# choi403/ALG

Hardware: AMD Instinct MI355X
Metric: frames/sec (whole node) CogVideoX-5B-I2V 49f x 50-step ALG (higher is better)
Workload: dtype bf16; 1 GPU; BASELINE config 2: CogVideoX-5B-I2V bf16, 49 frames @ 480x720, 50 steps, ALG interval down_up (resize_factor 0.25, interval [0, 0.04]), guidance 6.0; one video per GPU; layers=42, dit_sample_forwards=14, parallelism=dp1

## Files before the change

### alg_amd/_lib.py

```python
from __future__ import annotations

import ctypes
from collections import OrderedDict
import os
from ctypes import POINTER, Structure, byref, c_char_p, c_float, c_int, c_int32, c_int64, c_void_p

import torch

_HERE = os.path.dirname(os.path.abspath(__file__))
LIB_PATH = os.environ.get("ALG_HIP_LIB") or os.path.join(_HERE, "libalg_hip.so")

ALG_F32, ALG_BF16 = 0, 1
ACT_NONE, ACT_GELU_TANH, ACT_SILU = 0, 1, 2
GEMM_BIAS_PER_ROW, GEMM_PERMUTE_COLS, GEMM_GATE_F32, GEMM_GATE_SEG_STRIDE = 1, 4, 8, 16
GEMM_B_PACKED11 = 32

EXPORTS = (
    "alg_version", "alg_last_error", "alg_reload_env", "alg_down_up", "alg_gaussian_blur", "alg_cfg_ddim_step", "alg_gemm_bf16", "alg_gemm_bf16_pair", "alg_gemm_bf16_pair_qk", "alg_pack_b_p11", "alg_pack_b_p11_bytes",
    "alg_flash_attn_d64", "alg_layernorm_modulate", "alg_qk_norm_rope", "alg_patchify", "alg_unpatchify",
    "alg_timestep_embedding", "alg_cfg_combine", "alg_lincomb", "alg_unipc_update", "alg_concat_cast", "alg_flash_attn_d128", "alg_layernorm_mod_f32", "alg_layernorm_mod_f32_fp8", "alg_rmsnorm_rope",
    "alg_wan_modulation", "alg_patchify3d", "alg_unpatchify3d", "alg_timestep_embedding_f32", "alg_linear_f32",
    "alg_gelu_erf", "alg_layernorm_modulate_seg", "alg_headnorm_rope", "alg_masked_mean", "alg_silu", "alg_gemm_fp8", "alg_quantize_fp8_rows",
    "alg_conv_cl_bf16", "alg_vae_groupnorm_workspace", "alg_vae_groupnorm_stats", "alg_vae_spatial_norm", "alg_vae_upsample",
    "alg_vae_pack_latent", "alg_vae_unpack_video", "alg_vae_group_norm", "alg_vae_pad", "alg_vae_repitch",
    "alg_vae_unpack_planes", "alg_rms_norm_rows", "alg_softmax_hilo", "alg_flash_attn_d128_ex", "alg_flash_attn_d128_dual", "alg_rope_half", "alg_patchify_t", "alg_unpatchify_t", "alg_qk_norm_rope_scaled", "alg_flash_attn_d64_ex", "alg_embed_rows", "alg_t5_layernorm", "alg_attn_bias", "alg_mul_bf16", "alg_quick_gelu",
    "alg_lowpass_tables_bytes", "alg_lowpass_tables_build", "alg_down_up_workspace_bytes", "alg_gaussian_blur_workspace_bytes",
    "alg_flash_attn_d64_workspace_bytes", "alg_calib_mfma_bf16", "alg_wall_clock_khz", "alg_attn_clock_tap",
)
_RET_I64 = ("alg_vae_groupnorm_workspace", "alg_lowpass_tables_bytes", "alg_down_up_workspace_bytes",
            "alg_gaussian_blur_workspace_bytes", "alg_flash_attn_d64_workspace_bytes", "alg_pack_b_p11_bytes")


class AlgHipError(RuntimeError):
    pass


class GemmArgs(Structure):
    _fields_ = [
        ("A", c_void_p), ("B", c_void_p), ("C", c_void_p), ("bias", c_void_p), ("R", c_void_p), ("gate", c_void_p),
        ("lda", c_int64), ("ldb", c_int64), ("ldc", c_int64), ("ldr", c_int64),
        ("strideA", c_int64), ("strideB", c_int64), ("strideC", c_int64), ("strideR", c_int64),
        ("strideGate", c_int64),
        ("M", c_int32), ("N", c_int32), ("K", c_int32), ("batch", c_int32),
        ("seg_split", c_int32), ("act", c_int32), ("flags", c_int32),
        ("gate_seg_stride", c_int64), ("perm_col0", c_int32), ("conv_cin_log2", c_int32),
        ("a_scale", c_void_p), ("b_scale", c_void_p), ("strideAScale", c_int64), ("strideBScale", c_int64),
        ("conv_wp", c_int32), ("conv_hpwp", c_int32), ("conv_kw", c_int32), ("reserved1", c_int32),
    ]


class QkNormRopeArgs(Structure):
    _fields_ = [("wq", c_void_p), ("bq", c_void_p), ("wk", c_void_p), ("bk", c_void_p), ("cos_tab", c_void_p),
                ("sin_tab", c_void_p), ("heads", c_int32), ("text_len", c_int32), ("eps", c_float),
                ("q_scale", c_float)]


class VaeGeom(Structure):
    _fields_ = [(n, c_int32) for n in ("frames", "H", "W", "C", "first_len", "seg_len", "lat_first_single", "lat_rate",
                                       "lat_scale", "lat_h", "lat_w")]


_lib = None


def build_library(verbose=False):
    import subprocess

    src = os.path.join(_HERE, "csrc")
    r = subprocess.run(["make", "-C", src, "-j8"], capture_output=True, text=True)
    if verbose or r.returncode != 0:
        print(r.stdout[-4000:])
        print(r.stderr[-4000:])
    if r.returncode != 0:
        raise AlgHipError("building libalg_hip.so failed (see output above)")
    return LIB_PATH


def load_library():
    global _lib
    if _lib is not None:
        return _lib
    if not os.path.exists(LIB_PATH):
        raise AlgHipError(
            "%s not found: the HIP extension is not built (run `python -c 'import __graft_entry__ as g; g.build()'` "
            "or `make -C alg_amd/csrc`).  There is no CPU fallback for the ALG hot path." % LIB_PATH)
    lib = ctypes.CDLL(LIB_PATH)
    lib.alg_version.restype = c_int
    lib.alg_last_error.restype = c_char_p
    lib.alg_reload_env.restype = None
    lib.alg_reload_env.argtypes = []
    lib.alg_down_up.argtypes = [c_void_p, c_void_p, c_int64, c_int, c_int, c_int, c_int, c_int, c_int, c_void_p, c_void_p,
                                c_int64, c_void_p]
    lib.alg_gaussian_blur.argtypes = [c_void_p, c_void_p, c_int64, c_int, c_int, c_int, c_float, c_int, c_void_p, c_int64,
                                      c_void_p]
    lib.alg_lowpass_tables_bytes.argtypes = [c_int] * 4
    lib.alg_lowpass_tables_build.argtypes = [c_void_p, c_int64] + [c_int] * 4 + [c_void_p]
    lib.alg_down_up_workspace_bytes.argtypes = [c_int64] + [c_int] * 4
    lib.alg_gaussian_blur_workspace_bytes.argtypes = [c_int64] + [c_int] * 3
    lib.alg_flash_attn_d64_workspace_bytes.argtypes = [c_int] * 4
    lib.alg_pack_b_p11_bytes.argtypes = [c_int, c_int]
    lib.alg_pack_b_p11_bytes.restype = c_int64
    lib.alg_pack_b_p11.argtypes = [c_void_p, c_void_p, c_int, c_int, c_int64, c_void_p]
    lib.alg_cfg_ddim_step.argtypes = [c_void_p, c_int, c_void_p, c_int, c_int, c_int64, c_float, c_float, c_float,
                                      c_float, c_float, c_void_p]
    lib.alg_cfg_combine.argtypes = [c_void_p, c_void_p, c_int, c_int, c_int64, c_float, c_void_p]
    lib.alg_lincomb.argtypes = [POINTER(c_void_p), POINTER(c_float), POINTER(c_int), c_int, c_void_p, c_int, c_int64,
                                c_void_p]
    lib.alg_concat_cast.argtypes = [POINTER(c_void_p), c_int, POINTER(c_void_p), c_int, c_int] + [c_int64] * 7 + [
        c_void_p, c_int, c_void_p]
    lib.alg_flash_attn_d128.argtypes = [c_void_p] * 4 + [c_int] * 4 + [c_int64] * 8 + [c_float, c_void_p]
    lib.alg_flash_attn_d128_ex.argtypes = [c_void_p] * 4 + [c_int] * 4 + [c_int64] * 8 + [c_float, c_int, c_int, c_void_p]
    lib.alg_flash_attn_d128_dual.argtypes = ([c_void_p] * 3 + [c_int] + [c_int64] * 4 + [c_void_p] * 2 + [c_int] + [c_int64] * 4 +
                                             [c_void_p] + [c_int] * 3 + [c_int64] * 4 + [c_float, c_void_p])
    lib.alg_rope_half.argtypes = [c_void_p, c_void_p, c_void_p, c_void_p, c_int64, c_int, c_int64, c_void_p]
    lib.alg_layernorm_mod_f32.argtypes = [c_void_p] * 6 + [c_int64, c_int, c_int, c_int, c_float, c_void_p]
    lib.alg_layernorm_mod_f32_fp8.argtypes = [c_void_p] * 7 + [c_int64, c_int, c_int, c_int, c_float, c_void_p]
    lib.alg_rmsnorm_rope.argtypes = [c_void_p] * 4 + [c_int64, c_int, c_int, c_int, c_float, c_void_p]
    lib.alg_wan_modulation.argtypes = [c_void_p] * 3 + [c_int] * 5 + [c_void_p]
    lib.alg_patchify3d.argtypes = [c_void_p, c_void_p] + [c_int] * 8 + [c_void_p]
    lib.alg_unpatchify3d.argtypes = [c_void_p, c_int64, c_void_p] + [c_int] * 8 + [c_void_p]
    lib.alg_layernorm_modulate_seg.argtypes = [c_void_p] * 6 + [c_int64, c_int64, c_int, c_int, c_int, c_int64, c_int64,
                                               c_int, c_float, c_void_p]
    lib.alg_headnorm_rope.argtypes = [c_void_p] * 4 + [c_int64, c_int64, c_int, c_int, c_int, c_int, c_float, c_void_p]
    lib.alg_masked_mean.argtypes = [c_void_p, c_void_p, c_void_p, c_int, c_int, c_int, c_void_p]
    lib.alg_silu.argtypes = [c_void_p, c_void_p, c_int64, c_void_p]
    lib.alg_rms_norm_rows.argtypes = [c_void_p, c_void_p, c_void_p, c_int64, c_int, c_int, c_int, c_void_p]
    lib.alg_softmax_hilo.argtypes = [c_void_p, c_void_p, c_void_p, c_int64, c_int, c_int64, ctypes.c_float, c_void_p]
    lib.alg_gemm_fp8.argtypes = [POINTER(GemmArgs), c_void_p]
    lib.alg_conv_cl_bf16.argtypes = [c_void_p] * 5 + [c_int] * 7 + [c_void_p]
    lib.alg_vae_groupnorm_workspace.argtypes = [POINTER(VaeGeom)]
    lib.alg_vae_groupnorm_stats.argtypes = [c_void_p, POINTER(VaeGeom), c_float, c_void_p, c_void_p, c_void_p]
    lib.alg_vae_spatial_norm.argtypes = [c_void_p] * 6 + [POINTER(VaeGeom), c_int, c_void_p]
    lib.alg_vae_group_norm.argtypes = [c_void_p] * 5 + [POINTER(VaeGeom), c_int, c_void_p]
    lib.alg_vae_pad.argtypes = [c_void_p, c_void_p] + [c_int] * 4 + [c_void_p]
    lib.alg_vae_repitch.argtypes = [c_void_p, c_void_p] + [c_int] * 6 + [c_void_p]
    lib.alg_vae_unpack_planes.argtypes = [c_void_p, c_void_p] + [c_int] * 4 + [c_void_p]
    lib.alg_embed_rows.argtypes = [c_void_p, c_void_p, c_void_p, c_int64, c_int, c_int, c_void_p]
    lib.alg_t5_layernorm.argtypes = [c_void_p, c_void_p, c_void_p, c_int64, c_int, c_float, c_void_p]
    lib.alg_attn_bias.argtypes = [c_void_p] * 7 + [c_int, c_int, c_int, c_int, c_int64, c_int64, c_float, c_int, c_void_p]
    lib.alg_quick_gelu.argtypes = [c_void_p, c_int64, c_void_p]
    lib.alg_mul_bf16.argtypes = [c_void_p, c_void_p, c_void_p, c_int64, c_void_p]
    lib.alg_vae_upsample.argtypes = [c_void_p, c_void_p] + [c_int] * 6 + [c_void_p]
    lib.alg_vae_pack_latent.argtypes = [c_void_p, c_int64, c_int64, c_void_p, c_int, c_int, c_int, c_int, c_float, c_void_p]
    lib.alg_vae_unpack_video.argtypes = [c_void_p, c_void_p, c_int, c_int, c_int, c_int, c_void_p]
    lib.alg_quantize_fp8_rows.argtypes = [c_void_p, c_int64, c_void_p, c_void_p, c_int64, c_int, c_void_p]
    lib.alg_timestep_embedding_f32.argtypes = [c_void_p, c_void_p, c_int, c_int, c_void_p]
    lib.alg_linear_f32.argtypes = [c_void_p] * 6 + [c_int] * 4 + [c_void_p]
    lib.alg_gelu_erf.argtypes = [c_void_p, c_int64, c_void_p]
    lib.alg_unipc_update.argtypes = [c_void_p] * 5 + [c_int64] + [c_float] * 6 + [c_void_p]
    lib.alg_gemm_bf16.argtypes = [POINTER(GemmArgs), c_void_p]
    lib.alg_gemm_bf16_pair.argtypes = [POINTER(GemmArgs), POINTER(GemmArgs), c_void_p]
    lib.alg_gemm_bf16_pair_qk.argtypes = [POINTER(GemmArgs), POINTER(GemmArgs), POINTER(QkNormRopeArgs), c_void_p]
    lib.alg_flash_attn_d64.argtypes = [c_void_p, c_void_p, c_void_p, c_void_p, c_int, c_int, c_int, c_int64, c_int64,
                                       c_int64, c_int64, c_int64, c_int64, c_float, c_void_p]
    lib.alg_layernorm_modulate.argtypes = [c_void_p, c_void_p, c_void_p, c_void_p, c_void_p, c_void_p, c_int64, c_int,
                                           c_int, c_int, c_int64, c_int64, c_int, c_float, c_void_p]
    lib.alg_qk_norm_rope.argtypes = [c_void_p, c_void_p, c_void_p, c_void_p, c_void_p, c_void_p, c_void_p, c_int,
                                     c_int, c_int, c_int, c_float, c_void_p]
    lib.alg_qk_norm_rope_scaled.argtypes = [c_void_p] * 7 + [c_int, c_int, c_int, c_int, c_float, c_float, c_void_p]
    lib.alg_flash_attn_d64_ex.argtypes = [c_void_p, c_void_p, c_void_p, c_void_p, c_int, c_int, c_int, c_int64, c_int64,
                                          c_int64, c_int64, c_int64, c_int64, c_float, c_int, c_void_p, c_int64, c_void_p]
    lib.alg_patchify.argtypes = [c_void_p, c_int64, POINTER(c_void_p), c_void_p, c_int, c_int, c_int, c_int, c_int,
                                 c_int, c_void_p]
    lib.alg_unpatchify.argtypes = [c_void_p, c_void_p, c_int, c_int, c_int, c_int, c_int, c_int, c_void_p]
    lib.alg_patchify_t.argtypes = [c_void_p, c_int64, POINTER(c_void_p), c_void_p] + [c_int] * 7 + [c_void_p]
    lib.alg_unpatchify_t.argtypes = [c_void_p, c_void_p] + [c_int] * 7 + [c_void_p]
    lib.alg_timestep_embedding.argtypes = [c_void_p, c_void_p, c_int, c_int, c_int, c_void_p]
    lib.alg_calib_mfma_bf16.argtypes = [c_void_p, c_int, ctypes.c_uint, c_int, c_void_p, c_void_p]
    lib.alg_attn_clock_tap.argtypes = [c_void_p, c_int]
    for name in EXPORTS:
        fn = getattr(lib, name)
        if name == "alg_attn_clock_tap":
            fn.restype = None
        elif name not in ("alg_version", "alg_last_error", "alg_reload_env"):
            fn.restype = c_int64 if name in _RET_I64 else c_int
    _lib = lib
    return lib


def reload_env():
    load_library().alg_reload_env()


def _check(rc, what):
    if rc != 0:
        msg = load_library().alg_last_error()
        raise AlgHipError("%s failed (code %d): %s" % (what, rc, msg.decode() if msg else "?"))


def _stream():
    return c_void_p(torch.cuda.current_stream().cuda_stream)


def _dt(t):
    if t.dtype == torch.float32:
        return ALG_F32
    if t.dtype == torch.bfloat16:
        return ALG_BF16
    raise AlgHipError("unsupported dtype %s (the HIP path handles float32 and bfloat16)" % t.dtype)


def _dev(t, name):
    if not t.is_cuda:
        raise AlgHipError("%s must be a device tensor: the ALG hot path is HIP-only (no CPU fallback)" % name)
    return t


def _ptr(t):
    return c_void_p(t.data_ptr()) if t is not None else c_void_p(0)



_TABLES = OrderedDict()
_TABLES_MAX = 64
_SCRATCH = {}
_PINNED = {}


def _stream_key(t):
    return (t.device.index, torch.cuda.current_stream(t.device).cuda_stream)


def _capturing():
    return torch.cuda.is_available() and torch.cuda.is_current_stream_capturing()


def _pin(t):
    _PINNED[id(t)] = t
    return t


def release_captured_buffers():
    _PINNED.clear()


def clear_caches():
    _TABLES.clear()
    _SCRATCH.clear()


def lowpass_tables(x, h1, w1):
    lib = load_library()
    H, W = x.shape[-2:]
    key = _stream_key(x) + (H, W, h1, w1)
    cap = _capturing()
    t = _TABLES.get(key)
    if t is not None:
        _TABLES.move_to_end(key)
        return _pin(t) if cap else t
    n = int(lib.alg_lowpass_tables_bytes(H, W, h1, w1))
    if n <= 0:
        return None
    t = torch.empty(n, dtype=torch.uint8, device=x.device)
    _check(lib.alg_lowpass_tables_build(_ptr(t), n, H, W, h1, w1, _stream()), "alg_lowpass_tables_build")
    if cap:
        return _pin(t)
    _TABLES[key] = t
    while len(_TABLES) > _TABLES_MAX:
        _TABLES.popitem(last=False)
    return t


def scratch(ref, nbytes, tag):
    if nbytes <= 0:
        return None
    key = _stream_key(ref) + (tag,)
    t = _SCRATCH.get(key)
    cap = _capturing()
    if t is None or t.numel() < nbytes:
        t = torch.empty(int(nbytes), dtype=torch.uint8, device=ref.device)
        if cap:
            return _pin(t)
        _SCRATCH[key] = t
    return _pin(t) if cap else t


def calib_mfma_bf16(sink, iters, seed=1, blocks=0, clocks=None):
    lib = load_library()
    if clocks is not None:
        if int(blocks) <= 0:
            blocks = 2 * torch.cuda.get_device_properties(sink.device).multi_processor_count
        if not (clocks.is_cuda and clocks.device == sink.device and clocks.dtype == torch.int64 and clocks.is_contiguous()
                and clocks.numel() >= 4 * int(blocks)):
            raise AlgHipError("calib_mfma_bf16: clocks must be a contiguous int64 tensor on the sink's device with >= 4 * %d "
                              "elements" % int(blocks))
    rc = lib.alg_calib_mfma_bf16(_ptr(_dev(sink, "sink")), int(iters), int(seed), int(blocks), _ptr(clocks), _stream())
    if rc <= 0:
        _check(rc if rc < 0 else -1, "alg_calib_mfma_bf16")
    return rc


def wall_clock_khz():
    return int(load_library().alg_wall_clock_khz())


def attn_clock_tap(buffer):
    lib = load_library()
    if buffer is None:
        lib.alg_attn_clock_tap(None, 0)
        return
    if not (buffer.is_cuda and buffer.dtype == torch.int64 and buffer.is_contiguous() and buffer.dim() == 2 and buffer.shape[1] == 4):
        raise AlgHipError("attn_clock_tap needs a contiguous int64 device tensor [slots, 4]")
    lib.alg_attn_clock_tap(_ptr(buffer), int(buffer.shape[0]))


def clock_mhz_from_taps(taps, wall_khz):
    t = taps.detach().cpu().to(torch.float64)
    dc, dw = t[:, 2] - t[:, 0], t[:, 3] - t[:, 1]
    ok = (dc > 0) & (dw > 0)
    if not bool(ok.any()) or wall_khz <= 0:
        return None
    mhz = dc[ok] / dw[ok] * (wall_khz / 1e3)
    return {"mean": float(mhz.mean()), "min": float(mhz.min()), "max": float(mhz.max()), "workgroups": int(ok.sum())}


def down_up(x, h1, w1, round_intermediate=True):
    lib = load_library()
    _dev(x, "x")
    if not x.is_contiguous():
        raise AlgHipError("down_up needs a contiguous tensor")
    H, W = x.shape[-2:]
    planes = x.numel() // (H * W) if x.numel() else 0
    out = torch.empty_like(x)
    if planes == 0:
        return out
    wsb = int(lib.alg_down_up_workspace_bytes(planes, H, W, h1, w1))
    ws = scratch(x, wsb, "down_up")
    tables = lowpass_tables(x, h1, w1) if wsb == 0 else None
    _check(lib.alg_down_up(_ptr(x), _ptr(out), planes, H, W, h1, w1, _dt(x), 1 if round_intermediate else 0,
                           _ptr(tables), _ptr(ws), wsb, _stream()), "alg_down_up")
    return out


def gaussian_blur(x, ksize, sigma):
    lib = load_library()
    _dev(x, "x")
    if not x.is_contiguous():
        raise AlgHipError("gaussian_blur needs a contiguous tensor")
    H, W = x.shape[-2:]
    planes = x.numel() // (H * W) if x.numel() else 0
    out = torch.empty_like(x)
    wsb = int(lib.alg_gaussian_blur_workspace_bytes(planes, H, W, int(ksize))) if planes else 0
    ws = scratch(x, wsb, "gaussian")
    _check(lib.alg_gaussian_blur(_ptr(x), _ptr(out), planes, H, W, int(ksize), float(sigma), _dt(x), _ptr(ws), wsb,
                                 _stream()), "alg_gaussian_blur")
    return out


def cfg_ddim_step_(pred, latents, n_pass, guidance_scale, sqrt_alpha_t, sqrt_beta_t, coef_a, coef_b):
    lib = load_library()
    _dev(pred, "pred")
    _dev(latents, "latents")
    if not (pred.is_contiguous() and latents.is_contiguous()):
        raise AlgHipError("cfg_ddim_step_ needs contiguous tensors")
    numel = latents.numel()
    if pred.numel() != n_pass * numel:
        raise AlgHipError("pred has %d elements, expected n_pass*numel = %d" % (pred.numel(), n_pass * numel))
    _check(lib.alg_cfg_ddim_step(_ptr(pred), _dt(pred), _ptr(latents), _dt(latents), n_pass, numel,
                                 float(guidance_scale), float(sqrt_alpha_t), float(sqrt_beta_t), float(coef_a),
                                 float(coef_b), _stream()), "alg_cfg_ddim_step")
    return latents


def cfg_combine(pred, n_pass, guidance_scale):
    lib = load_library()
    _dev(pred, "pred")
    if not pred.is_contiguous() or pred.shape[0] % n_pass:
        raise AlgHipError("cfg_combine needs a contiguous [n_pass * B, ...] tensor")
    out = torch.empty((pred.shape[0] // n_pass,) + tuple(pred.shape[1:]), device=pred.device, dtype=pred.dtype)
    _check(lib.alg_cfg_combine(_ptr(pred), _ptr(out), _dt(pred), n_pass, out.numel(), float(guidance_scale), _stream()),
           "alg_cfg_combine")
    return out


def lincomb(terms, out_dtype, out=None):
    lib = load_library()
    xs = [t for _, t in terms]
    for t in xs:
        _dev(t, "term")
        if not t.is_contiguous() or t.shape != xs[0].shape:
            raise AlgHipError("lincomb needs contiguous tensors of one shape")
    n = len(xs)
    if out is None:
        out = torch.empty(xs[0].shape, device=xs[0].device, dtype=out_dtype)
    elif out.dtype != out_dtype or out.shape != xs[0].shape or not out.is_contiguous():
        raise AlgHipError("lincomb: `out` must be a contiguous tensor of the requested dtype and shape")
    arr = (c_void_p * n)(*[t.data_ptr() for t in xs])
    cf = (c_float * n)(*[float(c) for c, _ in terms])
    dts = (c_int * n)(*[_dt(t) for t in xs])
    _check(lib.alg_lincomb(arr, cf, dts, n, _ptr(out), ALG_F32 if out_dtype == torch.float32 else ALG_BF16,
                           out.numel(), _stream()), "alg_lincomb")
    return out


def concat_cast(src0, src1, O, A0, A1, R, s0_ostride, s1_ostride, a1_off, out_dtype):
    lib = load_library()
    n = len(src0)
    for t in list(src0) + list(src1):
        _dev(t, "concat source")
        if not t.is_contiguous():
            raise AlgHipError("concat_cast needs contiguous sources")
    out = torch.empty((n, O, A0 + A1, R), device=src0[0].device, dtype=out_dtype)
    a0 = (c_void_p * n)(*[t.data_ptr() for t in src0])
    a1 = (c_void_p * n)(*[t.data_ptr() for t in src1])
    _check(lib.alg_concat_cast(a0, _dt(src0[0]), a1, _dt(src1[0]), n, O, A0, A1, R, s0_ostride, s1_ostride, a1_off,
                               _ptr(out), ALG_F32 if out_dtype == torch.float32 else ALG_BF16, _stream()),
           "alg_concat_cast")
    return out


def rope_half_(x, cos, sin, pos, rows, heads, x_rstride, x_off=0):
    _check(load_library().alg_rope_half(_p(x, x_off), _p(cos), _p(sin), _p(pos), rows, heads, x_rstride, _stream()),
           "alg_rope_half")
    return x


def flash_attn_d128_dual(q, k, vt, Skv, k_bs, k_rs, vt_bs, vt_rs, k2, vt2, Skv2, k2_bs, k2_rs, vt2_bs, vt2_rs, o, batch, heads, Sq,
                         q_bs, q_rs, o_bs, o_rs, scale):
    lib = load_library()
    for t in (q, k, vt, k2, vt2, o):
        _dev(t, "attention operand")
    _check(lib.alg_flash_attn_d128_dual(_p(q), _p(k), _p(vt), Skv, k_bs, k_rs, vt_bs, vt_rs, _p(k2), _p(vt2), Skv2, k2_bs, k2_rs,
                                        vt2_bs, vt2_rs, _p(o), batch, heads, Sq, q_bs, q_rs, o_bs, o_rs, float(scale), _stream()),
           "alg_flash_attn_d128_dual")
    return o


def flash_attn_d128(q, k, vt, o, batch, heads, Sq, Skv, q_bs, q_rs, k_bs, k_rs, vt_bs, vt_rs, o_bs, o_rs, scale,
                    q_off=0, k_off=0, vt_off=0, o_off=0, kv_group=1, causal=False):
    lib = load_library()
    for t in (q, k, vt, o):
        _dev(t, "attention operand")
    at = lambda t, off: c_void_p(t.data_ptr() + 2 * off)
    if kv_group != 1 or causal:
        _check(lib.alg_flash_attn_d128_ex(at(q, q_off), at(k, k_off), at(vt, vt_off), at(o, o_off), batch, heads, Sq, Skv, q_bs,
                                          q_rs, k_bs, k_rs, vt_bs, vt_rs, o_bs, o_rs, float(scale), int(kv_group),
                                          int(bool(causal)), _stream()), "alg_flash_attn_d128_ex")
        return o
    _check(lib.alg_flash_attn_d128(at(q, q_off), at(k, k_off), at(vt, vt_off), at(o, o_off), batch, heads, Sq, Skv, q_bs, q_rs, k_bs, k_rs, vt_bs, vt_rs, o_bs, o_rs, float(scale),
                                   _stream()), "alg_flash_attn_d128")
    return o


def _p(t, off=0):
    if t is None:
        return c_void_p(0)
    _dev(t, "tensor")
    return c_void_p(t.data_ptr() + off * t.element_size())


def layernorm_mod_f32(x, y, weight, bias, scale, shift, mod_bstride, batch, rows, D, eps, scale_off=0, shift_off=0):
    _check(load_library().alg_layernorm_mod_f32(_p(x), _p(y), _p(weight), _p(bias), _p(scale, scale_off),
                                                _p(shift, shift_off), mod_bstride, batch, rows, D, float(eps), _stream()),
           "alg_layernorm_mod_f32")
    return y


def layernorm_mod_f32_fp8(x, q8, q8_scale, weight, bias, scale, shift, mod_bstride, batch, rows, D, eps, scale_off=0,
                          shift_off=0):
    _check(load_library().alg_layernorm_mod_f32_fp8(_p(x), _p(q8), _p(q8_scale), _p(weight), _p(bias),
                                                    _p(scale, scale_off), _p(shift, shift_off), mod_bstride, batch, rows,
                                                    D, float(eps), _stream()), "alg_layernorm_mod_f32_fp8")
    return q8


def rmsnorm_rope_(x, weight, cos, sin, x_rstride, batch, rows, D, eps, x_off=0):
    _check(load_library().alg_rmsnorm_rope(_p(x, x_off), _p(weight), _p(cos), _p(sin), x_rstride, batch, rows, D,
                                           float(eps), _stream()), "alg_rmsnorm_rope")
    return x


def wan_modulation(table, vec, out, layers, batch, J, D, vec_per_j):
    _check(load_library().alg_wan_modulation(_p(table), _p(vec), _p(out), layers, batch, J, D, int(vec_per_j), _stream()),
           "alg_wan_modulation")
    return out


def patchify3d(x, out, n, C, F, H, W, ph, pw, Kpad):
    _check(load_library().alg_patchify3d(_p(x), _p(out), n, C, F, H, W, ph, pw, Kpad, _stream()), "alg_patchify3d")
    return out


def unpatchify3d(x, ldin, out, n, C, F, H, W, ph, pw, channel_major=False):
    _check(load_library().alg_unpatchify3d(_p(x), ldin, _p(out), n, C, F, H, W, ph, pw, int(channel_major), _stream()),
           "alg_unpatchify3d")
    return out


def layernorm_modulate_seg(x, y, weight, bias, scale, shift, mod_bstride, seg_stride, batch, rows, D, seg_split, eps,
                           x_bstride=None, y_bstride=None, x_off=0, y_off=0, scale_off=0, shift_off=0):
    x_bstride = rows * D if x_bstride is None else x_bstride
    y_bstride = rows * D if y_bstride is None else y_bstride
    _check(load_library().alg_layernorm_modulate_seg(_p(x, x_off), _p(y, y_off), _p(weight), _p(bias), _p(scale, scale_off),
                                                     _p(shift, shift_off), mod_bstride, seg_stride, batch, rows, D,
                                                     x_bstride, y_bstride, seg_split, float(eps), _stream()),
           "alg_layernorm_modulate_seg")
    return y


def headnorm_rope_(x, weight, cos, sin, x_rstride, x_bstride, batch, rows, heads, rope_tokens, eps, x_off=0):
    _check(load_library().alg_headnorm_rope(_p(x, x_off), _p(weight), _p(cos), _p(sin), x_rstride, x_bstride, batch, rows,
                                            heads, rope_tokens, float(eps), _stream()), "alg_headnorm_rope")
    return x


def masked_mean(x, valid, out, batch, L, D):
    _check(load_library().alg_masked_mean(_p(x), _p(valid), _p(out), batch, L, D, _stream()), "alg_masked_mean")
    return out


def silu(x, y):
    _check(load_library().alg_silu(_p(x), _p(y), x.numel(), _stream()), "alg_silu")
    return y


def rms_norm_rows(x, gamma, y, rows, C, Cp, silu=True):
    _check(load_library().alg_rms_norm_rows(_p(x), _p(gamma), _p(y), rows, C, Cp, int(silu), _stream()), "alg_rms_norm_rows")
    return y


def softmax_hilo(neg_hi, lo, p, rows, cols, ld, scale):
    _check(load_library().alg_softmax_hilo(_p(neg_hi), _p(lo), _p(p), rows, cols, ld, float(scale), _stream()),
           "alg_softmax_hilo")
    return p


CONV_PLAIN, CONV_PAIR, CONV_STRIDE2 = 0, 1, 2


def conv_cl(x, w, bias, res, y, frames, Hp, Wp, Cin, Cout, kt, pair=False, stride2=False, x_off=0, y_off=0, res_off=0):
    mode = CONV_STRIDE2 if stride2 else (CONV_PAIR if pair else CONV_PLAIN)
    _check(load_library().alg_conv_cl_bf16(_p(x, x_off), _p(w), _p(bias), _p(res, res_off), _p(y, y_off), frames, Hp, Wp,
                                           Cin, Cout, kt, mode, _stream()), "alg_conv_cl_bf16")
    return y


def embed_rows(ids, table, out):
    _check(load_library().alg_embed_rows(_p(ids), _p(table), _p(out), ids.numel(), table.shape[1], table.shape[0],
                                         _stream()), "alg_embed_rows")
    return out


def t5_layernorm(x, weight, y, rows, D, eps):
    _check(load_library().alg_t5_layernorm(_p(x), _p(weight), _p(y), rows, D, eps, _stream()), "alg_t5_layernorm")
    return y


def attn_bias(qkv, out, bias_table, rel_bucket, key_mask, batch, heads, L, scale=1.0, head_dim=64, causal=False):
    inner = heads * head_dim
    _check(load_library().alg_attn_bias(_p(qkv), _p(qkv, inner), _p(qkv, 2 * inner), _p(out), _p(bias_table),
                                        _p(rel_bucket), _p(key_mask), batch, heads, head_dim, L, 3 * inner, inner,
                                        float(scale), int(causal), _stream()), "alg_attn_bias")
    return out


def quick_gelu_(x):
    _check(load_library().alg_quick_gelu(_p(x), x.numel(), _stream()), "alg_quick_gelu")
    return x


def mul_bf16(a, b, out):
    _check(load_library().alg_mul_bf16(_p(a), _p(b), _p(out), a.numel(), _stream()), "alg_mul_bf16")
    return out


def vae_group_norm(x, stats, gamma, beta, out, g, silu=True):
    _check(load_library().alg_vae_group_norm(_p(x), _p(stats), _p(gamma), _p(beta), _p(out), byref(g), int(silu),
                                             _stream()), "alg_vae_group_norm")
    return out


def vae_pad(x, out, frames, H, W, C):
    _check(load_library().alg_vae_pad(_p(x), _p(out), frames, H, W, C, _stream()), "alg_vae_pad")
    return out


def vae_repitch(x, out, frames, H, W, C, src_rows, src_wp):
    _check(load_library().alg_vae_repitch(_p(x), _p(out), frames, H, W, C, src_rows, src_wp, _stream()), "alg_vae_repitch")
    return out


def vae_unpack_planes(x, out, frames, H, W, C):
    _check(load_library().alg_vae_unpack_planes(_p(x), _p(out), frames, H, W, C, _stream()), "alg_vae_unpack_planes")
    return out


def pack_conv_pair(w, bias, taps_t):
    co = w.shape[0]
    w = w.reshape(co, taps_t, 3, 3, -1)
    wp = w.new_zeros(2, co, taps_t, 3, 4, w.shape[-1])
    wp[0, :, :, :, 0:3] = w
    wp[1, :, :, :, 1:4] = w
    return wp.reshape(2 * co, -1).contiguous(), torch.cat([bias, bias]).contiguous()


def vae_geom(**kw):
    g = VaeGeom()
    for k, v in kw.items():
        setattr(g, k, v)
    return g


def vae_groupnorm_workspace(g):
    n = load_library().alg_vae_groupnorm_workspace(byref(g))
    if n < 0:
        _check(1, "alg_vae_groupnorm_workspace")
    return n


def vae_groupnorm_stats(x, g, eps, workspace, stats):
    _check(load_library().alg_vae_groupnorm_stats(_p(x), byref(g), eps, _p(workspace), _p(stats), _stream()),
           "alg_vae_groupnorm_stats")
    return stats


def vae_spatial_norm(x, stats, gamma, beta, zyb, out, g, silu=True):
    _check(load_library().alg_vae_spatial_norm(_p(x), _p(stats), _p(gamma), _p(beta), _p(zyb), _p(out), byref(g),
                                               int(silu), _stream()), "alg_vae_spatial_norm")
    return out


def vae_upsample(x, out, frames_out, H, W, C, compress_time, first_single):
    _check(load_library().alg_vae_upsample(_p(x), _p(out), frames_out, H, W, C, int(compress_time), int(first_single),
                                           _stream()), "alg_vae_upsample")
    return out


def vae_pack_latent(z, c_stride, frame_stride, out, frames, h, w, channels, scale, z_off=0):
    _check(load_library().alg_vae_pack_latent(_p(z, z_off), c_stride, frame_stride, _p(out), frames, h, w, channels, scale,
                                              _stream()), "alg_vae_pack_latent")
    return out


def vae_unpack_video(x, out, frames, H, W, to_uint8=False):
    _check(load_library().alg_vae_unpack_video(_p(x), _p(out), frames, H, W, int(to_uint8), _stream()),
           "alg_vae_unpack_video")
    return out


def timestep_embedding_f32(t, out, n, dim):
    _check(load_library().alg_timestep_embedding_f32(_p(t), _p(out), n, dim, _stream()), "alg_timestep_embedding_f32")
    return out


def linear_f32(x, W, b, y, y_bf16, y_silu_bf16, M, N, K, act=0):
    _check(load_library().alg_linear_f32(_p(x), _p(W), _p(b), _p(y), _p(y_bf16), _p(y_silu_bf16), M, N, K, act, _stream()),
           "alg_linear_f32")


def gelu_erf_(x):
    _check(load_library().alg_gelu_erf(_p(x), x.numel(), _stream()), "alg_gelu_erf")
    return x


def unipc_update(x, m0, m1, m_new, r, c, k, rk=1.0, rho0=0.0, rho_new=0.0):
    lib = load_library()
    for t in (x, m0, m1, m_new):
        if t is None:
            continue
        _dev(t, "unipc term")
        if t.dtype != torch.float32 or not t.is_contiguous() or t.shape != x.shape:
            raise AlgHipError("unipc_update needs contiguous fp32 tensors of one shape")
    out = torch.empty_like(x)
    p = lambda t: None if t is None else _ptr(t)
    _check(lib.alg_unipc_update(p(x), p(m0), p(m1), p(m_new), _ptr(out), x.numel(), float(r), float(c), float(k),
                                float(rk), float(rho0), float(rho_new), _stream()), "alg_unipc_update")
    return out


def gemm_args(A, B, C, M, N, K, lda, ldb, ldc, bias=None, R=None, ldr=0, gate=None, batch=1, strideA=0, strideB=0,
              strideC=0, strideR=0, strideGate=0, seg_split=0, act=ACT_NONE, flags=0, a_off=0, b_off=0, c_off=0, r_off=0,
              gate_off=0, gate_seg_stride=None, bias_off=0, perm_col0=0, a_scale=None, b_scale=None, strideAScale=0,
              strideBScale=0, a_scale_off=0, b_scale_off=0):
    args = GemmArgs()
    fp8 = a_scale is not None
    if isinstance(B, PackedB):
        if (B.N, B.K) != (N, K) or b_off or strideB:
            raise AlgHipError("packed B was built for N = %d, K = %d (shared by the batch, no offset)" % (B.N, B.K))
        flags |= GEMM_B_PACKED11
    args.A = A.data_ptr() + A.element_size() * a_off
    args.B = B.data_ptr() + B.element_size() * b_off
    if fp8:
        args.a_scale = a_scale.data_ptr() + 4 * a_scale_off
        args.b_scale = b_scale.data_ptr() + 4 * b_scale_off
        args.strideAScale, args.strideBScale = strideAScale, strideBScale
    args.C = C.data_ptr() + 2 * c_off
    args.bias = (bias.data_ptr() + 2 * bias_off) if bias is not None else None
    if gate_seg_stride is not None:
        flags |= GEMM_GATE_SEG_STRIDE
        args.gate_seg_stride = gate_seg_stride
    args.R = (R.data_ptr() + 2 * r_off) if R is not None else None
    args.gate = (gate.data_ptr() + gate.element_size() * gate_off) if gate is not None else None
    args.lda, args.ldb, args.ldc, args.ldr = lda, ldb, ldc, ldr
    args.strideA, args.strideB, args.strideC, args.strideR, args.strideGate = strideA, strideB, strideC, strideR, strideGate
    args.M, args.N, args.K, args.batch = M, N, K, batch
    args.seg_split, args.act, args.flags = seg_split, act, flags
    args.perm_col0 = perm_col0
    return args, fp8


class PackedB:

    def __init__(self, w):
        lib = load_library()
        _dev(w, "weight")
        if w.dtype != torch.bfloat16 or w.dim() != 2 or w.stride(1) != 1:
            raise AlgHipError("PackedB takes a 2-D bf16 weight with unit column stride")
        self.N, self.K = int(w.shape[0]), int(w.shape[1])
        nbytes = int(lib.alg_pack_b_p11_bytes(self.N, self.K))
        if nbytes <= 0:
            raise AlgHipError("PackedB: K = %d must be a positive multiple of 64" % self.K)
        self.data = torch.empty(nbytes, dtype=torch.uint8, device=w.device)
        _check(lib.alg_pack_b_p11(_ptr(w), _ptr(self.data), self.N, self.K, int(w.stride(0)), _stream()), "alg_pack_b_p11")

    def data_ptr(self):
        return self.data.data_ptr()

    def element_size(self):
        return 2


def gemm(*a, **kw):
    lib = load_library()
    args, fp8 = gemm_args(*a, **kw)
    if fp8:
        _check(lib.alg_gemm_fp8(ctypes.byref(args), _stream()), "alg_gemm_fp8")
    else:
        _check(lib.alg_gemm_bf16(ctypes.byref(args), _stream()), "alg_gemm_bf16")


def gemm_pair(first, second):
    lib = load_library()
    a, fa = gemm_args(*first[0], **first[1])
    b, fb = gemm_args(*second[0], **second[1])
    if fa or fb:
        raise AlgHipError("gemm_pair takes bf16 problems")
    _check(lib.alg_gemm_bf16_pair(ctypes.byref(a), ctypes.byref(b), _stream()), "alg_gemm_bf16_pair")


def gemm_pair_qk(first, second, wq, bq, wk, bk, cos, sin, heads, text_len, eps, q_scale=1.0):
    lib = load_library()
    a, fa = gemm_args(*first[0], **first[1])
    b, fb = gemm_args(*second[0], **second[1])
    if fa or fb:
        raise AlgHipError("gemm_pair_qk takes bf16 problems")
    ptrs = [t.data_ptr() if t is not None else None for t in (wq, bq, wk, bk, cos, sin)]
    e = QkNormRopeArgs(*ptrs, heads, text_len, float(eps), float(q_scale))
    _check(lib.alg_gemm_bf16_pair_qk(ctypes.byref(a), ctypes.byref(b), ctypes.byref(e), _stream()), "alg_gemm_bf16_pair_qk")


def quantize_fp8_rows(x, q, scale, rows, K, x_rstride=None, x_off=0, q_off=0, scale_off=0):
    x_rstride = K if x_rstride is None else x_rstride
    _check(load_library().alg_quantize_fp8_rows(_p(x, x_off), x_rstride, _p(q, q_off), _p(scale, scale_off), rows, K,
                                                _stream()), "alg_quantize_fp8_rows")
    return q, scale


ATTN_Q_PRESCALED = 1


def flash_attn_d64(q, k, vt, o, batch, heads, S, q_bstride, q_rstride, vt_bstride, vt_rstride, o_bstride, o_rstride,
                   scale, q_off=0, k_off=0, q_prescaled=False):
    lib = load_library()
    flags = ATTN_Q_PRESCALED if q_prescaled else 0
    wsb = int(lib.alg_flash_attn_d64_workspace_bytes(batch, heads, S, flags))
    ws = scratch(o, wsb, "attn_d64")
    _check(lib.alg_flash_attn_d64_ex(c_void_p(q.data_ptr() + 2 * q_off), c_void_p(k.data_ptr() + 2 * k_off), _ptr(vt),
                                     _ptr(o), batch, heads, S, q_bstride, q_rstride, vt_bstride, vt_rstride, o_bstride,
                                     o_rstride, float(scale), flags, _ptr(ws), wsb, _stream()),
           "alg_flash_attn_d64")


def layernorm_modulate(x, y, weight, bias, scale, shift, mod_bstride, batch, rows, D, seg_split, eps,
                       x_bstride=None, y_bstride=None, x_off=0, y_off=0, scale_off=0, shift_off=0):
    lib = load_library()
    x_bstride = rows * D if x_bstride is None else x_bstride
    y_bstride = rows * D if y_bstride is None else y_bstride
    sc = c_void_p(scale.data_ptr() + 2 * scale_off) if scale is not None else c_void_p(0)
    sh = c_void_p(shift.data_ptr() + 2 * shift_off) if shift is not None else c_void_p(0)
    _check(lib.alg_layernorm_modulate(c_void_p(x.data_ptr() + 2 * x_off), c_void_p(y.data_ptr() + 2 * y_off),
                                      _ptr(weight), _ptr(bias), sc, sh, mod_bstride, batch, rows, D, x_bstride,
                                      y_bstride, seg_split, float(eps), _stream()), "alg_layernorm_modulate")


def qk_norm_rope_(qk, wq, bq, wk, bk, cos, sin, batch, S, heads, text_len, eps, q_scale=1.0):
    lib = load_library()
    _check(lib.alg_qk_norm_rope_scaled(_ptr(qk), _ptr(wq), _ptr(bq), _ptr(wk), _ptr(bk), _ptr(cos), _ptr(sin), batch, S,
                                       heads, text_len, float(eps), float(q_scale), _stream()), "alg_qk_norm_rope")


def patchify(latents, lat_bstride, conds, out, n_samples, frames, C, H, W, p, p_t=1):
    lib = load_library()
    arr = (c_void_p * n_samples)(*[c.data_ptr() for c in conds])
    _check(lib.alg_patchify_t(_ptr(latents), lat_bstride, arr, _ptr(out), n_samples, frames, C, H, W, p, p_t, _stream()),
           "alg_patchify")


def unpatchify(x, out, n_samples, frames, C, H, W, p, p_t=1):
    lib = load_library()
    _check(lib.alg_unpatchify_t(_ptr(x), _ptr(out), n_samples, frames, C, H, W, p, p_t, _stream()), "alg_unpatchify")


def timestep_embedding(t, out, n, dim, flip_sin_to_cos=True):
    lib = load_library()
    _check(lib.alg_timestep_embedding(_ptr(t), _ptr(out), n, dim, 1 if flip_sin_to_cos else 0, _stream()),
           "alg_timestep_embedding")
```

### alg_amd/csrc/gemm.hip

```cpp
#include <stdlib.h>

#include "common.h"

namespace alg {
constexpr int BM = 256, BN = 256;
int launch_gemm_p6(const alg_gemm_args* a, int m_tiles, int n_tiles, int64_t nwg, hipStream_t s);
int launch_gemm_p9(const alg_gemm_args* a, int m_tiles, int n_tiles, int64_t nwg, hipStream_t s);
int launch_gemm_p9_pair(const alg_gemm_args* a, int m_tiles_a, int n_tiles_a, const alg_gemm_args* b, int m_tiles_b, int n_tiles_b,
                        hipStream_t s);
int launch_gemm_p9_pair_qk(const alg_gemm_args* a, int m_tiles_a, int n_tiles_a, const alg_gemm_args* b, int m_tiles_b, int n_tiles_b,
                           const alg_qk_norm_rope_args* e, hipStream_t s);
int launch_gemm_p10(const alg_gemm_args* a, int m_tiles, int n_tiles, int64_t nwg, hipStream_t s);
int launch_gemm_p10_pair(const alg_gemm_args* a, int m_tiles_a, int n_tiles_a, const alg_gemm_args* b, int m_tiles_b, int n_tiles_b,
                         hipStream_t s);
int launch_gemm_p10_pair_qk(const alg_gemm_args* a, int m_tiles_a, int n_tiles_a, const alg_gemm_args* b, int m_tiles_b, int n_tiles_b,
                            const alg_qk_norm_rope_args* e, hipStream_t s);
int launch_gemm_p11(const alg_gemm_args* a, int m_tiles, int n_tiles, int64_t nwg, hipStream_t s);
int launch_gemm_p6_fp8(const alg_gemm_args* a, int m_tiles, int n_tiles, int64_t nwg, hipStream_t s);
int launch_gemm_p9_fp8(const alg_gemm_args* a, int m_tiles, int n_tiles, int64_t nwg, hipStream_t s);
int launch_gemm_p6_conv(const alg_gemm_args* a, int m_tiles, int n_tiles, int64_t nwg, hipStream_t s);
static int gemm_pipe() { return opt(OPT_GEMM_PIPE); }
static bool asm_pipe() { return gemm_pipe() == 9 || gemm_pipe() == 10; }
}

using namespace alg;

static int gemm_entry(const alg_gemm_args* a, void* stream, bool fp8, bool validate_only = false) {
  if (!a || !a->A || !a->B || !a->C) {
    set_error("alg_gemm_bf16: null argument");
    return ALG_EINVAL;
  }
  if (a->M <= 0 || a->N <= 0 || a->K <= 0 || a->batch <= 0) {
    set_error("alg_gemm_bf16: bad shape M=%d N=%d K=%d batch=%d", a->M, a->N, a->K, a->batch);
    return ALG_EINVAL;
  }
  if (a->K % (fp8 ? 128 : 64) != 0) {
    set_error("alg_gemm_%s: K=%d must be a multiple of %d", fp8 ? "fp8" : "bf16", a->K, fp8 ? 128 : 64);
    return ALG_EINVAL;
  }
  const int al = fp8 ? 16 : 8;
  if (a->lda % al || a->ldb % al || a->strideA % al || a->strideB % al || ((uintptr_t)a->A & 15) ||
      ((uintptr_t)a->B & 15)) {
    set_error("alg_gemm: A/B must be 16-byte aligned with lda/ldb/strides multiples of 16 bytes");
    return ALG_EINVAL;
  }
  if (fp8 && (!a->a_scale || !a->b_scale || ((uintptr_t)a->b_scale & 15) || (a->strideBScale & 3))) {
    set_error("alg_gemm_fp8: a_scale / b_scale are required (b_scale 16-byte aligned)");
    return ALG_EINVAL;
  }
  if (a->act < ALG_ACT_NONE || a->act > ALG_ACT_SILU) {
    set_error("alg_gemm_bf16: unknown activation %d", a->act);
    return ALG_EINVAL;
  }
  if ((a->flags & ALG_GEMM_PERMUTE_COLS) && (a->R || a->gate)) {
    set_error("alg_gemm_bf16: PERMUTE_COLS cannot be combined with residual/gate");
    return ALG_EINVAL;
  }
  if (a->R && a->act != ALG_ACT_NONE) {
    set_error("alg_gemm_bf16: an activation cannot be combined with the residual epilogue");
    return ALG_EINVAL;
  }
  if (a->gate && !a->R) {
    set_error("alg_gemm_bf16: gate needs a residual");
    return ALG_EINVAL;
  }
  if ((a->N & 3) == 0) {
    const bool bad = (a->ldc & 3) || (a->strideC & 3) || ((uintptr_t)a->C & 7) ||
                     (a->bias && !(a->flags & ALG_GEMM_BIAS_PER_ROW) && ((uintptr_t)a->bias & 7)) ||
                     (a->R && ((a->ldr & 3) || (a->strideR & 3) || ((uintptr_t)a->R & 7))) ||
                     (a->gate && ((a->strideGate & 3) ||
                                  ((uintptr_t)a->gate & ((a->flags & ALG_GEMM_GATE_F32) ? 15 : 7))));
    if (bad) {
      set_error("alg_gemm_bf16: C/bias/R/gate must be 8-byte aligned with ldc/ldr/strides multiples of 4 elements");
      return ALG_EINVAL;
    }
  }
  if (a->conv_wp) {
    const int cl = a->conv_cin_log2;
    const int taps = (cl >= 6 && cl <= 12) ? a->K >> cl : 0;
    const int kw = a->conv_kw;
    if (fp8 || (kw != 3 && kw != 4) || (taps != 3 * kw && taps != 9 * kw) || (taps << cl) != a->K ||
        (a->lda != ((int64_t)(kw - 2) << cl) && !(kw == 3 && a->lda == (2ll << cl))) || a->conv_wp < 3 ||
        a->conv_hpwp < 3 * a->conv_wp || a->act != ALG_ACT_NONE ||
        ((2ll * a->conv_hpwp + 2ll * a->conv_wp + 3) << cl) >= (1ll << 31)) {
      set_error("alg_gemm_bf16: bad convolution addressing (cin_log2=%d K=%d lda=%lld wp=%d hpwp=%d)", cl, a->K,
                (long long)a->lda, a->conv_wp, a->conv_hpwp);
      return ALG_EINVAL;
    }
  }
  if (validate_only) return ALG_OK;
  if ((int64_t)a->M * a->ldc >= (1ll << 31) || (a->R && (int64_t)a->M * a->ldr >= (1ll << 31))) {
    const int64_t ld = (a->R && a->ldr > a->ldc) ? a->ldr : a->ldc;
    const int64_t rows = ((1ll << 31) - 1) / ld / BM * BM;
    if (a->conv_wp || rows <= 0) {
      set_error("alg_gemm_bf16: M*ldc must stay below 2^31 (32-bit epilogue offsets)");
      return ALG_ELIMIT;
    }
    const int64_t esz = fp8 ? 1 : 2;
    for (int64_t m0 = 0; m0 < a->M; m0 += rows) {
      alg_gemm_args c = *a;
      c.M = (int32_t)((a->M - m0) < rows ? (a->M - m0) : rows);
      c.A = (const char*)a->A + m0 * a->lda * esz;
      c.C = (char*)a->C + m0 * a->ldc * 2;
      if (a->R) c.R = (const char*)a->R + m0 * a->ldr * 2;
      if (a->bias && (a->flags & ALG_GEMM_BIAS_PER_ROW)) c.bias = (const char*)a->bias + m0 * 2;
      if (a->a_scale) c.a_scale = a->a_scale + m0;
      c.seg_split = a->seg_split > m0 ? (int32_t)(a->seg_split - m0) : 0;
      const int rc = gemm_entry(&c, stream, fp8);
      if (rc != ALG_OK) return rc;
    }
    return ALG_OK;
  }
  const int m_tiles = (a->M + BM - 1) / BM, n_tiles = (a->N + BN - 1) / BN;
  const int64_t nwg = (int64_t)m_tiles * n_tiles * a->batch;
  if (nwg > 0x7fffffff) {
    set_error("alg_gemm_bf16: grid too large");
    return ALG_ELIMIT;
  }
  hipStream_t s = (hipStream_t)stream;
  if (fp8) {
    if (asm_pipe() && a->K >= 256 && 256 * a->lda + (int64_t)a->K < (1ll << 32) && 256 * a->ldb + (int64_t)a->K < (1ll << 32))
      return launch_gemm_p9_fp8(a, m_tiles, n_tiles, nwg, s);
    return launch_gemm_p6_fp8(a, m_tiles, n_tiles, nwg, s);
  }
  if (a->conv_wp) return launch_gemm_p6_conv(a, m_tiles, n_tiles, nwg, s);
  if (a->flags & ALG_GEMM_B_PACKED11) {
    if (a->K < 128 || 256 * a->lda * 2 + (int64_t)a->K * 2 >= (1ll << 32) || a->strideB != 0 ||
        (a->flags & (ALG_GEMM_BIAS_PER_ROW | ALG_GEMM_PERMUTE_COLS)) || ((uintptr_t)a->B & 15)) {
      set_error("alg_gemm_bf16: a packed B (ALG_GEMM_B_PACKED11) needs K >= 128, 32-bit byte offsets inside a 256-row A panel, a B shared by "
                "the batch (strideB = 0) and a plain column layout (no per-row bias / column permutation)");
      return ALG_EINVAL;
    }
    return launch_gemm_p11(a, m_tiles, n_tiles, nwg, s);
  }
  switch (gemm_pipe()) {
    case 9:
    case 10:
      if (a->K >= 128 && 256 * a->lda * 2 + (int64_t)a->K * 2 < (1ll << 32) && 256 * a->ldb * 2 + (int64_t)a->K * 2 < (1ll << 32))
        return gemm_pipe() == 10 ? launch_gemm_p10(a, m_tiles, n_tiles, nwg, s) : launch_gemm_p9(a, m_tiles, n_tiles, nwg, s);
      return launch_gemm_p6(a, m_tiles, n_tiles, nwg, s);
    default: return launch_gemm_p6(a, m_tiles, n_tiles, nwg, s);
  }
}

extern "C" int alg_gemm_bf16(const alg_gemm_args* a, void* stream) { return gemm_entry(a, stream, false); }

static bool pair_eligible(const alg_gemm_args* a) {
  return a && a->A && a->B && a->C && !a->R && !a->gate && a->act == ALG_ACT_NONE && !a->conv_wp && a->M > 0 && a->N > 0 &&
         a->batch > 0 && a->K >= 128 && a->K % 64 == 0 && 256 * a->lda * 2 + (int64_t)a->K * 2 < (1ll << 32) &&
         256 * a->ldb * 2 + (int64_t)a->K * 2 < (1ll << 32) && (int64_t)a->M * a->ldc < (1ll << 31) &&
         !(a->lda % 8 || a->ldb % 8 || a->strideA % 8 || a->strideB % 8 || ((uintptr_t)a->A & 15) || ((uintptr_t)a->B & 15)) &&
         ((a->N & 3) != 0 || !((a->ldc & 3) || (a->strideC & 3) || ((uintptr_t)a->C & 7) ||
                               (a->bias && !(a->flags & ALG_GEMM_BIAS_PER_ROW) && ((uintptr_t)a->bias & 7))));
}

extern "C" int alg_gemm_bf16_pair(const alg_gemm_args* a, const alg_gemm_args* b, void* stream) {
  int rc = gemm_entry(a, stream, false, true);
  if (rc == ALG_OK) rc = gemm_entry(b, stream, false, true);
  if (rc != ALG_OK) return rc;
  if (asm_pipe() && pair_eligible(a) && pair_eligible(b)) {
    const int64_t ta = (int64_t)((a->M + BM - 1) / BM) * ((a->N + BN - 1) / BN) * a->batch;
    const int64_t tb = (int64_t)((b->M + BM - 1) / BM) * ((b->N + BN - 1) / BN) * b->batch;
    if (ta + tb <= 0x7fffffff)
      return (gemm_pipe() == 10 ? launch_gemm_p10_pair : launch_gemm_p9_pair)(a, (a->M + BM - 1) / BM, (a->N + BN - 1) / BN, b, (b->M + BM - 1) / BM, (b->N + BN - 1) / BN,
                                 (hipStream_t)stream);
  }
  rc = gemm_entry(a, stream, false);
  return rc != ALG_OK ? rc : gemm_entry(b, stream, false);
}

extern "C" int alg_gemm_bf16_pair_qk(const alg_gemm_args* a, const alg_gemm_args* b, const alg_qk_norm_rope_args* e, void* stream) {
  int rc = gemm_entry(a, stream, false, true);
  if (rc == ALG_OK) rc = gemm_entry(b, stream, false, true);
  if (rc != ALG_OK) return rc;
  if (!e || !e->wq || !e->bq || !e->wk || !e->bk || e->heads <= 0 || e->text_len < 0 || e->text_len > a->M ||
      (e->cos_tab == nullptr) != (e->sin_tab == nullptr)) {
    set_error("alg_gemm_bf16_pair_qk: bad LayerNorm / rotary arguments");
    return ALG_EINVAL;
  }
  if (((uintptr_t)e->wq & 15) || ((uintptr_t)e->bq & 15) || ((uintptr_t)e->wk & 15) || ((uintptr_t)e->bk & 15) ||
      ((uintptr_t)e->cos_tab & 15) || ((uintptr_t)e->sin_tab & 15) || ((uintptr_t)a->C & 15)) {
    set_error("alg_gemm_bf16_pair_qk: pointers must be 16-byte aligned");
    return ALG_EINVAL;
  }
  if (a->N != 2 * e->heads * 64 || a->ldc != a->N || a->strideC != (int64_t)a->M * a->N || (a->flags & ALG_GEMM_PERMUTE_COLS) ||
      a->R || a->act != ALG_ACT_NONE) {
    set_error("alg_gemm_bf16_pair_qk: qk must be a plain GEMM onto the contiguous [batch][S][2][heads][64] tensor (N=%d heads=%d ldc=%lld)",
              a->N, e->heads, (long long)a->ldc);
    return ALG_EINVAL;
  }
  const bool fused = asm_pipe() && pair_eligible(a) && pair_eligible(b) && e->heads % 4 == 0 &&
                     !(a->bias && (a->flags & ALG_GEMM_BIAS_PER_ROW));
  if (fused) {
    const int64_t ta = (int64_t)((a->M + BM - 1) / BM) * ((a->N + BN - 1) / BN) * a->batch;
    const int64_t tb = (int64_t)((b->M + BM - 1) / BM) * ((b->N + BN - 1) / BN) * b->batch;
    if (ta + tb <= 0x7fffffff)
      return (gemm_pipe() == 10 ? launch_gemm_p10_pair_qk : launch_gemm_p9_pair_qk)(a, (a->M + BM - 1) / BM, (a->N + BN - 1) / BN, b, (b->M + BM - 1) / BM, (b->N + BN - 1) / BN, e,
                                    (hipStream_t)stream);
  }
  rc = alg_gemm_bf16_pair(a, b, stream);
  if (rc != ALG_OK) return rc;
  return alg_qk_norm_rope_scaled(a->C, e->wq, e->bq, e->wk, e->bk, e->cos_tab, e->sin_tab, a->batch, a->M, e->heads, e->text_len,
                                 e->eps, e->q_scale, stream);
}

extern "C" int alg_gemm_fp8(const alg_gemm_args* a, void* stream) { return gemm_entry(a, stream, true); }

extern "C" int alg_conv_cl_bf16(const void* x, const void* w, const void* bias, const void* res, void* y, int frames,
                                int Hp, int Wp, int Cin, int Cout, int kt, int mode, void* stream) {
  const bool pair = mode == ALG_CONV_PAIR, down = mode == ALG_CONV_STRIDE2;
  if (frames <= 0 || Hp < 3 || Wp < 3 || (kt != 1 && kt != 3) || Cin < 64 || (Cin & (Cin - 1)) || Cout <= 0 || (Cout & 3) ||
      mode < 0 || mode > ALG_CONV_STRIDE2 || (pair && (((Hp * Wp) & 1) || Cout > 128)) ||
      (down && (kt != 1 || (Hp & 1) || (Wp & 1)))) {
    set_error("alg_conv_cl_bf16: bad shape frames=%d Hp=%d Wp=%d Cin=%d Cout=%d kt=%d (Cin a power of two >= 64, Cout %% 4 == 0)",
              frames, Hp, Wp, Cin, Cout, kt);
    return ALG_EINVAL;
  }
  alg_gemm_args a = {};
  a.A = x, a.B = w, a.C = y, a.bias = bias, a.R = res;
  const int vox = pair ? 2 : 1, kw = pair ? 4 : 3;
  a.lda = (int64_t)vox * Cin, a.ldb = (int64_t)kt * 3 * kw * Cin, a.ldc = (int64_t)vox * Cout, a.ldr = a.ldc;
  a.strideA = (int64_t)Hp * Wp * Cin, a.strideB = 0, a.strideC = (int64_t)Hp * Wp * Cout, a.strideR = a.strideC;
  a.M = Hp * Wp / vox, a.N = vox * Cout, a.K = kt * 3 * kw * Cin, a.batch = frames;
  a.act = ALG_ACT_NONE;
  a.conv_cin_log2 = __builtin_ctz((unsigned)Cin), a.conv_wp = Wp, a.conv_hpwp = Hp * Wp, a.conv_kw = kw;
  if (down) {
    a.A = (const bf16_t*)x + (int64_t)(Wp + 1) * Cin;
    a.lda = 2ll * Cin;
    a.M = (Hp - 2) / 2 * Wp;
    a.strideC = a.strideR = (int64_t)a.M * Cout;
  }
  return gemm_entry(&a, stream, false);
}
```

### alg_amd/csrc/gemm_kernel.h

```cpp
#pragma once
#include <stdlib.h>

#include <type_traits>

#include "common.h"
#include "qk_norm_rope.h"
#ifdef ALG_P9_LOOP_INC
#include ALG_P9_LOOP_INC
#else
#include "gemm_p9_loop.inc"
#endif
#include "gemm_p9_fp8_loop.inc"
#ifdef ALG_P11_LOOP_INC
#include ALG_P11_LOOP_INC
#else
#include "gemm_p11_loop.inc"
#endif
#ifdef ALG_P10_LOOP_INC
#include ALG_P10_LOOP_INC
#else
#include "gemm_p10_loop.inc"
#endif

#ifndef ALG_FP8_MX
#define ALG_FP8_MX 1
#endif

namespace alg {

#ifdef ALG_ABL_NOSTORE
#define ALG_STORE16(ptr, val) asm volatile("" ::"v"((val).x), "v"((val).y), "v"((val).z), "v"((val).w))
#else
#define ALG_STORE16(ptr, val) (*(uint4*)(ptr) = (val))
#endif
#ifdef ALG_GEMM_TAP
static __device__ uint64_t gemm_tap_buf[1024 * 4];
static inline int gemm_tap_read(uint64_t* host) { return hipMemcpyFromSymbol(host, HIP_SYMBOL(gemm_tap_buf), sizeof(uint64_t) * 4096) == hipSuccess ? 0 : -1; }
#endif

#ifndef ALG_AUX_A
#define ALG_AUX_A 0
#endif
#ifndef ALG_AUX_B
#define ALG_AUX_B 0
#endif
constexpr int BM = 256, BN = 256;
constexpr int GEMM_LDS = 128 * 1024;
constexpr int GEMM_LDS_P9 = 160 * 1024;
constexpr int GROUP_M = 8;

template <int V>
struct IntC { static constexpr int value = V; };

template <typename F, int... I>
__device__ __forceinline__ void static_for_impl(F&& f, std::integer_sequence<int, I...>) {
  (f(IntC<I>{}), ...);
}
template <int N, typename F>
__device__ __forceinline__ void static_for(F&& f) {
  static_for_impl(f, std::make_integer_sequence<int, N>{});
}

template <int BLK>
__device__ __forceinline__ f32x16 read_acc_block() {
  float f[16];
  asm volatile("v_accvgpr_read_b32 %0, a[%c16]\n\tv_accvgpr_read_b32 %1, a[%c17]\n\tv_accvgpr_read_b32 %2, a[%c18]\n\t"
               "v_accvgpr_read_b32 %3, a[%c19]\n\tv_accvgpr_read_b32 %4, a[%c20]\n\tv_accvgpr_read_b32 %5, a[%c21]\n\t"
               "v_accvgpr_read_b32 %6, a[%c22]\n\tv_accvgpr_read_b32 %7, a[%c23]\n\tv_accvgpr_read_b32 %8, a[%c24]\n\t"
               "v_accvgpr_read_b32 %9, a[%c25]\n\tv_accvgpr_read_b32 %10, a[%c26]\n\tv_accvgpr_read_b32 %11, a[%c27]\n\t"
               "v_accvgpr_read_b32 %12, a[%c28]\n\tv_accvgpr_read_b32 %13, a[%c29]\n\tv_accvgpr_read_b32 %14, a[%c30]\n\t"
               "v_accvgpr_read_b32 %15, a[%c31]\n\ts_nop 0"
               : "=v"(f[0]), "=v"(f[1]), "=v"(f[2]), "=v"(f[3]), "=v"(f[4]), "=v"(f[5]), "=v"(f[6]), "=v"(f[7]), "=v"(f[8]),
                 "=v"(f[9]), "=v"(f[10]), "=v"(f[11]), "=v"(f[12]), "=v"(f[13]), "=v"(f[14]), "=v"(f[15])
               : "n"(BLK * 16), "n"(BLK * 16 + 1), "n"(BLK * 16 + 2), "n"(BLK * 16 + 3), "n"(BLK * 16 + 4), "n"(BLK * 16 + 5),
                 "n"(BLK * 16 + 6), "n"(BLK * 16 + 7), "n"(BLK * 16 + 8), "n"(BLK * 16 + 9), "n"(BLK * 16 + 10),
                 "n"(BLK * 16 + 11), "n"(BLK * 16 + 12), "n"(BLK * 16 + 13), "n"(BLK * 16 + 14), "n"(BLK * 16 + 15)
               : ALG_GEMM_P9_ACC_CLOBBERS);
  f32x16 r;
#pragma unroll
  for (int e = 0; e < 16; ++e) r[e] = f[e];
  return r;
}

typedef const __attribute__((address_space(1))) void* gptr_t;
typedef __attribute__((address_space(3))) void* lptr_t;

__device__ __forceinline__ float act_apply(float x, int act) {
  if (act == ALG_ACT_GELU_TANH) {
    const float k1 = -2.0f * 1.4426950408889634f * 0.7978845608028654f, k2 = 0.044715f * k1;
    return x * __builtin_amdgcn_rcpf(1.0f + __builtin_amdgcn_exp2f(x * fmaf(k2, x * x, k1)));
  }
  if (act == ALG_ACT_SILU) {
    return x * __builtin_amdgcn_rcpf(1.0f + __builtin_amdgcn_exp2f(-1.4426950408889634f * x));
  }
  return x;
}

__device__ __forceinline__ void unpack4(const uint2 v, float (&f)[4]) {
  f[0] = __uint_as_float(v.x << 16);
  f[1] = __uint_as_float(v.x & 0xffff0000u);
  f[2] = __uint_as_float(v.y << 16);
  f[3] = __uint_as_float(v.y & 0xffff0000u);
}

struct GemmNoPair {};
struct GemmPairArgs {
  alg_gemm_args p;
  int m_tiles, n_tiles, group_m;
};
struct GemmPairQkArgs : GemmPairArgs {
  QkNormRope qe;
};
template <int PAIR> struct GemmPairT { typedef GemmNoPair type; };
template <> struct GemmPairT<1> { typedef GemmPairArgs type; };
template <> struct GemmPairT<2> { typedef GemmPairQkArgs type; };
template <int ACT, bool RES, int PIPE, int WNW = 4, bool FP8 = false, bool CONV = false, int PAIR = 0>
__global__ __launch_bounds__((PIPE == 11 ? 1 : 2) * WNW * 64) void gemm_bf16_kernel(
    const alg_gemm_args p1, int m_tiles1, int n_tiles1, int group_m1, const typename GemmPairT<PAIR>::type pr) {
  constexpr bool P9 = PIPE == 9 || PIPE == 10 || PIPE == 11;
  constexpr bool M16 = PIPE == 10 || PIPE == 11;
  constexpr bool P11 = PIPE == 11;
  constexpr int WMW = P11 ? 1 : 2;
  constexpr int MT = BM / WMW / 32;
  static_assert(!PAIR || (P9 && !P11 && !RES && ACT == ALG_ACT_NONE), "the pair launch is built for the plain schedule-9 / 10 kernels");
  static_assert(!FP8 || PIPE == 6 || PIPE == 9, "the fp8 operands are built on the ping-pong schedule and on schedule 9");
  static_assert(!CONV || (PIPE == 6 && !FP8), "the convolution addressing is built on the bf16 ping-pong schedule");
  typedef typename std::conditional<FP8, uint8_t, bf16_t>::type elem_t;
  constexpr int EPS = 16 / (int)sizeof(elem_t);
  constexpr int GEMM_THREADS = WMW * WNW * 64;
  constexpr int NT = BN / WNW / 32;
  static_assert(PIPE == 0 || PIPE == 6 || PIPE == 7 || PIPE == 8 || P9,
                "schedules built: 0 (2-stage ring), 6 (ping-pong), 7 (4-wave interleaved), 8 (4-wave BK = 32 ring), 9 / 10 (asm loops)");
  static_assert((PIPE == 7 || PIPE == 8 || PIPE == 9 || PIPE == 10) == (WNW == 2) && P11 == (WNW == 4 && WMW == 1),
                "PIPE 7 / 8 / 9 / 10 are the 2 x 2 4-wave layouts, 11 the 1 x 4 one, the others run 8 waves");
  static_assert(!P11 || (!FP8 && !CONV), "schedule 11 takes bf16 plain GEMM addressing with a packed B");
  static_assert(!P9 || !CONV, "schedules 9 / 10 take plain GEMM addressing (bf16, or e4m3 on 9 since round 4)");
  constexpr bool BK64 = true;
  constexpr bool PP = PIPE == 6;
  constexpr int BK = FP8 ? 128 : 64;
  constexpr int NSTAGE = 2;
  constexpr int ROW_BYTES = BK * (int)sizeof(elem_t);
  constexpr int SLOTS = ROW_BYTES / 16;
  constexpr int TILE_BYTES = BM * ROW_BYTES;
  constexpr int STAGE_BYTES = 2 * TILE_BYTES;
  constexpr int LD_PER_OP = TILE_BYTES / (GEMM_THREADS * 16);
  constexpr int ROWS_PER_LD = GEMM_THREADS / SLOTS;
  static_assert(NSTAGE * STAGE_BYTES == GEMM_LDS, "ring must fill the 128 KiB LDS budget");

  extern __shared__ __attribute__((aligned(16))) char smem[];
  const int tid = threadIdx.x;
  const int lane = tid & 63;
  const int wave = __builtin_amdgcn_readfirstlane(tid >> 6);
  const int wm = wave / WNW, wn = wave % WNW;

  constexpr int abl = 0;
#ifdef ALG_GEMM_TAP
  uint64_t tap_loop = 0, tap_tiles = 0;
  const uint64_t tap_c0 = __builtin_readcyclecounter(), tap_r0 = wall_clock64();
#endif
  group_m1 &= 0xffff;
  const int total1 = m_tiles1 * n_tiles1 * p1.batch;
  auto do_tile = [&](const int wg_in) __attribute__((always_inline)) {
  bool second = false;
  if constexpr (PAIR) second = wg_in >= total1;
  const alg_gemm_args& p = [&]() -> const alg_gemm_args& {
    if constexpr (PAIR) return second ? pr.p : p1;
    else return p1;
  }();
  int m_tiles = m_tiles1, n_tiles = n_tiles1, group_m = group_m1, wg = wg_in;
  if constexpr (PAIR) {
    if (second) m_tiles = pr.m_tiles, n_tiles = pr.n_tiles, group_m = pr.group_m, wg = wg_in - total1;
  }
  const int tiles = m_tiles * n_tiles;
  const int b = wg / tiles;
  int t = wg - b * tiles;
  const int grp = t / (group_m * n_tiles);
  const int first_m = grp * group_m;
  const int gsize = min(m_tiles - first_m, group_m);
  t -= grp * group_m * n_tiles;
  const int m0 = (first_m + t % gsize) * BM;
  const int n0 = (t / gsize) * BN;

  const elem_t* A = (const elem_t*)p.A + (int64_t)b * p.strideA;
  const elem_t* B = (const elem_t*)p.B + (int64_t)b * p.strideB;

  const int srow = tid / SLOTS;
  const int sw_src = !BK64 ? ((tid >> 4) & 3) : ((tid >> 4) & 7);
  const int sslot = (tid & (SLOTS - 1)) ^ sw_src;
  const elem_t* a_src[LD_PER_OP];
  const elem_t* b_src[LD_PER_OP];
#pragma unroll
  for (int i = 0; i < LD_PER_OP; ++i) {
    const int r = i * ROWS_PER_LD + srow;
    const int am = (abl & 8) ? 0 : m0, bn = (abl & 8) ? 0 : n0;
    a_src[i] = A + (int64_t)min(am + r, p.M - 1) * p.lda + sslot * EPS;
    b_src[i] = B + (int64_t)min(bn + r, p.N - 1) * p.ldb + sslot * EPS;
  }
  auto a_koff = [&](int kt) -> int {
    if constexpr (CONV) {
      const int cl = p.conv_cin_log2 - 6;
      const int tap = kt >> cl;
      const bool k4 = p.conv_kw == 4;
      const int dt = k4 ? tap / 12 : tap / 9, r9 = tap - dt * (k4 ? 12 : 9);
      const int dy = k4 ? r9 >> 2 : r9 / 3, dx = r9 - dy * (k4 ? 4 : 3);
      return ((dt * p.conv_hpwp + dy * p.conv_wp + dx) << p.conv_cin_log2) + (kt & ((1 << cl) - 1)) * BK;
    } else {
      return kt * BK;
    }
  };
  auto stage = [&](int buf, int kt) {
    char* base = smem + buf * STAGE_BYTES;
#pragma unroll
    for (int i = 0; i < LD_PER_OP; ++i) {
      __builtin_amdgcn_global_load_lds((gptr_t)(a_src[i] + kt * BK),
                                       (lptr_t)(base + (i * GEMM_THREADS + wave * 64) * 16), 16, 0, 0);
      __builtin_amdgcn_global_load_lds((gptr_t)(b_src[i] + kt * BK),
                                       (lptr_t)(base + TILE_BYTES + (i * GEMM_THREADS + wave * 64) * 16), 16, 0, 0);
    }
  };

  auto stage_piece = [&](int buf, int kt, int w) {
    char* base = smem + buf * STAGE_BYTES;
    const int i = w >> 1;
    if (w & 1)
      __builtin_amdgcn_global_load_lds((gptr_t)(b_src[i] + kt * BK),
                                       (lptr_t)(base + TILE_BYTES + (i * GEMM_THREADS + wave * 64) * 16), 16, 0, 0);
    else
      __builtin_amdgcn_global_load_lds((gptr_t)(a_src[i] + kt * BK),
                                       (lptr_t)(base + (i * GEMM_THREADS + wave * 64) * 16), 16, 0, 0);
  };

  const int l31 = lane & 31, h2 = lane >> 5;
  const int sw = !BK64 ? ((l31 >> 2) & 3) : ((l31 >> 1) & 7);
  const int a_row_off = (wm * 128 + l31) * ROW_BYTES;
  const int b_row_off = (wn * (NT * 32) + l31) * ROW_BYTES;
  auto pp_a_row = [&](int mt) { return ((mt >> 1) * 128 + wm * 64 + (mt & 1) * 32 + l31) * ROW_BYTES; };
  auto pp_b_row = [&](int nt) { return (nt * 128 + wn * 32 + l31) * ROW_BYTES; };

  auto fma_frag = [](const bf16x8 bfrag, const bf16x8 afrag, f32x16 c) -> f32x16 {
    if constexpr (FP8) {
      typedef long l2 __attribute__((ext_vector_type(2)));
      const l2 bq = __builtin_bit_cast(l2, bfrag), aq = __builtin_bit_cast(l2, afrag);
      c = __builtin_amdgcn_mfma_f32_32x32x16_fp8_fp8(bq[0], aq[0], c, 0, 0, 0);
      return __builtin_amdgcn_mfma_f32_32x32x16_fp8_fp8(bq[1], aq[1], c, 0, 0, 0);
    } else {
      return __builtin_amdgcn_mfma_f32_32x32x16_bf16(bfrag, afrag, c, 0, 0, 0);
    }
  };

  f32x16 acc[4][NT];
  if constexpr (!P9) {
#pragma unroll
    for (int i = 0; i < 4; ++i)
#pragma unroll
      for (int j = 0; j < NT; ++j)
#pragma unroll
        for (int e = 0; e < 16; ++e) acc[i][j][e] = 0.0f;
  }
  auto get_acc = [&](auto mt_c, auto nt_c) -> f32x16 {
    constexpr int mt = decltype(mt_c)::value, nt = decltype(nt_c)::value;
    if constexpr (P9)
      return read_acc_block<NT * mt + nt>();
    else
      return acc[mt][nt];
  };

  auto load_frags = [&](const char* As, const char* Bs, int ks, bf16x8 (&af)[4], bf16x8 (&bfr)[NT]) {
    const int so = ((2 * ks + h2) ^ sw) * 16;
#pragma unroll
    for (int nt = 0; nt < NT; ++nt) bfr[nt] = *(const bf16x8*)(Bs + b_row_off + nt * 32 * ROW_BYTES + so);
#pragma unroll
    for (int mt = 0; mt < 4; ++mt) af[mt] = *(const bf16x8*)(As + a_row_off + mt * 32 * ROW_BYTES + so);
  };
  auto mma = [&](const bf16x8 (&af)[4], const bf16x8 (&bfr)[NT]) {
#pragma unroll
    for (int mt = 0; mt < 4; ++mt)
#pragma unroll
      for (int nt = 0; nt < NT; ++nt)
        acc[mt][nt] = fma_frag(bfr[nt], af[mt], acc[mt][nt]);
  };
  auto compute = [&](int buf) {
    const char* As = smem + buf * STAGE_BYTES;
    const char* Bs = As + TILE_BYTES;
    constexpr int KS = BK / 16;
    bf16x8 af0[4], bf0[NT], af1[4], bf1[NT];
    load_frags(As, Bs, 0, af0, bf0);
    auto interleave = [&]() {
#pragma unroll
      for (int i = 0; i < 4 + NT; ++i) {
        __builtin_amdgcn_sched_group_barrier(0x008, 1, 0);
        __builtin_amdgcn_sched_group_barrier(0x100, 1, 0);
      }
      __builtin_amdgcn_sched_group_barrier(0x008, 4 * NT - (4 + NT), 0);
    };
    __builtin_amdgcn_sched_barrier(0);
#pragma unroll
    for (int ks = 0; ks < KS; ks += 2) {
      load_frags(As, Bs, ks + 1, af1, bf1);
      mma(af0, bf0);
      interleave();
      __builtin_amdgcn_sched_barrier(0);
      if (ks + 2 < KS) {
        load_frags(As, Bs, ks + 2, af0, bf0);
        mma(af1, bf1);
        interleave();
      } else {
        mma(af1, bf1);
      }
      __builtin_amdgcn_sched_barrier(0);
    }
  };

  const int nk = p.K / BK;
  if constexpr (PIPE == 0) {
    stage(0, 0);
    for (int kt = 0; kt < nk; ++kt) {
      asm volatile("s_waitcnt vmcnt(0)" ::: "memory");
      __syncthreads();
      if (kt + 1 < nk) stage((kt + 1) & 1, kt + 1);
      compute(kt & 1);
    }
  } else if constexpr (PIPE == 6) {
    auto stage_half = [&](int kt, int kind) {
      char* base = smem + (kt & 1) * STAGE_BYTES + (kind >> 1) * TILE_BYTES;
#pragma unroll
      for (int ii = 0; ii < 2; ++ii) {
        const int i = (kind & 1) * 2 + ii;
        const elem_t* src = (kind >> 1) ? b_src[i] + kt * BK : a_src[i] + a_koff(kt);
        if (kind >> 1)
          __builtin_amdgcn_global_load_lds((gptr_t)src, (lptr_t)(base + (i * GEMM_THREADS + wave * 64) * 16), 16, 0, ALG_AUX_B);
        else
          __builtin_amdgcn_global_load_lds((gptr_t)src, (lptr_t)(base + (i * GEMM_THREADS + wave * 64) * 16), 16, 0, ALG_AUX_A);
      }
    };
    bf16x8 af[2][4], b0f[4], b1f[4];
    auto load_a = [&](const char* As, int half) {
#pragma unroll
      for (int m2 = 0; m2 < 2; ++m2)
#pragma unroll
        for (int ks = 0; ks < 4; ++ks)
          af[m2][ks] = *(const bf16x8*)(As + pp_a_row(half * 2 + m2) + (((2 * ks + h2) ^ sw) * 16));
    };
    auto load_b = [&](const char* Bs, int half, bf16x8 (&bf)[4]) {
#pragma unroll
      for (int ks = 0; ks < 4; ++ks) bf[ks] = *(const bf16x8*)(Bs + pp_b_row(half) + (((2 * ks + h2) ^ sw) * 16));
    };
    auto quad = [&](int mh, int nt, const bf16x8 (&bf)[4]) {
      __builtin_amdgcn_s_setprio(1);
      if constexpr (FP8 && ALG_FP8_MX) {
        typedef int i8v __attribute__((ext_vector_type(8)));
        typedef int i4v __attribute__((ext_vector_type(4)));
        auto cat = [](const bf16x8 lo, const bf16x8 hi) -> i8v {
          const i4v l = __builtin_bit_cast(i4v, lo), h = __builtin_bit_cast(i4v, hi);
          return i8v{l[0], l[1], l[2], l[3], h[0], h[1], h[2], h[3]};
        };
#pragma unroll
        for (int kp = 0; kp < 2; ++kp) {
          const i8v bq = cat(bf[2 * kp], bf[2 * kp + 1]);
#pragma unroll
          for (int m2 = 0; m2 < 2; ++m2)
            acc[mh * 2 + m2][nt] = __builtin_amdgcn_mfma_scale_f32_32x32x64_f8f6f4(
                bq, cat(af[m2][2 * kp], af[m2][2 * kp + 1]), acc[mh * 2 + m2][nt], 0, 0, 0, 0x7f7f7f7f, 0, 0x7f7f7f7f);
        }
      } else {
#pragma unroll
        for (int ks = 0; ks < 4; ++ks)
#pragma unroll
          for (int m2 = 0; m2 < 2; ++m2)
            acc[mh * 2 + m2][nt] = fma_frag(bf[ks], af[m2][ks], acc[mh * 2 + m2][nt]);
      }
      __builtin_amdgcn_s_setprio(0);
    };
    auto enter_mfma = [&]() {
      asm volatile("s_waitcnt lgkmcnt(0)" ::: "memory");
      __builtin_amdgcn_s_barrier();
      __builtin_amdgcn_sched_barrier(0);
    };
    auto leave_mfma = [&]() {
      __builtin_amdgcn_sched_barrier(0);
      __builtin_amdgcn_s_barrier();
      __builtin_amdgcn_sched_barrier(0);
    };
    stage_half(0, 0); stage_half(0, 3); stage_half(0, 1); stage_half(0, 2);
    if (nk > 1) {
      stage_half(1, 0); stage_half(1, 3); stage_half(1, 1);
      asm volatile("s_waitcnt vmcnt(6)" ::: "memory");
    } else {
      asm volatile("s_waitcnt vmcnt(0)" ::: "memory");
    }
    __builtin_amdgcn_s_barrier();
    if (wm == 1) __builtin_amdgcn_s_barrier();
    for (int t = 0; t < nk; ++t) {
      const char* As = smem + (t & 1) * STAGE_BYTES;
      const char* Bs = As + TILE_BYTES;
      bool do_b0 = true, do_b1 = true;
      if constexpr (CONV) {
        if (p.conv_kw == 4 && p.N == 256) {
          const int dx = (t >> (p.conv_cin_log2 - 6)) & 3;
          do_b0 = dx != 3, do_b1 = dx != 0;
        }
      }
      load_a(As, 0);
      if (do_b0) load_b(Bs, 0, b0f);
      if (t + 1 < nk) stage_half(t + 1, 2);
      enter_mfma();
      if (do_b0) quad(0, 0, b0f);
      leave_mfma();
      if (do_b1) load_b(Bs, 1, b1f);
      if (t + 2 < nk) stage_half(t + 2, 0);
      enter_mfma();
      if (do_b1) quad(0, 1, b1f);
      leave_mfma();
      load_a(As, 1);
      if (t + 2 < nk) stage_half(t + 2, 3);
      enter_mfma();
      if (do_b1) quad(1, 1, b1f);
      leave_mfma();
      if (t + 2 < nk) {
        stage_half(t + 2, 1);
        asm volatile("s_waitcnt vmcnt(6)" ::: "memory");
      } else {
        asm volatile("s_waitcnt vmcnt(0)" ::: "memory");
      }
      enter_mfma();
      if (do_b0) quad(1, 0, b0f);
      leave_mfma();
    }
    if (wm == 0) __builtin_amdgcn_s_barrier();
  } else if constexpr (PIPE == 7) {
    constexpr int NDMA = 2 * LD_PER_OP;
    bf16x8 af0[4], bf0[NT], af1[4], bf1[NT];
    auto il_ds = [&]() {
#pragma unroll
      for (int i = 0; i < 4 + NT; ++i) {
        __builtin_amdgcn_sched_group_barrier(0x008, 1, 0);
        __builtin_amdgcn_sched_group_barrier(0x100, 1, 0);
      }
      __builtin_amdgcn_sched_group_barrier(0x008, 4 * NT - (4 + NT), 0);
    };
    auto il_ds_dma = [&]() {
#pragma unroll
      for (int i = 0; i < 4 + NT; ++i) {
        __builtin_amdgcn_sched_group_barrier(0x008, 1, 0);
        __builtin_amdgcn_sched_group_barrier(0x100, 1, 0);
      }
#pragma unroll
      for (int i = 0; i < NDMA / 2; ++i) {
        __builtin_amdgcn_sched_group_barrier(0x008, 1, 0);
        __builtin_amdgcn_sched_group_barrier(0x010, 1, 0);
      }
    };
    auto iter = [&](int kt, auto dma0_c, auto bar_c, auto dma3_c) {
      constexpr bool DMA0 = decltype(dma0_c)::value, BAR = decltype(bar_c)::value, DMA3 = decltype(dma3_c)::value;
      const char* As = smem + (kt & 1) * STAGE_BYTES;
      const char* Bs = As + TILE_BYTES;
      load_frags(As, Bs, 1, af1, bf1);
      mma(af0, bf0);
      if (DMA0) {
#pragma unroll
        for (int w = NDMA / 2; w < NDMA; ++w) stage_piece((kt + 1) & 1, kt + 1, w);
        il_ds_dma();
      } else {
        il_ds();
      }
      __builtin_amdgcn_sched_barrier(0);
      load_frags(As, Bs, 2, af0, bf0);
      mma(af1, bf1);
      il_ds();
      __builtin_amdgcn_sched_barrier(0);
      load_frags(As, Bs, 3, af1, bf1);
      mma(af0, bf0);
      il_ds();
      __builtin_amdgcn_sched_barrier(0);
// ... 377 lines not shown
      }
      __builtin_amdgcn_sched_barrier(0);
      auto park_band = [&](auto mt_c, auto br_c) {
        constexpr int mt = decltype(mt_c)::value;
        constexpr bool BR = decltype(br_c)::value != 0;
        const float a_sc = a_sc4[mt];
        static_for<NT>([&](auto nt_c) {
          constexpr int nt = decltype(nt_c)::value;
          const f32x16 blk = get_acc(mt_c, nt_c);
#pragma unroll
          for (int g = 0; g < 4; ++g) {
            const float brow = brow4[mt][rq(g)];
            float bv[4], sv[4] = {1.f, 1.f, 1.f, 1.f};
            if constexpr (BIAS_F32) {
#pragma unroll
              for (int i = 0; i < 4; ++i) bv[i] = bvf[nt][cq(g)][i];
            } else {
              unpack4(bcol[nt][cq(g)], bv);
            }
            if constexpr (FP8) {
              const float4 s4 = scol[nt][g];
              sv[0] = s4.x * a_sc; sv[1] = s4.y * a_sc; sv[2] = s4.z * a_sc; sv[3] = s4.w * a_sc;
            }
            float v[4];
#pragma unroll
            for (int i = 0; i < 4; ++i) {
              const float dot = FP8 ? blk[4 * g + i] * sv[i] : blk[4 * g + i];
              v[i] = BR ? dot + bv[i] + brow : dot + bv[i];
            }
            if constexpr (ACT != ALG_ACT_NONE) {
#pragma unroll
              for (int i = 0; i < 4; i += 2) {
                const uint32_t pk = pack_bf2(v[i], v[i + 1]);
                v[i] = act_apply(__uint_as_float(pk << 16), ACT);
                v[i + 1] = act_apply(__uint_as_float(pk & 0xffff0000u), ACT);
              }
            }
            uint2 o;
            o.x = pack_bf2(v[0], v[1]);
            o.y = pack_bf2(v[2], v[3]);
            if constexpr (M16) {
              const int pr_ = quad_row(g, lane_e), pc_ = quad_col(g, lane_e);
              *(uint2*)(my + (mt * NT + nt) * 2048 + pr_ * 64 + (((pc_ >> 3) ^ ((pr_ >> 2) & 3)) * 16) + (pc_ & 7) * 2) = o;
            } else {
              *(uint2*)(my + (mt * NT + nt) * 2048 + l31_e * 64 + ((g ^ ((l31_e >> 2) & 3)) * 16) + h2_e * 8) = o;
            }
          }
          if constexpr (FP8 && PIPE == 9) __builtin_amdgcn_sched_barrier(0);
        });
      };
      if constexpr (NT_OUTER) {
        uint2 bc[2][4];
        float4 sc4[2][4];
        auto load_cols = [&](auto nt_c) {
          constexpr int nt = decltype(nt_c)::value;
#pragma unroll
          for (int g = 0; g < 4; ++g) {
            const int n = n0 + blk_col(nt) + 8 * g + 4 * h2_e;
            const int nc = n < p.N ? n : 0;
            bc[nt & 1][g] = (bias && !bias_row) ? *(const uint2*)(bias + nc) : make_uint2(0u, 0u);
            sc4[nt & 1][g] = *(const float4*)(p.b_scale + (int64_t)b * p.strideBScale + nc);
          }
        };
        load_cols(IntC<0>{});
        static_for<NT>([&](auto nt_c) {
          constexpr int nt = decltype(nt_c)::value;
          if constexpr (nt + 1 < NT) load_cols(IntC<nt + 1>{});
          static_for<4>([&](auto mt_c) {
            constexpr int mt = decltype(mt_c)::value;
            const float a_sc = a_sc4[mt];
            const f32x16 blk = get_acc(mt_c, nt_c);
#pragma unroll
            for (int g = 0; g < 4; ++g) {
              float bv[4];
              unpack4(bc[nt & 1][g], bv);
              const float4 s4 = sc4[nt & 1][g];
              const float sv[4] = {s4.x * a_sc, s4.y * a_sc, s4.z * a_sc, s4.w * a_sc};
              float v[4];
#pragma unroll
              for (int i = 0; i < 4; ++i) v[i] = blk[4 * g + i] * sv[i] + bv[i];
              uint2 o;
              o.x = pack_bf2(v[0], v[1]);
              o.y = pack_bf2(v[2], v[3]);
              *(uint2*)(my + (mt * NT + nt) * 2048 + l31_e * 64 + ((g ^ ((l31_e >> 2) & 3)) * 16) + h2_e * 8) = o;
            }
            __builtin_amdgcn_sched_barrier(0);
          });
        });
      } else {
      constexpr bool BR_SPLIT = !RES && ACT == ALG_ACT_NONE;
      constexpr bool BR_ALWAYS = BR_SPLIT && FP8 && PIPE == 9;
      if (BR_ALWAYS) {
        static_for<MT>([&](auto mt_c) { park_band(mt_c, IntC<1>{}); });
      } else if (BR_SPLIT && bias && bias_row) {
        static_for<MT>([&](auto mt_c) { park_band(mt_c, IntC<1>{}); });
      } else {
        static_for<MT>([&](auto mt_c) { park_band(mt_c, IntC<0>{}); });
      }
      }
      asm volatile("s_waitcnt lgkmcnt(0)" ::: "memory");
      if (RES && !P9) {
#pragma unroll
        for (int it = 0; it < NIT; ++it) {
          const int blk = it >> 1, mt = blk / NT, nt = blk % NT;
          const int rr = (it & 1) * 16 + (lane_e >> 2), ch = lane_e & 3;
          const int row = m0 + blk_row(mt) + rr;
          const int c0 = n0 + blk_col(nt) + ch * 8;
          rbuf[it] = (row < p.M && c0 < p.N) ? *(const uint4*)(R + row * ldr + c0) : make_uint4(0, 0, 0, 0);
        }
        __builtin_amdgcn_sched_barrier(0);
      }
      if constexpr (RES) {
        auto res_loop = [&](auto kind_c) {
          constexpr int KIND = decltype(kind_c)::value;
          if constexpr (!GATE_EARLY) load_gates();
          if constexpr (KIND == 1) {
#pragma unroll
            for (int nt = 0; nt < NT; ++nt)
              asm volatile("" : "+v"(g0p[nt].x), "+v"(g0p[nt].y), "+v"(g0p[nt].z), "+v"(g0p[nt].w), "+v"(g1p[nt].x),
                           "+v"(g1p[nt].y), "+v"(g1p[nt].z), "+v"(g1p[nt].w));
          }
          if constexpr (KIND == 2) {
#pragma unroll
            for (int nt = 0; nt < NT; ++nt)
              asm volatile("" : "+v"(gfa[nt].x), "+v"(gfa[nt].y), "+v"(gfa[nt].z), "+v"(gfa[nt].w), "+v"(gfb[nt].x),
                           "+v"(gfb[nt].y), "+v"(gfb[nt].z), "+v"(gfb[nt].w));
          }
          const int lrow = lane_e >> 2, ch = lane_e & 3;
          const uint32_t voff = (uint32_t)(lrow * ldc + ch * 8) * 2;
          const char* ldsl = my + lrow * 64 + ((ch ^ ((lrow >> 2) & 3)) * 16);
          auto lds_raw = [&](auto it_c) -> uint4 {
            constexpr int it = decltype(it_c)::value;
            return *(const uint4*)(ldsl + (it >> 1) * 2048 + (it & 1) * 1024);
          };
          uint4 raw_next = lds_raw(IntC<0>{});
          static_for<NIT>([&](auto it_c) {
            constexpr int it = decltype(it_c)::value;
            constexpr int blk = it >> 1, mt = blk / NT, nt = blk % NT;
            const uint4 raw = raw_next;
            if constexpr (it + 1 < NIT) raw_next = lds_raw(IntC<it + 1>{});
            const int r0 = m0 + blk_row(mt) + (it & 1) * 16, cb = n0 + blk_col(nt);
            char* const cp = (char*)(Cb + (int64_t)r0 * ldc + cb);
            const bool ok = lrow < p.M - r0 && ch * 8 < p.N - cb;
            const uint4 rraw = rbuf[it];
            const uint32_t u[4] = {raw.x, raw.y, raw.z, raw.w};
            const uint32_t ru[4] = {rraw.x, rraw.y, rraw.z, rraw.w};
            uint32_t gu[4] = {0, 0, 0, 0};
            float gq[8] = {1.f, 1.f, 1.f, 1.f, 1.f, 1.f, 1.f, 1.f};
            if constexpr (KIND == 1) {
              const bool seg1 = lrow >= p.seg_split - r0;
              gu[0] = seg1 ? g1p[nt].x : g0p[nt].x; gu[1] = seg1 ? g1p[nt].y : g0p[nt].y;
              gu[2] = seg1 ? g1p[nt].z : g0p[nt].z; gu[3] = seg1 ? g1p[nt].w : g0p[nt].w;
            }
            if constexpr (KIND == 2) {
              gq[0] = gfa[nt].x; gq[1] = gfa[nt].y; gq[2] = gfa[nt].z; gq[3] = gfa[nt].w;
              gq[4] = gfb[nt].x; gq[5] = gfb[nt].y; gq[6] = gfb[nt].z; gq[7] = gfb[nt].w;
            }
            float y[8];
#pragma unroll
            for (int k = 0; k < 4; ++k) {
              const float x0 = __uint_as_float(u[k] << 16), x1 = __uint_as_float(u[k] & 0xffff0000u);
              const float r0f = __uint_as_float(ru[k] << 16), r1f = __uint_as_float(ru[k] & 0xffff0000u);
              if constexpr (KIND == 0) {
                y[2 * k] = r0f + x0;
                y[2 * k + 1] = r1f + x1;
              } else if constexpr (KIND == 1) {
                const uint32_t pk = pack_bf2(__uint_as_float(gu[k] << 16) * x0, __uint_as_float(gu[k] & 0xffff0000u) * x1);
                y[2 * k] = r0f + __uint_as_float(pk << 16);
                y[2 * k + 1] = r1f + __uint_as_float(pk & 0xffff0000u);
              } else {
                float m0_ = gq[2 * k] * x0, m1_ = gq[2 * k + 1] * x1;
                asm volatile("" : "+v"(m0_), "+v"(m1_));
                y[2 * k] = r0f + m0_;
                y[2 * k + 1] = r1f + m1_;
              }
            }
            if (ok) {
              uint4 outv;
              outv.x = pack_bf2(y[0], y[1]); outv.y = pack_bf2(y[2], y[3]);
              outv.z = pack_bf2(y[4], y[5]); outv.w = pack_bf2(y[6], y[7]);
              ALG_STORE16(cp + voff, outv);
            }
            __builtin_amdgcn_sched_barrier(0);
          });
        };
        if (gkind == 0) { res_loop(IntC<0>{}); return; }
        if (gkind == 1) { res_loop(IntC<1>{}); return; }
        if (gkind == 2) { res_loop(IntC<2>{}); return; }
      } else {
        const int lrow = lane_e >> 2, ch = lane_e & 3;
        const uint32_t voff = (uint32_t)(lrow * ldc + ch * 8) * 2;
        const char* ldsl = my + lrow * 64 + ((ch ^ ((lrow >> 2) & 3)) * 16);
        auto plain_loop = [&](auto perm_c) {
          constexpr bool PERM = decltype(perm_c)::value != 0;
          static_for<NIT / 8>([&](auto grp_c) {
            constexpr int g0 = decltype(grp_c)::value * 8;
            uint4 raw[8];
            static_for<8>([&](auto j_c) {
              constexpr int it = g0 + decltype(j_c)::value;
              raw[decltype(j_c)::value] = *(const uint4*)(ldsl + (it >> 1) * 2048 + (it & 1) * 1024);
            });
            static_for<8>([&](auto j_c) {
              constexpr int it = g0 + decltype(j_c)::value;
              constexpr int blk = it >> 1, mt = blk / NT, nt = blk % NT;
              const int r0 = m0 + blk_row(mt) + (it & 1) * 16, cb = n0 + blk_col(nt);
              const uint4 outv = raw[decltype(j_c)::value];
              if (lrow < p.M - r0 && ch * 8 < p.N - cb) {
                if constexpr (PERM) {
                  const int c0 = cb + ch * 8;
                  bf16_t* crow = Cb + (int64_t)(r0 + lrow) * ldc;
                  const int base = col0 + (c0 & ~12), b3 = (c0 >> 3) & 1;
                  *(uint2*)(crow + base + (b3 << 2)) = make_uint2(outv.x, outv.y);
                  *(uint2*)(crow + base + 8 + (b3 << 2)) = make_uint2(outv.z, outv.w);
                } else {
                  ALG_STORE16((char*)(Cb + (int64_t)r0 * ldc + cb) + voff, outv);
                }
              }
            });
            __builtin_amdgcn_sched_barrier(0);
          });
        };
        if constexpr (PAIR == 2) {
          if (!second) {
            const QkNormRope& e = pr.qe;
            const bool is_k = n0 >= e.heads * 64;
            const float qs = is_k ? 1.0f : e.q_scale;
            float wA[8], bA[8], wB[8], bB[8];
            unpack8(*(const uint4*)((is_k ? e.wk : e.wq) + ch * 8), wA);
            unpack8(*(const uint4*)((is_k ? e.wk : e.wq) + 32 + ch * 8), wB);
            unpack8(*(const uint4*)((is_k ? e.bk : e.bq) + ch * 8), bA);
            unpack8(*(const uint4*)((is_k ? e.bk : e.bq) + 32 + ch * 8), bB);
            const bool any_rope = e.cos_tab && e.text_len < p.M;
            float tab[2][32] = {};
            bool rp[2];
            auto fetch = [&](auto u_c) {
              constexpr int u = decltype(u_c)::value, slot = u & 1;
              const int srow = m0 + blk_row(u >> 1) + (u & 1) * 16 + lrow;
              rp[slot] = any_rope && srow >= e.text_len && srow < p.M;
              if (any_rope) {
                const int64_t pos = rp[slot] ? (int64_t)(srow - e.text_len) * 64 + ch * 8 : (int64_t)ch * 8;
                const float4 c0 = *(const float4*)(e.cos_tab + pos), c1 = *(const float4*)(e.cos_tab + pos + 4);
                const float4 c2 = *(const float4*)(e.cos_tab + pos + 32), c3 = *(const float4*)(e.cos_tab + pos + 36);
                const float4 s0 = *(const float4*)(e.sin_tab + pos), s1 = *(const float4*)(e.sin_tab + pos + 4);
                const float4 s2 = *(const float4*)(e.sin_tab + pos + 32), s3 = *(const float4*)(e.sin_tab + pos + 36);
                const float4 q[8] = {c0, c1, c2, c3, s0, s1, s2, s3};
#pragma unroll
                for (int k = 0; k < 8; ++k)
                  tab[slot][4 * k] = q[k].x, tab[slot][4 * k + 1] = q[k].y, tab[slot][4 * k + 2] = q[k].z, tab[slot][4 * k + 3] = q[k].w;
              }
            };
            fetch(IntC<0>{});
            static_for<8>([&](auto u_c) {
              constexpr int u = decltype(u_c)::value, mt = u >> 1, half = u & 1, slot = u & 1;
              uint4 raw[4];
              static_for<4>([&](auto nt_c) {
                constexpr int nt = decltype(nt_c)::value;
                raw[nt] = *(const uint4*)(ldsl + (mt * NT + nt) * 2048 + half * 1024);
              });
              const bool roped = rp[slot];
              float csA[8], csB[8], snA[8], snB[8];
#pragma unroll
              for (int k = 0; k < 8; ++k)
                csA[k] = tab[slot][k], csB[k] = tab[slot][8 + k], snA[k] = tab[slot][16 + k], snB[k] = tab[slot][24 + k];
              if constexpr (u + 1 < 8) fetch(IntC<u + 1>{});
              static_for<2>([&](auto hh_c) {
                constexpr int hh = decltype(hh_c)::value;
                uint4& ra = raw[2 * hh];
                uint4& rb = raw[2 * hh + 1];
                float va[8], vb[8];
                unpack8(ra, va);
                unpack8(rb, vb);
                float sa = qk_chunk_sum(va), sb = qk_chunk_sum(vb);
                sa += __shfl_xor(sa, 1, 64); sb += __shfl_xor(sb, 1, 64);
                sa += __shfl_xor(sa, 2, 64); sb += __shfl_xor(sb, 2, 64);
                const float mean = qk_mean(sa + sb);
                float qa = qk_chunk_sqdev(va, mean), qb = qk_chunk_sqdev(vb, mean);
                qa += __shfl_xor(qa, 1, 64); qb += __shfl_xor(qb, 1, 64);
                qa += __shfl_xor(qa, 2, 64); qb += __shfl_xor(qb, 2, 64);
                const float rstd = qk_rstd(qa + qb, e.eps);
                float oa[8], ob[8];
                qk_ln_chunk(va, mean, rstd, wA, bA, roped, qs, oa);
                qk_ln_chunk(vb, mean, rstd, wB, bB, roped, qs, ob);
                float ta[8], tb[8];
#pragma unroll
                for (int k = 0; k < 8; ++k) ta[k] = oa[k], tb[k] = ob[k];
                qk_rope_chunk(ta, csA, snA, qs);
                qk_rope_chunk(tb, csB, snB, qs);
#pragma unroll
                for (int k = 0; k < 8; ++k) oa[k] = roped ? ta[k] : oa[k], ob[k] = roped ? tb[k] : ob[k];
                ra = pack8(oa);
                rb = pack8(ob);
              });
              const int r0 = m0 + blk_row(mt) + half * 16;
              static_for<4>([&](auto nt_c) {
                constexpr int nt = decltype(nt_c)::value;
                const int cb = n0 + blk_col(nt);
                if (lrow < p.M - r0 && ch * 8 < p.N - cb) *(uint4*)((char*)(Cb + (int64_t)r0 * ldc + cb) + voff) = raw[nt];
              });
              __builtin_amdgcn_sched_barrier(0);
            });
            return;
          }
        }
        if (perm) plain_loop(IntC<1>{}); else plain_loop(IntC<0>{});
        return;
      }
#pragma unroll
      for (int it = 0; it < NIT; ++it) {
        const int blk = it >> 1, mt = blk / NT, nt = blk % NT;
        const int rr = (it & 1) * 16 + (lane_e >> 2), ch = lane_e & 3;
        const uint4 raw = *(const uint4*)(my + blk * 2048 + rr * 64 + ((ch ^ ((rr >> 2) & 3)) * 16));
        const int row = m0 + blk_row(mt) + rr;
        const int c0 = n0 + blk_col(nt) + ch * 8;
        if (row < p.M && c0 < p.N) {
          uint4 outv = raw;
          if (RES) {
            float x[8], r[8], gq[8];
            const uint32_t u[4] = {raw.x, raw.y, raw.z, raw.w};
            const uint4 rraw = rbuf[it];
            const uint32_t ru[4] = {rraw.x, rraw.y, rraw.z, rraw.w};
#pragma unroll
            for (int k = 0; k < 4; ++k) {
              x[2 * k] = __uint_as_float(u[k] << 16);
              x[2 * k + 1] = __uint_as_float(u[k] & 0xffff0000u);
              r[2 * k] = __uint_as_float(ru[k] << 16);
              r[2 * k + 1] = __uint_as_float(ru[k] & 0xffff0000u);
              gq[2 * k] = gq[2 * k + 1] = 1.0f;
            }
            const bool seg1 = row >= p.seg_split;
            if (gate) {
              if (gate_f32) {
                const float* gp = (const float*)p.gate + (int64_t)b * p.strideGate + (seg1 ? gate_seg : 0) + c0;
                const float4 g0 = *(const float4*)gp, g1 = *(const float4*)(gp + 4);
                gq[0] = g0.x; gq[1] = g0.y; gq[2] = g0.z; gq[3] = g0.w; gq[4] = g1.x; gq[5] = g1.y; gq[6] = g1.z; gq[7] = g1.w;
              } else {
                const uint4 graw = *(const uint4*)(gate + (seg1 ? gate_seg : 0) + c0);
                const uint32_t gu[4] = {graw.x, graw.y, graw.z, graw.w};
#pragma unroll
                for (int k = 0; k < 4; ++k) {
                  gq[2 * k] = __uint_as_float(gu[k] << 16);
                  gq[2 * k + 1] = __uint_as_float(gu[k] & 0xffff0000u);
                }
              }
            }
            float y[8];
#pragma unroll
            for (int k = 0; k < 8; ++k) y[k] = gate_f32 ? r[k] + gq[k] * x[k] : r[k] + rbf(gq[k] * x[k]);
            outv.x = pack_bf2(y[0], y[1]); outv.y = pack_bf2(y[2], y[3]);
            outv.z = pack_bf2(y[4], y[5]); outv.w = pack_bf2(y[6], y[7]);
          }
          bf16_t* crow = Cb + row * ldc;
          if (perm) {
            const int base = col0 + (c0 & ~12), b3 = (c0 >> 3) & 1;
            *(uint2*)(crow + base + (b3 << 2)) = make_uint2(outv.x, outv.y);
            *(uint2*)(crow + base + 8 + (b3 << 2)) = make_uint2(outv.z, outv.w);
          } else {
            *(uint4*)(crow + c0) = outv;
          }
        }
      }
      return;
    }
  }

  auto epilogue_band = [&](auto mt_c) {
    constexpr int mt = decltype(mt_c)::value;
    int row_[NRQ], rowc_[NRQ];
    float brow_[NRQ];
#pragma unroll
    for (int r = 0; r < NRQ; ++r) {
      row_[r] = (PP ? m0 + (mt >> 1) * 128 + wm * 64 + (mt & 1) * 32 : m0 + wm * (MT * 32) + mt * 32) + quad_row(2 * r, lane);
      rowc_[r] = row_[r] < p.M ? row_[r] : p.M - 1;
      brow_[r] = (bias && bias_row) ? bf2f(bias[rowc_[r]]) : 0.0f;
    }
    const float a_sc = FP8 ? p.a_scale[(int64_t)b * p.strideAScale + rowc_[0]] : 1.0f;
    static_for<NT>([&](auto nt_c) {
      constexpr int nt = decltype(nt_c)::value;
      const f32x16 blk = get_acc(mt_c, nt_c);
#pragma unroll
      for (int g = 0; g < 4; ++g) {
        const int row = row_[rq(g)], rowc = rowc_[rq(g)];
        const bool row_ok = row < p.M;
        const float brow = brow_[rq(g)];
        const bool seg1 = row >= p.seg_split;
        const int n = (PP ? n0 + nt * 128 + wn * 32 : n0 + wn * (NT * 32) + nt * 32) + quad_col(g, lane);
        if (n_vec) {
          if (n < p.N) {
            float bv[4] = {0.f, 0.f, 0.f, 0.f}, gv[4] = {1.f, 1.f, 1.f, 1.f}, rv[4] = {0.f, 0.f, 0.f, 0.f};
            if (bias && !bias_row) unpack4(*(const uint2*)(bias + n), bv);
            if (RES && gate) {
              if (gate_f32) {
                const float4 g4 = *(const float4*)((const float*)p.gate + (int64_t)b * p.strideGate + (seg1 ? gate_seg : 0) + n);
                gv[0] = g4.x; gv[1] = g4.y; gv[2] = g4.z; gv[3] = g4.w;
              } else {
                unpack4(*(const uint2*)(gate + (seg1 ? gate_seg : 0) + n), gv);
              }
            }
            if (RES) unpack4(*(const uint2*)(R + rowc * ldr + n), rv);
            float sv[4] = {1.f, 1.f, 1.f, 1.f};
            if (FP8) {
              const float4 s4 = *(const float4*)(p.b_scale + (int64_t)b * p.strideBScale + n);
              sv[0] = s4.x * a_sc; sv[1] = s4.y * a_sc; sv[2] = s4.z * a_sc; sv[3] = s4.w * a_sc;
            }
            float v[4];
#pragma unroll
            for (int i = 0; i < 4; ++i) {
              const float dot = FP8 ? blk[4 * g + i] * sv[i] : blk[4 * g + i];
              float x = rbf(dot + bv[i] + brow);
              if (ACT != ALG_ACT_NONE) x = rbf(act_apply(x, ACT));
              if (RES) x = gate_f32 ? rv[i] + gv[i] * x : rv[i] + rbf(gv[i] * x);
              v[i] = x;
            }
            if (row_ok) {
              const int nc = perm ? col0 + ((n & ~12) | ((n & 4) << 1) | ((n & 8) >> 1)) : n;
              uint2 o;
              o.x = pack_bf2(v[0], v[1]);
              o.y = pack_bf2(v[2], v[3]);
              *(uint2*)(Cb + row * ldc + nc) = o;
            }
          }
        } else {
#pragma unroll
          for (int i = 0; i < 4; ++i) {
            const int nn = n + i;
            if (nn < p.N && row_ok) {
              const float dot = FP8 ? blk[4 * g + i] * (a_sc * p.b_scale[(int64_t)b * p.strideBScale + nn]) : blk[4 * g + i];
              float x = rbf(dot + ((bias && !bias_row) ? bf2f(bias[nn]) : 0.0f) + brow);
              if (ACT != ALG_ACT_NONE) x = rbf(act_apply(x, ACT));
              if (RES) {
                if (gate_f32) {
                  x = bf2f(R[rowc * ldr + nn]) +
                      ((const float*)p.gate)[(int64_t)b * p.strideGate + (seg1 ? gate_seg : 0) + nn] * x;
                } else {
                  const float gg = gate ? bf2f(gate[(seg1 ? gate_seg : 0) + nn]) : 1.0f;
                  x = bf2f(R[rowc * ldr + nn]) + rbf(gg * x);
                }
              }
              const int nj = nn + col0;
              const int nc = perm ? ((nj & ~12) | ((nj & 4) << 1) | ((nj & 8) >> 1)) : nn;
              Cb[row * ldc + nc] = f2bf(x);
            }
          }
        }
      }
    });
  };
#ifndef ALG_EPI_STAGED_ONLY
  static_for<MT>([&](auto mt_c) { epilogue_band(mt_c); });
#endif
  };

  int total_wg = total1;
  if constexpr (PAIR) total_wg += pr.m_tiles * pr.n_tiles * pr.p.batch;
  for (int L = blockIdx.x; L < total_wg; L += gridDim.x) {
    const int xcd = L & 7, q = total_wg >> 3, r = total_wg & 7;
    const int wg = (xcd < r ? xcd * (q + 1) : r * (q + 1) + (xcd - r) * q) + (L >> 3);
    if (L != (int)blockIdx.x) __syncthreads();
    do_tile(wg);
  }
#ifdef ALG_GEMM_TAP
  if (threadIdx.x == 0 && blockIdx.x < 1024) {
    uint64_t* t = gemm_tap_buf + blockIdx.x * 4;
    t[0] = __builtin_readcyclecounter() - tap_c0, t[1] = wall_clock64() - tap_r0, t[2] = tap_loop, t[3] = tap_tiles;
  }
#endif
}

inline unsigned gemm_grid(int64_t nwg) {
  static std::atomic<int> cus{0};
  int n = cus.load();
  if (n == 0) {
    hipDeviceProp_t prop;
    int dev = 0;
    n = (hipGetDevice(&dev) == hipSuccess && hipGetDeviceProperties(&prop, dev) == hipSuccess) ? prop.multiProcessorCount : 256;
    n &= ~7;
    if (n < 8) n = 8;
    cus.store(n);
  }
  return (unsigned)(nwg < n ? nwg : n);
}

inline int gemm_group_m(int pipe, int n_tiles = 0, int K = 0) {
  const int dflt = (pipe != 9 && pipe != 10 && pipe != 11) ? GROUP_M : n_tiles >= 32 ? 4 : (K >= 8192 && n_tiles <= 16) ? 2 : 3;
#ifdef ALG_GROUP_M_OVERRIDE
  return ALG_GROUP_M_OVERRIDE;
#endif
  return dflt;
}

}

using namespace alg;

template <int PIPE, int WNW = 4, bool FP8 = false>
int launch_gemm(const alg_gemm_args* a, int m_tiles, int n_tiles, int64_t nwg, hipStream_t s) {
  constexpr int LDS = (PIPE == 9 || PIPE == 10 || PIPE == 11) ? GEMM_LDS_P9 : GEMM_LDS;
  static PerDeviceOnce attr_set;
  const int dev_slot = current_device_slot();
  if (!device_done(attr_set, dev_slot)) {
    const void* fns[4] = {(const void*)gemm_bf16_kernel<ALG_ACT_NONE, true, PIPE, WNW, FP8>,
                          (const void*)gemm_bf16_kernel<ALG_ACT_GELU_TANH, false, PIPE, WNW, FP8>,
                          (const void*)gemm_bf16_kernel<ALG_ACT_SILU, false, PIPE, WNW, FP8>,
                          (const void*)gemm_bf16_kernel<ALG_ACT_NONE, false, PIPE, WNW, FP8>};
    for (const void* fn : fns) {
      hipError_t e = hipFuncSetAttribute(fn, hipFuncAttributeMaxDynamicSharedMemorySize, LDS);
      if (e != hipSuccess) {
        set_error("alg_gemm_bf16: hipFuncSetAttribute(%d B LDS): %s", LDS, hipGetErrorString(e));
        return ALG_ELAUNCH;
      }
    }
    device_mark(attr_set, dev_slot);
  }
  const dim3 grid(gemm_grid(nwg)), block((PIPE == 11 ? 1 : 2) * WNW * 64);
  const int gm = gemm_group_m(PIPE, n_tiles, a->K);
  if (a->R) {
    hipLaunchKernelGGL((gemm_bf16_kernel<ALG_ACT_NONE, true, PIPE, WNW, FP8>), grid, block, LDS, s, *a, m_tiles,
                       n_tiles, gm, GemmNoPair{});
  } else if (a->act == ALG_ACT_GELU_TANH) {
    hipLaunchKernelGGL((gemm_bf16_kernel<ALG_ACT_GELU_TANH, false, PIPE, WNW, FP8>), grid, block, LDS, s, *a, m_tiles,
                       n_tiles, gm, GemmNoPair{});
  } else if (a->act == ALG_ACT_SILU) {
    hipLaunchKernelGGL((gemm_bf16_kernel<ALG_ACT_SILU, false, PIPE, WNW, FP8>), grid, block, LDS, s, *a, m_tiles,
                       n_tiles, gm, GemmNoPair{});
  } else {
    hipLaunchKernelGGL((gemm_bf16_kernel<ALG_ACT_NONE, false, PIPE, WNW, FP8>), grid, block, LDS, s, *a, m_tiles,
                       n_tiles, gm, GemmNoPair{});
  }
  return check_launch("alg_gemm_bf16");
}
```

### alg_amd/csrc/gemm_p11.hip

```cpp
#include "gemm_kernel.h"

namespace alg {
int launch_gemm_p11(const alg_gemm_args* a, int m_tiles, int n_tiles, int64_t nwg, hipStream_t s) {
  return launch_gemm<11, 4>(a, m_tiles, n_tiles, nwg, s);
}

__global__ __launch_bounds__(256) void pack_b_p11_kernel(const bf16_t* __restrict__ w, uint4* __restrict__ out, int N, int K, int64_t ldb,
                                                          int64_t total) {
  const int64_t i = (int64_t)blockIdx.x * 256 + threadIdx.x;
  if (i >= total) return;
  const int lane = (int)(i & 63);
  const int f = (int)((i >> 6) & 7), wv = (int)((i >> 9) & 3);
  const int64_t tile = i >> 11;
  const int nkt = K / 64;
  const int kt = (int)(tile % nkt);
  const int64_t nt = tile / nkt;
  const int n = (int)(nt * 256) + wv * 64 + (f & 3) * 16 + (lane & 15);
  const int k = kt * 64 + (f >> 2) * 32 + (lane >> 4) * 8;
  uint4 v = make_uint4(0u, 0u, 0u, 0u);
  if (n < N) v = *(const uint4*)(w + (int64_t)n * ldb + k);
  out[i] = v;
}
}

using namespace alg;

extern "C" int64_t alg_pack_b_p11_bytes(int N, int K) {
  if (N <= 0 || K <= 0 || K % 64) return 0;
  return (int64_t)((N + 255) / 256) * (K / 64) * 32768;
}

extern "C" int alg_pack_b_p11(const void* w, void* packed, int N, int K, int64_t ldb, void* stream) {
  if (!w || !packed || N <= 0 || K < 128 || K % 64 || ldb < K || ldb % 8 || ((uintptr_t)w & 15) || ((uintptr_t)packed & 15)) {
    set_error("alg_pack_b_p11: bad argument (N=%d K=%d ldb=%lld; K a multiple of 64 and >= 128, 16-byte aligned rows)", N, K, (long long)ldb);
    return ALG_EINVAL;
  }
  const int64_t total = alg_pack_b_p11_bytes(N, K) / 16;
  hipLaunchKernelGGL(pack_b_p11_kernel, dim3((unsigned)((total + 255) / 256)), dim3(256), 0, (hipStream_t)stream, (const bf16_t*)w,
                     (uint4*)packed, N, K, ldb, total);
  return check_launch("alg_pack_b_p11");
}

#ifdef ALG_GEMM_TAP
extern "C" int alg_dbg_gemm_tap(uint64_t* host) { return alg::gemm_tap_read(host); }
#endif
```

### alg_amd/transformer_cogvideox.py

```python
from __future__ import annotations

import math
import os
from dataclasses import dataclass, asdict
from typing import Optional

import torch

from . import _lib


@dataclass
class CogVideoXTransformerConfig:

    num_attention_heads: int = 48
    attention_head_dim: int = 64
    in_channels: int = 32
    out_channels: int = 16
    num_layers: int = 42
    time_embed_dim: int = 512
    text_embed_dim: int = 4096
    max_text_seq_length: int = 226
    sample_width: int = 90
    sample_height: int = 60
    sample_frames: int = 49
    patch_size: int = 2
    patch_size_t: Optional[int] = None
    temporal_compression_ratio: int = 4
    ff_inner_mult: int = 4
    norm_eps: float = 1e-5
    qk_norm_eps: float = 1e-6
    flip_sin_to_cos: bool = True
    freq_shift: int = 0
    use_rotary_positional_embeddings: bool = True
    use_learned_positional_embeddings: bool = True
    ofs_embed_dim: Optional[int] = None
    spatial_interpolation_scale: float = 1.875
    temporal_interpolation_scale: float = 1.0

    @property
    def inner_dim(self):
        return self.num_attention_heads * self.attention_head_dim

    def to_dict(self):
        return asdict(self)


def _bf(t, device):
    return t.to(device=device, dtype=torch.bfloat16).contiguous()


class CogVideoXTransformer3DModel:
    dtype = torch.bfloat16

    def __init__(self, config: CogVideoXTransformerConfig, weights: dict, device="cuda"):
        cfg = self.config = config
        self.device = torch.device(device)
        if self.device.type != "cuda":
            raise _lib.AlgHipError("CogVideoXTransformer3DModel runs on the GPU only (HIP kernels, no CPU fallback)")
        if cfg.attention_head_dim != 64:
            raise _lib.AlgHipError("the attention kernel is specialised for head_dim 64")
        if cfg.ofs_embed_dim is not None and cfg.ofs_embed_dim != cfg.time_embed_dim:
            raise _lib.AlgHipError("ofs_embed_dim must equal time_embed_dim (emb = emb + ofs_emb)")
        D = cfg.inner_dim
        if D % 512:
            raise _lib.AlgHipError("inner_dim must be a multiple of 512 (LayerNorm kernel tiling)")
        _lib.load_library()
        self.attn_prescale = True
        self.pair_qkv = True
        self.fuse_qk_norm = False
        self.packed_weights = True
        self._sincos = {}
        dev = self.device
        w = weights
        p = cfg.patch_size
        self.p_t = cfg.patch_size_t or 1
        self.k_patch = cfg.in_channels * p * p * self.p_t
        if self.k_patch % 64 or cfg.text_embed_dim % 64 or cfg.time_embed_dim % 64:
            raise _lib.AlgHipError("GEMM K dimensions must be multiples of 64")
        self.w_patch = _bf(w["patch_embed.proj.weight"].reshape(D, self.k_patch), dev)
        self.b_patch = _bf(w["patch_embed.proj.bias"], dev)
        self.w_text = _bf(w["patch_embed.text_proj.weight"], dev)
        self.b_text = _bf(w["patch_embed.text_proj.bias"], dev)
        self.pos_emb = _bf(w["patch_embed.pos_embedding"][0], dev) if cfg.use_learned_positional_embeddings else None
        self.w_t1 = _bf(w["time_embedding.linear_1.weight"], dev)
        self.b_t1 = _bf(w["time_embedding.linear_1.bias"], dev)
        self.w_t2 = _bf(w["time_embedding.linear_2.weight"], dev)
        self.b_t2 = _bf(w["time_embedding.linear_2.bias"], dev)
        if cfg.ofs_embed_dim is not None:
            self.w_o1, self.b_o1 = _bf(w["ofs_embedding.linear_1.weight"], dev), _bf(w["ofs_embedding.linear_1.bias"], dev)
            self.w_o2, self.b_o2 = _bf(w["ofs_embedding.linear_2.weight"], dev), _bf(w["ofs_embedding.linear_2.bias"], dev)

        def reorder6(t):
            c = t.chunk(6, dim=0)
            return torch.cat([c[3], c[0], c[4], c[1], c[5], c[2]], dim=0)

        mw, mb = [], []
        self.layers = []
        for i in range(cfg.num_layers):
            b = "transformer_blocks.%d." % i
            L = {}
            for nm in ("norm1", "norm2"):
                mw.append(reorder6(w[b + nm + ".linear.weight"]))
                mb.append(reorder6(w[b + nm + ".linear.bias"]))
                L[nm + "_w"] = _bf(w[b + nm + ".norm.weight"], dev)
                L[nm + "_b"] = _bf(w[b + nm + ".norm.bias"], dev)
            L["wqk"] = _bf(torch.cat([w[b + "attn1.to_q.weight"], w[b + "attn1.to_k.weight"]], dim=0), dev)
            L["bqk"] = _bf(torch.cat([w[b + "attn1.to_q.bias"], w[b + "attn1.to_k.bias"]], dim=0), dev)
            L["wv"] = _bf(w[b + "attn1.to_v.weight"], dev)
            L["bv"] = _bf(w[b + "attn1.to_v.bias"], dev)
            for nm in ("norm_q", "norm_k"):
                L[nm + "_w"] = _bf(w[b + "attn1." + nm + ".weight"], dev)
                L[nm + "_b"] = _bf(w[b + "attn1." + nm + ".bias"], dev)
            L["wo"] = _bf(w[b + "attn1.to_out.0.weight"], dev)
            L["bo"] = _bf(w[b + "attn1.to_out.0.bias"], dev)
            L["wf1"] = _bf(w[b + "ff.net.0.proj.weight"], dev)
            L["bf1"] = _bf(w[b + "ff.net.0.proj.bias"], dev)
            L["wf2"] = _bf(w[b + "ff.net.2.weight"], dev)
            L["bf2"] = _bf(w[b + "ff.net.2.bias"], dev)
            for nm in ("wo", "wf1", "wf2"):
                L["p" + nm] = _lib.PackedB(L[nm])
            self.layers.append(L)
        ow, ob = w["norm_out.linear.weight"], w["norm_out.linear.bias"]
        sh_w, sc_w = ow.chunk(2, dim=0)
        sh_b, sc_b = ob.chunk(2, dim=0)
        mw.append(torch.cat([sh_w, sh_w, sc_w, sc_w], dim=0))
        mb.append(torch.cat([sh_b, sh_b, sc_b, sc_b], dim=0))
        self.w_mod = _bf(torch.cat(mw, dim=0), dev)
        self.b_mod = _bf(torch.cat(mb, dim=0), dev)
        self.mod_cols = self.w_mod.shape[0]
        self.norm_final_w = _bf(w["norm_final.weight"], dev)
        self.norm_final_b = _bf(w["norm_final.bias"], dev)
        self.norm_out_w = _bf(w["norm_out.norm.weight"], dev)
        self.norm_out_b = _bf(w["norm_out.norm.bias"], dev)
        self.w_out = _bf(w["proj_out.weight"], dev)
        self.b_out = _bf(w["proj_out.bias"], dev)
        self._ws = {}
        self._rope_cache = {}
        self.profile = None

    def _positional(self, Hh, Ww, Fr, S):
        cfg = self.config
        learned = cfg.use_learned_positional_embeddings
        if not learned and cfg.use_rotary_positional_embeddings:
            return None
        pre_frames = (Fr - 1) * cfg.temporal_compression_ratio + 1
        if learned and pre_frames == cfg.sample_frames and self.pos_emb is not None and self.pos_emb.shape[0] == S:
            return self.pos_emb
        p = cfg.patch_size
        gh, gw, gt = Hh // p, Ww // p, Fr // self.p_t
        key = (gh, gw, gt)
        hit = self._sincos.get(key)
        if hit is None:
            D = cfg.inner_dim
            ds, dt = 3 * D // 4, D // 4

            def sc1(dim, pos):
                omega = 1.0 / 10000 ** (torch.arange(dim // 2, dtype=torch.float64) / (dim / 2.0))
                out = torch.outer(pos.reshape(-1).double(), omega)
                return torch.cat([out.sin(), out.cos()], dim=1)

            hh = torch.arange(gh, dtype=torch.float32) / cfg.spatial_interpolation_scale
            ww = torch.arange(gw, dtype=torch.float32) / cfg.spatial_interpolation_scale
            tt = torch.arange(gt, dtype=torch.float32) / cfg.temporal_interpolation_scale
            grid = torch.stack(torch.meshgrid(ww, hh, indexing="xy"), dim=0).reshape(2, 1, gh, gw)
            sp = torch.cat([sc1(ds // 2, grid[0]), sc1(ds // 2, grid[1])], dim=1)
            tp = sc1(dt, tt)
            pe = torch.cat([tp[:, None].expand(-1, gh * gw, -1), sp[None].expand(gt, -1, -1)], dim=-1).reshape(gt * gh * gw, D)
            joint = torch.zeros(cfg.max_text_seq_length + pe.shape[0], D, dtype=torch.float32)
            joint[cfg.max_text_seq_length:] = pe.float()
            hit = joint.to(device=self.device, dtype=torch.bfloat16).contiguous()
            self._sincos[key] = hit
        if hit.shape[0] != S:
            raise ValueError("positional embedding covers %d tokens, the sequence has %d" % (hit.shape[0], S))
        return hit

    def _timed(self, name, fn, *args, **kwargs):
        if self.profile is None:
            return fn(*args, **kwargs)
        e0, e1 = torch.cuda.Event(enable_timing=True), torch.cuda.Event(enable_timing=True)
        e0.record()
        out = fn(*args, **kwargs)
        e1.record()
        self.profile.setdefault(name, []).append((e0, e1))
        return out

    @classmethod
    def from_synthetic(cls, config=None, seed=1234, std=0.02, device="cuda", randomize_affine=False):
        from .weights import synthetic_state_dict

        config = config or CogVideoXTransformerConfig()
        return cls(config, synthetic_state_dict(config, seed=seed, std=std, device=device,
                                                 randomize_affine=randomize_affine), device=device)

    @classmethod
    def from_pretrained(cls, path, subfolder="transformer", torch_dtype=torch.bfloat16, device="cuda", **_):
        from .weights import load_diffusers_transformer

        config, sd = load_diffusers_transformer(path, subfolder)
        return cls(config, sd, device=device)

    def to(self, *args, **kwargs):
        return self

    def _workspace(self, N, S, P):
        key = (N, S, P)
        ws = self._ws.get(key)
        if ws is not None:
            return ws
        cfg, dev = self.config, self.device
        D = cfg.inner_dim
        bf = dict(device=dev, dtype=torch.bfloat16)
        S_pad = (S + 127) // 128 * 128
        ws = dict(
            S_pad=S_pad,
            x=torch.empty(N, S, D, **bf),
            y=torch.empty(N, S, D, **bf),
            qk=torch.empty(N, S, 2 * D, **bf),
            vt=torch.zeros(N, D, S_pad, **bf),
            att=torch.empty(N, S, D, **bf),
            h=torch.empty(N, S, cfg.ff_inner_mult * D, **bf),
            patches=torch.empty(N, P, self.k_patch, **bf),
            tsin=torch.empty(N, D, **bf),
            t1=torch.empty(N, cfg.time_embed_dim, **bf),
            semb=torch.empty(N, cfg.time_embed_dim, **bf),
            mod=torch.empty(N, self.mod_cols, **bf),
            po=torch.empty(N * P, self.w_out.shape[0], **bf),
        )
        if len(self._ws) >= 4:
            self._ws.pop(next(iter(self._ws)))
        self._ws[key] = ws
        return ws

    def _rope(self, image_rotary_emb):
        if image_rotary_emb is None:
            return None, None
        cos, sin = image_rotary_emb
        key = (cos.data_ptr(), sin.data_ptr(), tuple(cos.shape))
        hit = self._rope_cache.get(key)
        if hit is None:
            hit = (cos.to(device=self.device, dtype=torch.float32).contiguous(),
                   sin.to(device=self.device, dtype=torch.float32).contiguous())
            self._rope_cache = {key: hit}
        return hit

    def forward_assembled(self, latents, conds, encoder_hidden_states, timestep, image_rotary_emb=None, ofs=None):
        cfg = self.config
        N = len(conds)
        lat = latents.to(device=self.device, dtype=torch.bfloat16).contiguous()
        Bl, Fr, C, Hh, Ww = lat.shape
        if Bl not in (1, N):
            raise ValueError("latents batch must be 1 or len(conds)")
        if 2 * C != cfg.in_channels:
            raise ValueError("latents have %d channels, transformer expects in_channels=%d" % (C, cfg.in_channels))
        conds = [c.to(device=self.device, dtype=torch.bfloat16).contiguous() for c in conds]
        for c in conds:
            if c.numel() != Fr * C * Hh * Ww:
                raise ValueError("conditioning latents must have shape [1, F, C, H, W] matching the latents")
        ehs = encoder_hidden_states.to(device=self.device, dtype=torch.bfloat16).contiguous()
        if ehs.shape[0] != N:
            raise ValueError("encoder_hidden_states batch %d != %d samples" % (ehs.shape[0], N))
        T = ehs.shape[1]
        p, p_t = cfg.patch_size, self.p_t
        if Fr % p_t:
            raise ValueError("latent frames (%d) must be a multiple of patch_size_t=%d (cog:963-968 pads them)" % (Fr, p_t))
        P = (Fr // p_t) * (Hh // p) * (Ww // p)
        S = T + P
        D, Hn = cfg.inner_dim, cfg.num_attention_heads
        if cfg.use_learned_positional_embeddings:
            if cfg.sample_width != Ww or cfg.sample_height != Hh:
                raise ValueError(
                    "It is currently not possible to generate videos at a different resolution that the defaults. "
                    "This should only be the case with 'THUDM/CogVideoX-5b-I2V'.")
        pos_emb = self._positional(Hh, Ww, Fr, S)
        ws = self._workspace(N, S, P)
        x, y, qk, vt, att, h, mod = ws["x"], ws["y"], ws["qk"], ws["vt"], ws["att"], ws["h"], ws["mod"]
        S_pad = ws["S_pad"]
        cos, sin = self._rope(image_rotary_emb)
        G = _lib.gemm
        TM = self._timed

        ts = timestep.to(device=self.device, dtype=torch.float32).contiguous()
        if ts.numel() != N:
            ts = ts.reshape(-1)[:1].expand(N).contiguous()
        _lib.timestep_embedding(ts, ws["tsin"], N, D, cfg.flip_sin_to_cos)
        E = cfg.time_embed_dim
        G(ws["tsin"], self.w_t1, ws["t1"], N, E, D, D, D, E, bias=self.b_t1, act=_lib.ACT_SILU)
        if cfg.ofs_embed_dim is None:
            G(ws["t1"], self.w_t2, ws["semb"], N, E, E, E, E, E, bias=self.b_t2, act=_lib.ACT_SILU)
        else:
            if ofs is None:
                raise ValueError("this transformer has an ofs embedding: pass `ofs` (cog:998)")
            O = cfg.ofs_embed_dim
            emb, osin, o1, oemb = (torch.empty(N, E, device=self.device, dtype=torch.bfloat16) for _ in range(4))
            G(ws["t1"], self.w_t2, emb, N, E, E, E, E, E, bias=self.b_t2)
            ofs_v = ofs.to(device=self.device, dtype=torch.float32).reshape(-1)
            ofs_v = (ofs_v if ofs_v.numel() == N else ofs_v[:1].expand(N)).contiguous()
            _lib.timestep_embedding(ofs_v, osin, N, O, cfg.flip_sin_to_cos)
            G(osin, self.w_o1, o1, N, O, O, O, O, O, bias=self.b_o1, act=_lib.ACT_SILU)
            G(o1, self.w_o2, oemb, N, O, O, O, O, O, bias=self.b_o2)
            _lib.lincomb([(1.0, emb), (1.0, oemb)], torch.bfloat16, out=emb)
            _lib.silu(emb, ws["semb"])
        G(ws["semb"], self.w_mod, mod, N, self.mod_cols, E, E, E, self.mod_cols, bias=self.b_mod)

        G(ehs, self.w_text, x, T, D, cfg.text_embed_dim, cfg.text_embed_dim, cfg.text_embed_dim, D,
          bias=self.b_text, R=pos_emb, ldr=D, batch=N, strideA=T * cfg.text_embed_dim, strideC=S * D)
        _lib.patchify(lat, 0 if Bl == 1 else Fr * C * Hh * Ww, conds, ws["patches"], N, Fr, C, Hh, Ww, p, p_t)
        G(ws["patches"], self.w_patch, x, P, D, self.k_patch, self.k_patch, self.k_patch, D, bias=self.b_patch,
          R=pos_emb, ldr=D, r_off=T * D, batch=N, strideA=P * self.k_patch, strideC=S * D, c_off=T * D)

        scale = 1.0 / math.sqrt(cfg.attention_head_dim)
        prescale = self.attn_prescale
        q_scale = scale * 1.4426950408889634 if prescale else 1.0
        F4 = cfg.ff_inner_mult * D
        packed = self.packed_weights and os.environ.get("ALG_GEMM_PIPE", "10") == "10"
        wo_k, wf1_k, wf2_k = ("pwo", "pwf1", "pwf2") if packed else ("wo", "wf1", "wf2")
        for li, L in enumerate(self.layers):
            m1 = li * 12 * D
            m2 = m1 + 6 * D
            TM("ln_mod", _lib.layernorm_modulate, x, y, L["norm1_w"], L["norm1_b"], mod, mod, self.mod_cols, N, S, D,
               T, cfg.norm_eps, scale_off=m1 + 2 * D, shift_off=m1)
            qk_call = ((y, L["wqk"], qk, S, 2 * D, D, D, D, 2 * D), dict(bias=L["bqk"], batch=N, strideA=S * D, strideC=S * 2 * D))
            vt_call = ((L["wv"], y, vt, D, S, D, D, D, S_pad), dict(bias=L["bv"], batch=N, strideB=S * D, strideC=D * S_pad,
                                                                   flags=_lib.GEMM_BIAS_PER_ROW | _lib.GEMM_PERMUTE_COLS))
            if self.pair_qkv and self.fuse_qk_norm:
                TM("gemm_qkv", _lib.gemm_pair_qk, qk_call, vt_call, L["norm_q_w"], L["norm_q_b"], L["norm_k_w"], L["norm_k_b"], cos, sin,
                               Hn, T, cfg.qk_norm_eps, q_scale=q_scale)
            else:
                if self.pair_qkv:
                    TM("gemm_qkv", _lib.gemm_pair, qk_call, vt_call)
                else:
                    TM("gemm_qk", G, *qk_call[0], **qk_call[1])
                    TM("gemm_vt", G, *vt_call[0], **vt_call[1])
                TM("qk_norm_rope", _lib.qk_norm_rope_, qk, L["norm_q_w"], L["norm_q_b"], L["norm_k_w"], L["norm_k_b"], cos, sin, N, S, Hn, T,
                                   cfg.qk_norm_eps, q_scale=q_scale)
            TM("attn", _lib.flash_attn_d64, qk, qk, vt, att, N, Hn, S, S * 2 * D, 2 * D, D * S_pad, S_pad, S * D, D, scale,
                                k_off=D, q_prescaled=prescale)
            TM("gemm_out", G, att, L[wo_k], x, S, D, D, D, D, D, bias=L["bo"], R=x, ldr=D, gate=mod, gate_off=m1 + 4 * D,
              strideGate=self.mod_cols, seg_split=T, batch=N, strideA=S * D, strideC=S * D, strideR=S * D)
            TM("ln_mod", _lib.layernorm_modulate, x, y, L["norm2_w"], L["norm2_b"], mod, mod, self.mod_cols, N, S, D,
               T, cfg.norm_eps, scale_off=m2 + 2 * D, shift_off=m2)
            TM("gemm_ff1", G, y, L[wf1_k], h, S, F4, D, D, D, F4, bias=L["bf1"], act=_lib.ACT_GELU_TANH, batch=N, strideA=S * D,
              strideC=S * F4)
            TM("gemm_ff2", G, h, L[wf2_k], x, S, D, F4, F4, F4, D, bias=L["bf2"], R=x, ldr=D, gate=mod, gate_off=m2 + 4 * D,
              strideGate=self.mod_cols, seg_split=T, batch=N, strideA=S * F4, strideC=S * D, strideR=S * D)

        _lib.layernorm_modulate(x, y, self.norm_final_w, self.norm_final_b, None, None, 0, N, S, D, T, cfg.norm_eps)
        mo = cfg.num_layers * 12 * D
        _lib.layernorm_modulate(y, att, self.norm_out_w, self.norm_out_b, mod, mod, self.mod_cols, N, P, D, 0,
                                cfg.norm_eps, x_bstride=S * D, y_bstride=P * D, x_off=T * D, scale_off=mo + 2 * D,
                                shift_off=mo)
        n_out = self.w_out.shape[0]
        G(att, self.w_out, ws["po"], N * P, n_out, D, D, D, n_out, bias=self.b_out)
        out = torch.empty(N, Fr, cfg.out_channels, Hh, Ww, device=self.device, dtype=torch.bfloat16)
        _lib.unpatchify(ws["po"], out, N, Fr, cfg.out_channels, Hh, Ww, p, p_t)
        return out

    def __call__(self, hidden_states, encoder_hidden_states, timestep, timestep_cond=None, ofs=None,
                 image_rotary_emb=None, attention_kwargs=None, return_dict=True):
        if timestep_cond is not None:
            raise NotImplementedError("timestep_cond is not used by the CogVideoX I2V checkpoints")
        C = hidden_states.shape[2] // 2
        lat = hidden_states[:, :, :C].contiguous()
        conds = [hidden_states[n:n + 1, :, C:].contiguous() for n in range(hidden_states.shape[0])]
        out = self.forward_assembled(lat, conds, encoder_hidden_states, timestep, image_rotary_emb, ofs=ofs)
        if not return_dict:
            return (out,)
        return TransformerOutput(sample=out)


@dataclass
class TransformerOutput:
    sample: torch.Tensor
```

### alg_amd/transformer_wan.py

```python
from __future__ import annotations

import glob
import json
import math
import os
from dataclasses import asdict, dataclass
from types import SimpleNamespace

import torch

from . import _lib

BF = torch.bfloat16


@dataclass
class WanTransformerConfig:
    patch_size: tuple = (1, 2, 2)
    num_attention_heads: int = 40
    attention_head_dim: int = 128
    in_channels: int = 36
    out_channels: int = 16
    text_dim: int = 4096
    freq_dim: int = 256
    ffn_dim: int = 13824
    num_layers: int = 40
    cross_attn_norm: bool = True
    qk_norm: str = "rms_norm_across_heads"
    eps: float = 1e-6
    image_dim: int = 1280
    added_kv_proj_dim: int = 5120
    rope_max_seq_len: int = 1024
    pos_embed_seq_len: int = None

    @property
    def dim(self):
        return self.num_attention_heads * self.attention_head_dim

    def to_dict(self):
        return asdict(self)


def parameter_shapes(cfg):
    D, Ff = cfg.dim, cfg.ffn_dim
    pt, ph, pw = cfg.patch_size
    f32 = torch.float32
    s = {"patch_embedding.weight": ((D, cfg.in_channels, pt, ph, pw), BF), "patch_embedding.bias": ((D,), BF)}
    ce = "condition_embedder."
    s[ce + "time_embedder.linear_1.weight"] = ((D, cfg.freq_dim), f32)
    s[ce + "time_embedder.linear_1.bias"] = ((D,), f32)
    s[ce + "time_embedder.linear_2.weight"] = ((D, D), f32)
    s[ce + "time_embedder.linear_2.bias"] = ((D,), f32)
    for n, shp in (("time_proj", (6 * D, D)), ("text_embedder.linear_1", (D, cfg.text_dim)),
                   ("text_embedder.linear_2", (D, D))):
        s[ce + n + ".weight"] = (shp, BF)
        s[ce + n + ".bias"] = ((shp[0],), BF)
    if cfg.image_dim is not None:
        I = cfg.image_dim
        for n, shp in (("image_embedder.ff.net.0.proj", (I, I)), ("image_embedder.ff.net.2", (D, I))):
            s[ce + n + ".weight"] = (shp, BF)
            s[ce + n + ".bias"] = ((shp[0],), BF)
        for n, d in (("image_embedder.norm1", I), ("image_embedder.norm2", D)):
            s[ce + n + ".weight"] = ((d,), BF)
            s[ce + n + ".bias"] = ((d,), BF)
        if cfg.pos_embed_seq_len is not None:
            s[ce + "image_embedder.pos_embed"] = ((1, cfg.pos_embed_seq_len, I), BF)
    for l in range(cfg.num_layers):
        b = f"blocks.{l}."
        s[b + "scale_shift_table"] = ((1, 6, D), f32)
        for a in ("attn1", "attn2"):
            names = ["to_q", "to_k", "to_v", "to_out.0"]
            if a == "attn2" and cfg.added_kv_proj_dim is not None:
                names += ["add_k_proj", "add_v_proj"]
            for n in names:
                s[b + f"{a}.{n}.weight"] = ((D, D), BF)
                s[b + f"{a}.{n}.bias"] = ((D,), BF)
            s[b + f"{a}.norm_q.weight"] = ((D,), BF)
            s[b + f"{a}.norm_k.weight"] = ((D,), BF)
            if a == "attn2" and cfg.added_kv_proj_dim is not None:
                s[b + f"{a}.norm_added_k.weight"] = ((D,), BF)
        if cfg.cross_attn_norm:
            s[b + "norm2.weight"] = ((D,), f32)
            s[b + "norm2.bias"] = ((D,), f32)
        s[b + "ffn.net.0.proj.weight"] = ((Ff, D), BF)
        s[b + "ffn.net.0.proj.bias"] = ((Ff,), BF)
        s[b + "ffn.net.2.weight"] = ((D, Ff), BF)
        s[b + "ffn.net.2.bias"] = ((D,), BF)
    s["scale_shift_table"] = ((1, 2, D), f32)
    n_out = cfg.out_channels * pt * ph * pw
    s["proj_out.weight"] = ((n_out, D), BF)
    s["proj_out.bias"] = ((n_out,), BF)
    return s


def synthetic_state_dict(cfg, seed=1234, device="cuda"):
    dev = torch.device(device)
    g = torch.Generator(device=dev).manual_seed(seed)
    sd = {}
    for name, (shape, dt) in parameter_shapes(cfg).items():
        r = lambda: torch.randn(shape, generator=g, device=dev, dtype=torch.float32)
        if "scale_shift_table" in name:
            t = r() / shape[-1] ** 0.5
        elif name.endswith("weight") and len(shape) == 1:
            t = 1.0 + 0.1 * r()
        elif name.endswith("bias"):
            t = 0.02 * r()
        elif name.endswith("pos_embed"):
            t = 0.5 * r()
        else:
            t = r() / math.prod(shape[1:]) ** 0.5
        sd[name] = t.to(dt)
    return sd


class WanTransformer3DModel:
    dtype = BF

    def __init__(self, config: WanTransformerConfig, weights: dict, device="cuda", fp8=False):
        self.fp8 = bool(fp8)
        self.pair_qkv = True
        self.dual_cross = True
        self.fuse_quant = True
        self.packed_weights = True
        if config.qk_norm != "rms_norm_across_heads" or config.attention_head_dim != 128:
            raise NotImplementedError("the Wan DiT path is built for rms_norm_across_heads and head_dim 128")
        if tuple(config.patch_size)[0] != 1:
            raise NotImplementedError("temporal patch size 1 only (every Wan 2.1 checkpoint)")
        if config.pos_embed_seq_len is not None and config.image_dim is None:
            raise ValueError("pos_embed_seq_len (FLF2V) needs an image embedder (image_dim)")
        self.config = config
        self.device = torch.device(device)
        dev = self.device
        if dev.type != "cuda":
            raise _lib.AlgHipError("WanTransformer3DModel runs on the GPU only (HIP kernels); there is no CPU fallback")
        _lib.load_library()
        missing = [k for k in parameter_shapes(config) if k not in weights]
        if missing:
            raise KeyError("state dict is missing %d tensors, e.g. %s" % (len(missing), missing[:3]))
        D = config.dim
        bf = lambda n: weights[n].to(device=dev, dtype=BF).contiguous()
        f32 = lambda n: weights[n].to(device=dev, dtype=torch.float32).contiguous()
        w = SimpleNamespace()
        kin = config.in_channels * config.patch_size[1] * config.patch_size[2]
        self.k_patch = (kin + 63) // 64 * 64
        wp = torch.zeros(D, self.k_patch, dtype=BF, device=dev)
        wp[:, :kin] = bf("patch_embedding.weight").reshape(D, kin)
        w.patch_w, w.patch_b = wp, bf("patch_embedding.bias")
        ce = "condition_embedder."
        w.t1_w, w.t1_b = f32(ce + "time_embedder.linear_1.weight"), f32(ce + "time_embedder.linear_1.bias")
        w.t2_w, w.t2_b = f32(ce + "time_embedder.linear_2.weight"), f32(ce + "time_embedder.linear_2.bias")
        w.tp_w, w.tp_b = bf(ce + "time_proj.weight"), bf(ce + "time_proj.bias")
        w.x1_w, w.x1_b = bf(ce + "text_embedder.linear_1.weight"), bf(ce + "text_embedder.linear_1.bias")
        w.x2_w, w.x2_b = bf(ce + "text_embedder.linear_2.weight"), bf(ce + "text_embedder.linear_2.bias")
        self.has_image = config.image_dim is not None
        if self.has_image:
            ie = ce + "image_embedder."
            w.in1_w, w.in1_b = f32(ie + "norm1.weight"), f32(ie + "norm1.bias")
            w.in2_w, w.in2_b = f32(ie + "norm2.weight"), f32(ie + "norm2.bias")
            w.if1_w, w.if1_b = bf(ie + "ff.net.0.proj.weight"), bf(ie + "ff.net.0.proj.bias")
            w.if2_w, w.if2_b = bf(ie + "ff.net.2.weight"), bf(ie + "ff.net.2.bias")
            w.img_pos = bf(ie + "pos_embed").reshape(-1, config.image_dim) if config.pos_embed_seq_len is not None else None
        w.tables = torch.stack([f32(f"blocks.{l}.scale_shift_table").reshape(6, D)
                                for l in range(config.num_layers)]).contiguous()
        w.table_out = f32("scale_shift_table").reshape(1, 2, D).contiguous()
        w.out_w, w.out_b = bf("proj_out.weight"), bf("proj_out.bias")
        self.blocks = []
        for l in range(config.num_layers):
            b = f"blocks.{l}."
            L = SimpleNamespace()
            L.wqk = torch.cat([bf(b + "attn1.to_q.weight"), bf(b + "attn1.to_k.weight")], dim=0).contiguous()
            L.bqk = torch.cat([bf(b + "attn1.to_q.bias"), bf(b + "attn1.to_k.bias")]).contiguous()
            L.wv, L.bv = bf(b + "attn1.to_v.weight"), bf(b + "attn1.to_v.bias")
            L.wo, L.bo = bf(b + "attn1.to_out.0.weight"), bf(b + "attn1.to_out.0.bias")
            L.nq, L.nk = bf(b + "attn1.norm_q.weight"), bf(b + "attn1.norm_k.weight")
            L.n2w = f32(b + "norm2.weight") if config.cross_attn_norm else None
            L.n2b = f32(b + "norm2.bias") if config.cross_attn_norm else None
            L.cq_w, L.cq_b = bf(b + "attn2.to_q.weight"), bf(b + "attn2.to_q.bias")
            L.ck_w, L.ck_b = bf(b + "attn2.to_k.weight"), bf(b + "attn2.to_k.bias")
            L.cv_w, L.cv_b = bf(b + "attn2.to_v.weight"), bf(b + "attn2.to_v.bias")
            L.co_w, L.co_b = bf(b + "attn2.to_out.0.weight"), bf(b + "attn2.to_out.0.bias")
            L.cnq, L.cnk = bf(b + "attn2.norm_q.weight"), bf(b + "attn2.norm_k.weight")
            if config.added_kv_proj_dim is not None:
                L.ak_w, L.ak_b = bf(b + "attn2.add_k_proj.weight"), bf(b + "attn2.add_k_proj.bias")
                L.av_w, L.av_b = bf(b + "attn2.add_v_proj.weight"), bf(b + "attn2.add_v_proj.bias")
                L.cnak = bf(b + "attn2.norm_added_k.weight")
            L.f1_w, L.f1_b = bf(b + "ffn.net.0.proj.weight"), bf(b + "ffn.net.0.proj.bias")
            L.f2_w, L.f2_b = bf(b + "ffn.net.2.weight"), bf(b + "ffn.net.2.bias")
            if self.fp8:
                for name in ("wqk", "wv", "wo", "cq_w", "co_w", "f1_w", "f2_w"):
                    wt = getattr(L, name)
                    q = torch.empty(wt.shape, dtype=torch.uint8, device=dev)
                    sc = torch.empty(wt.shape[0], dtype=torch.float32, device=dev)
                    _lib.quantize_fp8_rows(wt, q, sc, wt.shape[0], wt.shape[1])
                    setattr(L, name, (q, sc))
            else:
                L.packed = {name: _lib.PackedB(getattr(L, name)) for name in ("wo", "cq_w", "co_w", "f1_w", "f2_w")}
            self.blocks.append(L)
        self.w = w
        self._ws = {}
        self._rope_cache = {}
        self.profile = None

    @classmethod
    def from_synthetic(cls, config=None, seed=1234, device="cuda", fp8=False):
        config = config or WanTransformerConfig()
        return cls(config, synthetic_state_dict(config, seed=seed, device=device), device=device, fp8=fp8)

    @classmethod
    def from_pretrained(cls, path, subfolder="transformer", torch_dtype=BF, device="cuda", fp8=False, **_):
        root = os.path.join(path, subfolder) if subfolder and os.path.isdir(os.path.join(path, subfolder)) else path
        cfg_path = os.path.join(root, "config.json")
        if not os.path.exists(cfg_path):
            raise FileNotFoundError("%s not found: weights must be on local disk (no network access in this build; use "
                                    "WanTransformer3DModel.from_synthetic for shape-faithful synthetic weights)" % cfg_path)
        with open(cfg_path) as f:
            raw = json.load(f)
        fields = WanTransformerConfig.__dataclass_fields__
        cfg = WanTransformerConfig(**{k: (tuple(v) if k == "patch_size" else v) for k, v in raw.items() if k in fields})
        from .weights import read_shards
        sd = read_shards(root)
        return cls(cfg, sd, device=device, fp8=fp8)

    def to(self, *args, **kwargs):
        return self

    def _timed(self, name, fn, *a, **k):
        if self.profile is None:
            return fn(*a, **k)
        e0, e1 = torch.cuda.Event(enable_timing=True), torch.cuda.Event(enable_timing=True)
        e0.record()
        r = fn(*a, **k)
        e1.record()
        self.profile.setdefault(name, []).append((e0, e1))
        return r

    def rope_tables(self, F_, H, W):
        key = (F_, H, W)
        hit = self._rope_cache.get(key)
        if hit is None:
            cfg = self.config
            d = cfg.attention_head_dim
            pt, ph, pw = cfg.patch_size
            h_dim = w_dim = 2 * (d // 6)
            t_dim = d - h_dim - w_dim
            tabs = []
            for dim in (t_dim, h_dim, w_dim):
                freqs = 1.0 / (10000.0 ** (torch.arange(0, dim, 2, dtype=torch.float64)[: dim // 2] / dim))
                tabs.append(torch.outer(torch.arange(cfg.rope_max_seq_len, dtype=torch.float64), freqs))
            ppf, pph, ppw = F_ // pt, H // ph, W // pw
            ang = torch.cat([tabs[0][:ppf].view(ppf, 1, 1, -1).expand(ppf, pph, ppw, -1),
                             tabs[1][:pph].view(1, pph, 1, -1).expand(ppf, pph, ppw, -1),
                             tabs[2][:ppw].view(1, 1, ppw, -1).expand(ppf, pph, ppw, -1)], dim=-1)
            ang = ang.reshape(ppf * pph * ppw, -1)
            hit = (torch.cos(ang).float().to(self.device).contiguous(), torch.sin(ang).float().to(self.device).contiguous())
            self._rope_cache[key] = hit
        return hit

    def _workspace(self, N, S, n_txt, n_img):
        key = (N, S, n_txt, n_img)
        ws = self._ws.get(key)
        if ws is None:
            self._ws.clear()
            cfg, dev = self.config, self.device
            D, Ff = cfg.dim, cfg.ffn_dim
            e = lambda *s, dt=BF: torch.empty(*s, dtype=dt, device=dev)
            z = lambda *s, dt=BF: torch.zeros(*s, dtype=dt, device=dev)
            ws = SimpleNamespace()
            ws.S_pad = (S + 63) // 64 * 64
            ws.patches = e(N, S, self.k_patch)
            ws.x, ws.y, ws.att, ws.qc = e(N, S, D), e(N, S, D), e(N, S, D), e(N, S, D)
            ws.qk = e(N, S, 2 * D)
            ws.vt = z(N, D, ws.S_pad)
            ws.h = e(N, S, Ff)
            ws.o2 = None
            ws.tok = e(N, S, self.w.out_w.shape[0])
            if self.fp8:
                ws.q8 = e(N * S, max(D, Ff), dt=torch.uint8)
                ws.q8s = e(N * S, dt=torch.float32)
            ws.temb_f32 = e(N, cfg.freq_dim, dt=torch.float32)
            ws.t1 = e(N, D, dt=torch.float32)
            ws.temb, ws.temb_silu = e(N, D), e(N, D)
            ws.tproj = e(N, 6 * D)
            ws.mod = e(cfg.num_layers, N, 6, D, dt=torch.float32)
            ws.mod_out = e(1, N, 2, D, dt=torch.float32)
            ws.txt_h, ws.txt = e(N, n_txt, D), e(N, n_txt, D)
            ws.kt = e(N, n_txt, D)
            ws.txt_pad = (n_txt + 63) // 64 * 64
            ws.vtt = z(N, D, ws.txt_pad)
            if n_img:
                I = cfg.image_dim
                ws.img_n, ws.img_h = e(N, n_img, I), e(N, n_img, I)
                ws.img_p, ws.img = e(N, n_img, D), e(N, n_img, D)
                ws.ki = e(N, n_img, D)
                ws.img_pad = (n_img + 63) // 64 * 64
                ws.vti = z(N, D, ws.img_pad)
            self._ws[key] = ws
        return ws

    def __call__(self, hidden_states, timestep, encoder_hidden_states, encoder_hidden_states_image=None,
                 attention_kwargs=None, return_dict=True):
        cfg, w, G, T = self.config, self.w, _lib.gemm, self._timed
        if hidden_states.device.type != "cuda":
            raise _lib.AlgHipError("WanTransformer3DModel needs device tensors; there is no CPU fallback")
        N, C, F_, H, W = hidden_states.shape
        pt, ph, pw = cfg.patch_size
        if C != cfg.in_channels or H % ph or W % pw:
            raise ValueError(f"hidden_states must be [N, {cfg.in_channels}, F, H, W] with H, W divisible by the patch size")
        if self.has_image and encoder_hidden_states_image is None:
            raise ValueError("this checkpoint has an image embedder: pass encoder_hidden_states_image")
        D, Ff, heads = cfg.dim, cfg.ffn_dim, cfg.num_attention_heads
        S = F_ * (H // ph) * (W // pw)
        n_txt = encoder_hidden_states.shape[1]
        if encoder_hidden_states_image is not None and cfg.pos_embed_seq_len is not None:
            b2, s2, i2 = encoder_hidden_states_image.shape
            if (b2 * s2) % cfg.pos_embed_seq_len or b2 * s2 // cfg.pos_embed_seq_len != N:
                raise ValueError("FLF2V: encoder_hidden_states_image %s does not view as [%d, %d, %d]" % (
                    tuple(encoder_hidden_states_image.shape), N, cfg.pos_embed_seq_len, i2))
            encoder_hidden_states_image = encoder_hidden_states_image.reshape(N, cfg.pos_embed_seq_len, i2)
        n_img = encoder_hidden_states_image.shape[1] if encoder_hidden_states_image is not None else 0
        ws = self._workspace(N, S, n_txt, n_img)
        S_pad, scale = ws.S_pad, 1.0 / math.sqrt(cfg.attention_head_dim)
        cos, sin = self.rope_tables(F_, H, W)
        hs = hidden_states.to(BF).contiguous()
        ehs_in = encoder_hidden_states.to(BF).contiguous()

        T("patchify", _lib.patchify3d, hs, ws.patches, N, C, F_, H, W, ph, pw, self.k_patch)
        T("gemm_patch", G, ws.patches, w.patch_w, ws.x, N * S, D, self.k_patch, self.k_patch, self.k_patch, D, bias=w.patch_b)
        t = timestep.to(device=self.device, dtype=torch.float32).reshape(-1)
        if t.numel() == 1:
            t = t.expand(N)
        t = t.contiguous()
        _lib.timestep_embedding_f32(t, ws.temb_f32, N, cfg.freq_dim)
        _lib.linear_f32(ws.temb_f32, w.t1_w, w.t1_b, ws.t1, None, None, N, D, cfg.freq_dim, act=1)
        _lib.linear_f32(ws.t1, w.t2_w, w.t2_b, None, ws.temb, ws.temb_silu, N, D, D, act=0)
        G(ws.temb_silu, w.tp_w, ws.tproj, N, 6 * D, D, D, D, 6 * D, bias=w.tp_b)
        _lib.wan_modulation(w.tables, ws.tproj, ws.mod, cfg.num_layers, N, 6, D, True)
        _lib.wan_modulation(w.table_out, ws.temb, ws.mod_out, 1, N, 2, D, False)
        G(ehs_in, w.x1_w, ws.txt_h, N * n_txt, D, cfg.text_dim, cfg.text_dim, cfg.text_dim, D, bias=w.x1_b,
          act=_lib.ACT_GELU_TANH)
        G(ws.txt_h, w.x2_w, ws.txt, N * n_txt, D, D, D, D, D, bias=w.x2_b)
        if n_img:
            I = cfg.image_dim
            im = encoder_hidden_states_image.to(BF).contiguous()
            if w.img_pos is not None:
                im = torch.stack([_lib.lincomb([(1.0, im[n]), (1.0, w.img_pos)], BF) for n in range(N)])
            _lib.layernorm_mod_f32(im, ws.img_n, w.in1_w, w.in1_b, None, None, 0, N, n_img, I, 1e-5)
            G(ws.img_n, w.if1_w, ws.img_h, N * n_img, I, I, I, I, I, bias=w.if1_b)
            _lib.gelu_erf_(ws.img_h)
            G(ws.img_h, w.if2_w, ws.img_p, N * n_img, D, I, I, I, D, bias=w.if2_b)
            _lib.layernorm_mod_f32(ws.img_p, ws.img, w.in2_w, w.in2_b, None, None, 0, N, n_img, D, 1e-5)

        mod_bs = 6 * D

        def lin(name, A, Wt, C, M_, N_, K_, lda, ldc, requant=True, **kw):
            if not self.fp8:
                return T(name, G, A, (packed.get(id(Wt)) or Wt) if packed else Wt, C, M_, N_, K_, lda, K_, ldc, **kw)
            if requant:
                T("quant", _lib.quantize_fp8_rows, A, ws.q8, ws.q8s, N * S, K_, x_rstride=lda)
            sa = kw.pop("strideA", 0)
            return T(name, G, ws.q8, Wt[0], C, M_, N_, K_, K_, K_, ldc, a_scale=ws.q8s, b_scale=Wt[1],
                     strideA=(S * K_ if sa else 0), strideAScale=(S if sa else 0), **kw)

        fuse_q = self.fp8 and D % 512 == 0 and self.fuse_quant

        def ln_mod(wgt, bia, sc, sh, bs, **kw):
            if fuse_q:
                return T("ln_mod", _lib.layernorm_mod_f32_fp8, ws.x, ws.q8, ws.q8s, wgt, bia, sc, sh, bs, N, S, D, cfg.eps, **kw)
            return T("ln_mod", _lib.layernorm_mod_f32, ws.x, ws.y, wgt, bia, sc, sh, bs, N, S, D, cfg.eps, **kw)

        use_packed = not self.fp8 and self.packed_weights and os.environ.get("ALG_GEMM_PIPE", "10") == "10"
        packed = None
        for li, L in enumerate(self.blocks):
            if use_packed:
                packed = {id(getattr(L, name)): pw for name, pw in L.packed.items()}
            m0 = li * N * 6 * D
            ln_mod(None, None, ws.mod, ws.mod, mod_bs, scale_off=m0 + D, shift_off=m0)
            vt_kw = dict(bias=L.bv, batch=N, strideB=S * D, strideC=D * S_pad, flags=_lib.GEMM_BIAS_PER_ROW | _lib.GEMM_PERMUTE_COLS)
            if self.fp8:
                lin("gemm_qk", ws.y, L.wqk, ws.qk, N * S, 2 * D, D, D, 2 * D, requant=not fuse_q, bias=L.bqk)
                T("gemm_vt", G, L.wv[0], ws.q8, ws.vt, D, S, D, D, D, S_pad, a_scale=L.wv[1], b_scale=ws.q8s, strideBScale=S, **vt_kw)
            elif self.pair_qkv:
                T("gemm_qkv", _lib.gemm_pair, ((ws.y, L.wqk, ws.qk, N * S, 2 * D, D, D, D, 2 * D), dict(bias=L.bqk)),
                  ((L.wv, ws.y, ws.vt, D, S, D, D, D, S_pad), vt_kw))
            else:
                lin("gemm_qk", ws.y, L.wqk, ws.qk, N * S, 2 * D, D, D, 2 * D, bias=L.bqk)
                T("gemm_vt", G, L.wv, ws.y, ws.vt, D, S, D, D, D, S_pad, **vt_kw)
            T("rms_rope", _lib.rmsnorm_rope_, ws.qk, L.nq, cos, sin, 2 * D, N, S, D, cfg.eps)
            T("rms_rope", _lib.rmsnorm_rope_, ws.qk, L.nk, cos, sin, 2 * D, N, S, D, cfg.eps, x_off=D)
            T("attn_self", _lib.flash_attn_d128, ws.qk, ws.qk, ws.vt, ws.att, N, heads, S, S, S * 2 * D, 2 * D,
              S * 2 * D, 2 * D, D * S_pad, S_pad, S * D, D, scale, k_off=D)
            lin("gemm_out", ws.att, L.wo, ws.x, S, D, D, D, D, bias=L.bo, R=ws.x, ldr=D, gate=ws.mod,
                gate_off=m0 + 2 * D, strideGate=mod_bs, batch=N, strideA=S * D, strideC=S * D, strideR=S * D,
                seg_split=1 << 30, flags=_lib.GEMM_GATE_F32)
            if cfg.cross_attn_norm:
                ln_mod(L.n2w, L.n2b, None, None, 0)
                lin("gemm_cq", ws.y, L.cq_w, ws.qc, N * S, D, D, D, D, requant=not fuse_q, bias=L.cq_b)
            else:
                lin("gemm_cq", ws.x, L.cq_w, ws.qc, N * S, D, D, D, D, bias=L.cq_b)
            T("rms_rope", _lib.rmsnorm_rope_, ws.qc, L.cnq, None, None, D, N, S, D, cfg.eps)
            G(ws.txt, L.ck_w, ws.kt, N * n_txt, D, D, D, D, D, bias=L.ck_b)
            _lib.rmsnorm_rope_(ws.kt, L.cnk, None, None, D, N, n_txt, D, cfg.eps)
            G(L.cv_w, ws.txt, ws.vtt, D, n_txt, D, D, D, ws.txt_pad, bias=L.cv_b, batch=N, strideB=n_txt * D,
              strideC=D * ws.txt_pad, flags=_lib.GEMM_BIAS_PER_ROW | _lib.GEMM_PERMUTE_COLS)
            if n_img:
                G(ws.img, L.ak_w, ws.ki, N * n_img, D, D, D, D, D, bias=L.ak_b)
                _lib.rmsnorm_rope_(ws.ki, L.cnak, None, None, D, N, n_img, D, cfg.eps)
                G(L.av_w, ws.img, ws.vti, D, n_img, D, D, D, ws.img_pad, bias=L.av_b, batch=N, strideB=n_img * D,
                  strideC=D * ws.img_pad, flags=_lib.GEMM_BIAS_PER_ROW | _lib.GEMM_PERMUTE_COLS)
            if n_img and self.dual_cross:
                T("attn_cross", _lib.flash_attn_d128_dual, ws.qc, ws.kt, ws.vtt, n_txt, n_txt * D, D, D * ws.txt_pad, ws.txt_pad,
                  ws.ki, ws.vti, n_img, n_img * D, D, D * ws.img_pad, ws.img_pad, ws.att, N, heads, S, S * D, D, S * D, D, scale)
            else:
                T("attn_cross", _lib.flash_attn_d128, ws.qc, ws.kt, ws.vtt, ws.att, N, heads, S, n_txt, S * D, D, n_txt * D, D,
                  D * ws.txt_pad, ws.txt_pad, S * D, D, scale)
                if n_img:
                    if ws.o2 is None:
                        ws.o2 = torch.empty_like(ws.att)
                    T("attn_cross", _lib.flash_attn_d128, ws.qc, ws.ki, ws.vti, ws.o2, N, heads, S, n_img, S * D, D, n_img * D,
                      D, D * ws.img_pad, ws.img_pad, S * D, D, scale)
                    T("add", _lib.lincomb, [(1.0, ws.att), (1.0, ws.o2)], BF, out=ws.att)
            lin("gemm_cout", ws.att, L.co_w, ws.x, N * S, D, D, D, D, bias=L.co_b, R=ws.x, ldr=D)
            ln_mod(None, None, ws.mod, ws.mod, mod_bs, scale_off=m0 + 4 * D, shift_off=m0 + 3 * D)
            lin("gemm_ff1", ws.y, L.f1_w, ws.h, N * S, Ff, D, D, Ff, requant=not fuse_q, bias=L.f1_b,
                act=_lib.ACT_GELU_TANH)
            lin("gemm_ff2", ws.h, L.f2_w, ws.x, S, D, Ff, Ff, D, bias=L.f2_b, R=ws.x, ldr=D, gate=ws.mod,
                gate_off=m0 + 5 * D, strideGate=mod_bs, batch=N, strideA=S * Ff, strideC=S * D, strideR=S * D,
                seg_split=1 << 30, flags=_lib.GEMM_GATE_F32)

        _lib.layernorm_mod_f32(ws.x, ws.y, None, None, ws.mod_out, ws.mod_out, 2 * D, N, S, D, cfg.eps, scale_off=D,
                               shift_off=0)
        n_out = w.out_w.shape[0]
        G(ws.y, w.out_w, ws.tok, N * S, n_out, D, D, D, n_out, bias=w.out_b)
        out = torch.empty(N, cfg.out_channels, F_, H, W, dtype=BF, device=self.device)
        _lib.unpatchify3d(ws.tok, n_out, out, N, cfg.out_channels, F_, H, W, ph, pw)
        if not return_dict:
            return (out,)
        return SimpleNamespace(sample=out)
```

### include/alg_hip.h

```cpp
#ifndef ALG_HIP_H
#define ALG_HIP_H

#include <stdint.h>

#ifdef __cplusplus
extern "C" {
#endif

#define ALG_F32 0
#define ALG_BF16 1

#define ALG_OK 0
#define ALG_EINVAL (-1)
#define ALG_ELAUNCH (-2)
#define ALG_ELIMIT (-3)

#define ALG_VERSION 110

int alg_version(void);
const char* alg_last_error(void);

void alg_reload_env(void);


int alg_down_up(const void* in, void* out, int64_t planes, int H, int W, int h1, int w1, int dtype,
                int round_intermediate, const void* tables, void* workspace, int64_t workspace_bytes, void* stream);

int64_t alg_lowpass_tables_bytes(int H, int W, int h1, int w1);
int alg_lowpass_tables_build(void* tables, int64_t bytes, int H, int W, int h1, int w1, void* stream);

int64_t alg_down_up_workspace_bytes(int64_t planes, int H, int W, int h1, int w1);

int alg_gaussian_blur(const void* in, void* out, int64_t planes, int H, int W, int ksize, float sigma, int dtype,
                      void* workspace, int64_t workspace_bytes, void* stream);
int64_t alg_gaussian_blur_workspace_bytes(int64_t planes, int H, int W, int ksize);

int alg_cfg_ddim_step(const void* pred, int pred_dtype, void* latents, int lat_dtype, int n_pass, int64_t numel,
                      float guidance_scale, float sqrt_alpha_t, float sqrt_beta_t, float coef_a, float coef_b,
                      void* stream);

int alg_cfg_combine(const void* pred, void* out, int dtype, int n_pass, int64_t numel, float guidance_scale,
                    void* stream);

int alg_lincomb(const void* const* xs, const float* coefs, const int* dtypes, int n_terms, void* out, int out_dtype,
                int64_t numel, void* stream);

int alg_concat_cast(const void* const* src0, int dtype0, const void* const* src1, int dtype1, int n, int64_t O,
                    int64_t A0, int64_t A1, int64_t R, int64_t s0_ostride, int64_t s1_ostride, int64_t a1_off,
                    void* out, int out_dtype, void* stream);

int alg_unipc_update(const float* x, const float* m0, const float* m1, const float* m_new, float* out,
                     int64_t numel, float r, float c, float k, float rk, float rho0, float rho_new, void* stream);


#define ALG_ACT_NONE 0
#define ALG_ACT_GELU_TANH 1
#define ALG_ACT_SILU 2

#define ALG_GEMM_BIAS_PER_ROW 1
#define ALG_GEMM_PERMUTE_COLS 4
#define ALG_GEMM_GATE_SEG_STRIDE 16
#define ALG_GEMM_B_PACKED11 32
#define ALG_GEMM_GATE_F32 8

typedef struct alg_gemm_args {
  const void* A;
  const void* B;
  void* C;
  const void* bias;
  const void* R;
  const void* gate;
  int64_t lda, ldb, ldc, ldr;
  int64_t strideA, strideB, strideC, strideR, strideGate;
  int32_t M, N, K, batch;
  int32_t seg_split;
  int32_t act;
  int32_t flags;
  int64_t gate_seg_stride;
  int32_t perm_col0;
  int32_t conv_cin_log2;
  const float* a_scale;
  const float* b_scale;
  int64_t strideAScale, strideBScale;
  int32_t conv_wp;
  int32_t conv_hpwp;
  int32_t conv_kw;
  int32_t reserved1;
} alg_gemm_args;

int alg_gemm_bf16(const alg_gemm_args* args, void* stream);

int64_t alg_pack_b_p11_bytes(int N, int K);
int alg_pack_b_p11(const void* w, void* packed, int N, int K, int64_t ldb, void* stream);

int alg_gemm_bf16_pair(const alg_gemm_args* a, const alg_gemm_args* b, void* stream);

typedef struct alg_qk_norm_rope_args {
  const void *wq, *bq, *wk, *bk;
  const float *cos_tab, *sin_tab;
  int32_t heads, text_len;
  float eps, q_scale;
} alg_qk_norm_rope_args;
int alg_gemm_bf16_pair_qk(const alg_gemm_args* qk, const alg_gemm_args* vt, const alg_qk_norm_rope_args* e, void* stream);

int alg_gemm_fp8(const alg_gemm_args* args, void* stream);

int alg_quantize_fp8_rows(const void* x, int64_t x_rstride, void* q, float* scale, int64_t rows, int K, void* stream);

int alg_flash_attn_d64(const void* q, const void* k, const void* vt, void* o, int batch, int heads, int S,
                       int64_t q_bstride, int64_t q_rstride, int64_t vt_bstride, int64_t vt_rstride,
                       int64_t o_bstride, int64_t o_rstride, float scale, void* stream);

#define ALG_ATTN_Q_PRESCALED 1
int alg_flash_attn_d64_ex(const void* q, const void* k, const void* vt, void* o, int batch, int heads, int S,
                          int64_t q_bstride, int64_t q_rstride, int64_t vt_bstride, int64_t vt_rstride,
                          int64_t o_bstride, int64_t o_rstride, float scale, int flags, void* workspace,
                          int64_t workspace_bytes, void* stream);
int64_t alg_flash_attn_d64_workspace_bytes(int batch, int heads, int S, int flags);

int alg_flash_attn_d128(const void* q, const void* k, const void* vt, void* o, int batch, int heads, int Sq, int Skv,
                        int64_t q_bstride, int64_t q_rstride, int64_t k_bstride, int64_t k_rstride, int64_t vt_bstride,
                        int64_t vt_rstride, int64_t o_bstride, int64_t o_rstride, float scale, void* stream);

int alg_flash_attn_d128_ex(const void* q, const void* k, const void* vt, void* o, int batch, int heads, int Sq, int Skv,
                           int64_t q_bstride, int64_t q_rstride, int64_t k_bstride, int64_t k_rstride, int64_t vt_bstride,
                           int64_t vt_rstride, int64_t o_bstride, int64_t o_rstride, float scale, int kv_group, int causal,
                           void* stream);

int alg_flash_attn_d128_dual(const void* q, const void* k, const void* vt, int Skv, int64_t k_bstride, int64_t k_rstride,
                             int64_t vt_bstride, int64_t vt_rstride, const void* k2, const void* vt2, int Skv2, int64_t k2_bstride,
                             int64_t k2_rstride, int64_t vt2_bstride, int64_t vt2_rstride, void* o, int batch, int heads, int Sq,
                             int64_t q_bstride, int64_t q_rstride, int64_t o_bstride, int64_t o_rstride, float scale, void* stream);

int alg_rope_half(void* x, const float* cos_tab, const float* sin_tab, const int* pos, int64_t rows, int heads,
                  int64_t x_rstride, void* stream);


int alg_embed_rows(const int64_t* ids, const void* table, void* out, int64_t n, int D, int vocab, void* stream);

int alg_t5_layernorm(const void* x, const void* weight, void* y, int64_t rows, int D, float eps, void* stream);

int alg_attn_bias(const void* q, const void* k, const void* v, void* out, const void* bias_table, const int* rel_bucket,
                  const int* key_mask, int batch, int heads, int head_dim, int L, int64_t qkv_rstride, int64_t out_rstride,
                  float scale, int causal, void* stream);

int alg_quick_gelu(void* x, int64_t numel, void* stream);

int alg_mul_bf16(const void* a, const void* b, void* out, int64_t numel, void* stream);


#define ALG_CONV_PLAIN 0
#define ALG_CONV_PAIR 1
#define ALG_CONV_STRIDE2 2
int alg_conv_cl_bf16(const void* x, const void* w, const void* bias, const void* res, void* y, int frames, int Hp,
                     int Wp, int Cin, int Cout, int kt, int mode, void* stream);

typedef struct alg_vae_geom {
  int32_t frames, H, W, C;
  int32_t first_len, seg_len;
  int32_t lat_first_single;
  int32_t lat_rate, lat_scale;
  int32_t lat_h, lat_w;
} alg_vae_geom;

int64_t alg_vae_groupnorm_workspace(const alg_vae_geom* g);
int alg_vae_groupnorm_stats(const void* x, const alg_vae_geom* g, float eps, void* workspace, float* stats, void* stream);

int alg_vae_spatial_norm(const void* x, const float* stats, const void* gamma, const void* beta, const void* zyb,
                         void* out, const alg_vae_geom* g, int silu, void* stream);

int alg_vae_group_norm(const void* x, const float* stats, const void* gamma, const void* beta, void* out,
                       const alg_vae_geom* g, int silu, void* stream);

int alg_vae_pad(const void* x, void* out, int frames, int H, int W, int C, void* stream);

int alg_vae_repitch(const void* x, void* out, int frames, int H, int W, int C, int src_rows, int src_wp, void* stream);

int alg_vae_unpack_planes(const void* x, void* out, int frames, int H, int W, int C, void* stream);

int alg_vae_upsample(const void* x, void* out, int frames_out, int H, int W, int C, int compress_time, int first_single,
                     void* stream);

int alg_vae_pack_latent(const void* z, int64_t c_stride, int64_t frame_stride, void* out, int frames, int h, int w,
                        int channels, float scale, void* stream);

int alg_vae_unpack_video(const void* x, void* out, int frames, int H, int W, int to_uint8, void* stream);


int alg_headnorm_rope(void* x, const void* weight, const float* cos_tab, const float* sin_tab, int64_t x_rstride,
                      int64_t x_bstride, int batch, int rows, int heads, int rope_tokens, float eps, void* stream);

int alg_masked_mean(const void* x, const int* valid, void* out, int batch, int L, int D, void* stream);

int alg_silu(const void* x, void* y, int64_t numel, void* stream);


int alg_layernorm_mod_f32(const void* x, void* y, const float* weight, const float* bias, const float* scale,
                          const float* shift, int64_t mod_bstride, int batch, int rows, int D, float eps, void* stream);

int alg_layernorm_mod_f32_fp8(const void* x, void* q8, float* q8_scale, const float* weight, const float* bias,
                              const float* scale, const float* shift, int64_t mod_bstride, int batch, int rows, int D,
                              float eps, void* stream);

int alg_rmsnorm_rope(void* x, const void* weight, const float* cos_tab, const float* sin_tab, int64_t x_rstride,
                     int batch, int rows, int D, float eps, void* stream);

int alg_wan_modulation(const float* table, const void* vec, float* out, int layers, int batch, int J, int D,
                       int vec_per_j, void* stream);

int alg_patchify3d(const void* in, void* out, int n, int C, int F, int H, int W, int ph, int pw, int Kpad, void* stream);

int alg_unpatchify3d(const void* in, int64_t ldin, void* out, int n, int C, int F, int H, int W, int ph, int pw,
                     int channel_major, void* stream);

int alg_timestep_embedding_f32(const float* t, float* out, int n, int dim, void* stream);

int alg_linear_f32(const float* x, const float* W, const float* b, float* y, void* y_bf16, void* y_silu_bf16, int M,
                   int N, int K, int act, void* stream);

int alg_gelu_erf(void* x, int64_t numel, void* stream);

int alg_layernorm_modulate(const void* x, void* y, const void* weight, const void* bias, const void* scale,
                           const void* shift, int64_t mod_bstride, int batch, int rows, int D, int64_t x_bstride,
                           int64_t y_bstride, int seg_split, float eps, void* stream);
int alg_layernorm_modulate_seg(const void* x, void* y, const void* weight, const void* bias, const void* scale,
                               const void* shift, int64_t mod_bstride, int64_t seg_stride, int batch, int rows, int D,
                               int64_t x_bstride, int64_t y_bstride, int seg_split, float eps, void* stream);

int alg_qk_norm_rope(void* qk, const void* wq, const void* bq, const void* wk, const void* bk, const float* cos_tab,
                     const float* sin_tab, int batch, int S, int heads, int text_len, float eps, void* stream);

int alg_qk_norm_rope_scaled(void* qk, const void* wq, const void* bq, const void* wk, const void* bk, const float* cos_tab,
                            const float* sin_tab, int batch, int S, int heads, int text_len, float eps, float q_scale,
                            void* stream);

int alg_patchify(const void* latents, int64_t lat_bstride, const void* const* cond_ptrs, void* out, int n_samples,
                 int frames, int C, int H, int W, int p, void* stream);

int alg_unpatchify(const void* in, void* out, int n_samples, int frames, int C, int H, int W, int p, void* stream);

int alg_patchify_t(const void* latents, int64_t lat_bstride, const void* const* cond_ptrs, void* out, int n_samples,
                   int frames, int C, int H, int W, int p, int p_t, void* stream);
int alg_unpatchify_t(const void* in, void* out, int n_samples, int frames, int C, int H, int W, int p, int p_t,
                     void* stream);

int alg_timestep_embedding(const float* t, void* out, int n, int dim, int flip_sin_to_cos, void* stream);


int alg_rms_norm_rows(const void* x, const void* gamma, void* y, int64_t rows, int C, int Cp, int silu, void* stream);

int alg_softmax_hilo(const void* neg_hi, const void* lo, void* p, int64_t rows, int cols, int64_t ld, float scale, void* stream);


int alg_calib_mfma_bf16(float* sink, int iters, unsigned seed, int blocks, uint64_t* clocks, void* stream);

int alg_wall_clock_khz(void);

void alg_attn_clock_tap(uint64_t* buffer, int slots);

#ifdef __cplusplus
}
#endif
#endif
```

Before: 1.557 frames/s.

## Fuse Q|K|V projection into one packed-B GEMM with transposed V epilogue

Measured after the change: 1.565 frames/s (median of 6 runs). Within noise of the previous version (+0.5%).

```diff
diff --git a/alg_amd/_lib.py b/alg_amd/_lib.py
--- a/alg_amd/_lib.py
+++ b/alg_amd/_lib.py
@@ -16,7 +16,7 @@
 GEMM_B_PACKED11 = 32
 
 EXPORTS = (
-    "alg_version", "alg_last_error", "alg_reload_env", "alg_down_up", "alg_gaussian_blur", "alg_cfg_ddim_step", "alg_gemm_bf16", "alg_gemm_bf16_pair", "alg_gemm_bf16_pair_qk", "alg_pack_b_p11", "alg_pack_b_p11_bytes",
+    "alg_version", "alg_last_error", "alg_reload_env", "alg_down_up", "alg_gaussian_blur", "alg_cfg_ddim_step", "alg_gemm_bf16", "alg_gemm_bf16_pair", "alg_gemm_bf16_pair_qk", "alg_gemm_bf16_qkv", "alg_pack_b_p11", "alg_pack_b_p11_bytes",
     "alg_flash_attn_d64", "alg_layernorm_modulate", "alg_qk_norm_rope", "alg_patchify", "alg_unpatchify",
     "alg_timestep_embedding", "alg_cfg_combine", "alg_lincomb", "alg_unipc_update", "alg_concat_cast", "alg_flash_attn_d128", "alg_layernorm_mod_f32", "alg_layernorm_mod_f32_fp8", "alg_rmsnorm_rope",
     "alg_wan_modulation", "alg_patchify3d", "alg_unpatchify3d", "alg_timestep_embedding_f32", "alg_linear_f32",
@@ -151,6 +151,7 @@
     lib.alg_gemm_bf16.argtypes = [POINTER(GemmArgs), c_void_p]
     lib.alg_gemm_bf16_pair.argtypes = [POINTER(GemmArgs), POINTER(GemmArgs), c_void_p]
     lib.alg_gemm_bf16_pair_qk.argtypes = [POINTER(GemmArgs), POINTER(GemmArgs), POINTER(QkNormRopeArgs), c_void_p]
+    lib.alg_gemm_bf16_qkv.argtypes = [POINTER(GemmArgs), POINTER(GemmArgs), c_void_p]
     lib.alg_flash_attn_d64.argtypes = [c_void_p, c_void_p, c_void_p, c_void_p, c_int, c_int, c_int, c_int64, c_int64,
                                        c_int64, c_int64, c_int64, c_int64, c_float, c_void_p]
     lib.alg_layernorm_modulate.argtypes = [c_void_p, c_void_p, c_void_p, c_void_p, c_void_p, c_void_p, c_int64, c_int,
@@ -675,6 +676,8 @@
     args = GemmArgs()
     fp8 = a_scale is not None
     if isinstance(B, PackedB):
+        if fp8:
+            raise AlgHipError("a packed B is a bf16 weight: no a_scale / b_scale")
         if (B.N, B.K) != (N, K) or b_off or strideB:
             raise AlgHipError("packed B was built for N = %d, K = %d (shared by the batch, no offset)" % (B.N, B.K))
         flags |= GEMM_B_PACKED11
@@ -749,6 +752,15 @@
     _check(lib.alg_gemm_bf16_pair_qk(ctypes.byref(a), ctypes.byref(b), ctypes.byref(e), _stream()), "alg_gemm_bf16_pair_qk")
 
 
+def gemm_qkv(qkv, vt):
+    lib = load_library()
+    a, fa = gemm_args(*qkv[0], **qkv[1])
+    b, fb = gemm_args(*vt[0], **vt[1])
+    if fa or fb:
+        raise AlgHipError("gemm_qkv takes bf16 problems")
+    _check(lib.alg_gemm_bf16_qkv(ctypes.byref(a), ctypes.byref(b), _stream()), "alg_gemm_bf16_qkv")
+
+
 def quantize_fp8_rows(x, q, scale, rows, K, x_rstride=None, x_off=0, q_off=0, scale_off=0):
     x_rstride = K if x_rstride is None else x_rstride
     _check(load_library().alg_quantize_fp8_rows(_p(x, x_off), x_rstride, _p(q, q_off), _p(scale, scale_off), rows, K,
diff --git a/alg_amd/csrc/gemm.hip b/alg_amd/csrc/gemm.hip
--- a/alg_amd/csrc/gemm.hip
+++ b/alg_amd/csrc/gemm.hip
@@ -16,6 +16,8 @@
 int launch_gemm_p10_pair_qk(const alg_gemm_args* a, int m_tiles_a, int n_tiles_a, const alg_gemm_args* b, int m_tiles_b, int n_tiles_b,
                             const alg_qk_norm_rope_args* e, hipStream_t s);
 int launch_gemm_p11(const alg_gemm_args* a, int m_tiles, int n_tiles, int64_t nwg, hipStream_t s);
+int launch_gemm_p11_qkv(const alg_gemm_args* a, int m_tiles, int n_tiles, int64_t nwg, void* vt, int64_t ldvt, int64_t stridevt,
+                        int split, hipStream_t s);
 int launch_gemm_p6_fp8(const alg_gemm_args* a, int m_tiles, int n_tiles, int64_t nwg, hipStream_t s);
 int launch_gemm_p9_fp8(const alg_gemm_args* a, int m_tiles, int n_tiles, int64_t nwg, hipStream_t s);
 int launch_gemm_p6_conv(const alg_gemm_args* a, int m_tiles, int n_tiles, int64_t nwg, hipStream_t s);
@@ -87,6 +89,13 @@
                 (long long)a->lda, a->conv_wp, a->conv_hpwp);
       return ALG_EINVAL;
     }
+  }
+  if ((a->flags & ALG_GEMM_B_PACKED11) &&
+      (fp8 || a->conv_wp || a->K < 128 || 256 * a->lda * 2 + (int64_t)a->K * 2 >= (1ll << 32) || a->strideB != 0 ||
+       (a->flags & (ALG_GEMM_BIAS_PER_ROW | ALG_GEMM_PERMUTE_COLS)) || ((uintptr_t)a->B & 15))) {
+    set_error("alg_gemm_bf16: a packed B (ALG_GEMM_B_PACKED11) needs bf16 operands, K >= 128, 32-bit byte offsets inside a 256-row A "
+              "panel, a B shared by the batch (strideB = 0) and a plain column layout (no per-row bias / column permutation)");
+    return ALG_EINVAL;
   }
   if (validate_only) return ALG_OK;
   if ((int64_t)a->M * a->ldc >= (1ll << 31) || (a->R && (int64_t)a->M * a->ldr >= (1ll << 31))) {
@@ -124,15 +133,7 @@
     return launch_gemm_p6_fp8(a, m_tiles, n_tiles, nwg, s);
   }
   if (a->conv_wp) return launch_gemm_p6_conv(a, m_tiles, n_tiles, nwg, s);
-  if (a->flags & ALG_GEMM_B_PACKED11) {
-    if (a->K < 128 || 256 * a->lda * 2 + (int64_t)a->K * 2 >= (1ll << 32) || a->strideB != 0 ||
-        (a->flags & (ALG_GEMM_BIAS_PER_ROW | ALG_GEMM_PERMUTE_COLS)) || ((uintptr_t)a->B & 15)) {
-      set_error("alg_gemm_bf16: a packed B (ALG_GEMM_B_PACKED11) needs K >= 128, 32-bit byte offsets inside a 256-row A panel, a B shared by "
-                "the batch (strideB = 0) and a plain column layout (no per-row bias / column permutation)");
-      return ALG_EINVAL;
-    }
-    return launch_gemm_p11(a, m_tiles, n_tiles, nwg, s);
-  }
+  if (a->flags & ALG_GEMM_B_PACKED11) return launch_gemm_p11(a, m_tiles, n_tiles, nwg, s);
   switch (gemm_pipe()) {
     case 9:
     case 10:
@@ -146,7 +147,7 @@
 extern "C" int alg_gemm_bf16(const alg_gemm_args* a, void* stream) { return gemm_entry(a, stream, false); }
 
 static bool pair_eligible(const alg_gemm_args* a) {
-  return a && a->A && a->B && a->C && !a->R && !a->gate && a->act == ALG_ACT_NONE && !a->conv_wp && a->M > 0 && a->N > 0 &&
+  return a && a->A && a->B && a->C && !(a->flags & ALG_GEMM_B_PACKED11) && !a->R && !a->gate && a->act == ALG_ACT_NONE && !a->conv_wp && a->M > 0 && a->N > 0 &&
          a->batch > 0 && a->K >= 128 && a->K % 64 == 0 && 256 * a->lda * 2 + (int64_t)a->K * 2 < (1ll << 32) &&
          256 * a->ldb * 2 + (int64_t)a->K * 2 < (1ll << 32) && (int64_t)a->M * a->ldc < (1ll << 31) &&
          !(a->lda % 8 || a->ldb % 8 || a->strideA % 8 || a->strideB % 8 || ((uintptr_t)a->A & 15) || ((uintptr_t)a->B & 15)) &&
@@ -173,6 +174,10 @@
   int rc = gemm_entry(a, stream, false, true);
   if (rc == ALG_OK) rc = gemm_entry(b, stream, false, true);
   if (rc != ALG_OK) return rc;
+  if ((a->flags | b->flags) & ALG_GEMM_B_PACKED11) {
+    set_error("alg_gemm_bf16_pair_qk: a packed B (ALG_GEMM_B_PACKED11) is not taken by the fused Q|K store loop");
+    return ALG_EINVAL;
+  }
   if (!e || !e->wq || !e->bq || !e->wk || !e->bk || e->heads <= 0 || e->text_len < 0 || e->text_len > a->M ||
       (e->cos_tab == nullptr) != (e->sin_tab == nullptr)) {
     set_error("alg_gemm_bf16_pair_qk: bad LayerNorm / rotary arguments");
@@ -202,6 +207,37 @@
   if (rc != ALG_OK) return rc;
   return alg_qk_norm_rope_scaled(a->C, e->wq, e->bq, e->wk, e->bk, e->cos_tab, e->sin_tab, a->batch, a->M, e->heads, e->text_len,
                                  e->eps, e->q_scale, stream);
+}
+
+extern "C" int alg_gemm_bf16_qkv(const alg_gemm_args* a, const alg_gemm_args* v, void* stream) {
+  if (!a || !v || !v->C) {
+    set_error("alg_gemm_bf16_qkv: null argument");
+    return ALG_EINVAL;
+  }
+  const int rc = gemm_entry(a, stream, false, true);
+  if (rc != ALG_OK) return rc;
+  const int D = a->N / 3, split = 2 * D;
+  const bool qk_ok = (a->flags == ALG_GEMM_B_PACKED11) && !a->R && !a->gate && a->act == ALG_ACT_NONE && !a->a_scale &&
+                     a->N % 3 == 0 && split % 256 == 0 && a->ldc >= split && a->ldc % 8 == 0 && a->strideC % 8 == 0 &&
+                     ((uintptr_t)a->C & 15) == 0 && (int64_t)a->M * a->ldc < (1ll << 31);
+  const bool vt_ok = (v->flags & ~ALG_GEMM_BIAS_PER_ROW) == ALG_GEMM_PERMUTE_COLS && v->perm_col0 == 0 && v->M == D && v->N == a->M && v->batch == a->batch &&
+                     v->ldc >= (((int64_t)a->M + 15) & ~15ll) && v->ldc % 8 == 0 && v->strideC % 8 == 0 &&
+                     (a->batch == 1 || v->strideC >= (int64_t)D * v->ldc) && ((uintptr_t)v->C & 15) == 0 &&
+                     (int64_t)D * v->ldc < (1ll << 31);
+  if (!qk_ok || !vt_ok) {
+    set_error("alg_gemm_bf16_qkv: not a Q|K|V call this launch takes (qkv: packed B, N = 3D with 2D %% 256 == 0, no residual / "
+              "activation, ldc >= 2D, 16-byte rows; vt: PERMUTE_COLS (+ BIAS_PER_ROW), M = D, N = S = qkv M, the same batch, ldc >= S rounded "
+              "up to 16, 16-byte rows) -- N=%d M=%d batch=%d / vt M=%d N=%d batch=%d ldc=%lld flags=%d",
+              a->N, a->M, a->batch, v->M, v->N, v->batch, (long long)v->ldc, v->flags);
+    return ALG_EINVAL;
+  }
+  const int m_tiles = (a->M + BM - 1) / BM, n_tiles = (a->N + BN - 1) / BN;
+  const int64_t nwg = (int64_t)m_tiles * n_tiles * a->batch;
+  if (nwg > 0x7fffffff) {
+    set_error("alg_gemm_bf16_qkv: grid too large");
+    return ALG_ELIMIT;
+  }
+  return launch_gemm_p11_qkv(a, m_tiles, n_tiles, nwg, v->C, v->ldc, v->strideC, split, (hipStream_t)stream);
 }
 
 extern "C" int alg_gemm_fp8(const alg_gemm_args* a, void* stream) { return gemm_entry(a, stream, true); }
diff --git a/alg_amd/csrc/gemm_kernel.h b/alg_amd/csrc/gemm_kernel.h
--- a/alg_amd/csrc/gemm_kernel.h
+++ b/alg_amd/csrc/gemm_kernel.h
@@ -111,9 +111,15 @@
 struct GemmPairQkArgs : GemmPairArgs {
   QkNormRope qe;
 };
+struct GemmVtArgs {
+  bf16_t* vt;
+  int64_t ldvt, stridevt;
+  int split;
+};
 template <int PAIR> struct GemmPairT { typedef GemmNoPair type; };
 template <> struct GemmPairT<1> { typedef GemmPairArgs type; };
 template <> struct GemmPairT<2> { typedef GemmPairQkArgs type; };
+template <> struct GemmPairT<3> { typedef GemmVtArgs type; };
 template <int ACT, bool RES, int PIPE, int WNW = 4, bool FP8 = false, bool CONV = false, int PAIR = 0>
 __global__ __launch_bounds__((PIPE == 11 ? 1 : 2) * WNW * 64) void gemm_bf16_kernel(
     const alg_gemm_args p1, int m_tiles1, int n_tiles1, int group_m1, const typename GemmPairT<PAIR>::type pr) {
@@ -122,7 +128,9 @@
   constexpr bool P11 = PIPE == 11;
   constexpr int WMW = P11 ? 1 : 2;
   constexpr int MT = BM / WMW / 32;
-  static_assert(!PAIR || (P9 && !P11 && !RES && ACT == ALG_ACT_NONE), "the pair launch is built for the plain schedule-9 / 10 kernels");
+  constexpr bool TWO = PAIR == 1 || PAIR == 2;
+  static_assert(!TWO || (P9 && !P11 && !RES && ACT == ALG_ACT_NONE), "the pair launch is built for the plain schedule-9 / 10 kernels");
+  static_assert(PAIR != 3 || (P11 && !RES && ACT == ALG_ACT_NONE), "the Q|K|V launch is built for the plain schedule-11 kernel");
   static_assert(!FP8 || PIPE == 6 || PIPE == 9, "the fp8 operands are built on the ping-pong schedule and on schedule 9");
   static_assert(!CONV || (PIPE == 6 && !FP8), "the convolution addressing is built on the bf16 ping-pong schedule");
   typedef typename std::conditional<FP8, uint8_t, bf16_t>::type elem_t;
@@ -162,13 +170,13 @@
   const int total1 = m_tiles1 * n_tiles1 * p1.batch;
   auto do_tile = [&](const int wg_in) __attribute__((always_inline)) {
   bool second = false;
-  if constexpr (PAIR) second = wg_in >= total1;
+  if constexpr (TWO) second = wg_in >= total1;
   const alg_gemm_args& p = [&]() -> const alg_gemm_args& {
-    if constexpr (PAIR) return second ? pr.p : p1;
+    if constexpr (TWO) return second ? pr.p : p1;
     else return p1;
   }();
   int m_tiles = m_tiles1, n_tiles = n_tiles1, group_m = group_m1, wg = wg_in;
-  if constexpr (PAIR) {
+  if constexpr (TWO) {
     if (second) m_tiles = pr.m_tiles, n_tiles = pr.n_tiles, group_m = pr.group_m, wg = wg_in - total1;
   }
   const int tiles = m_tiles * n_tiles;
@@ -1152,6 +1160,58 @@
             return;
           }
         }
+        if constexpr (PAIR == 3) {
+          if (n0 >= pr.split) {
+            typedef short v4i16_t __attribute__((ext_vector_type(4)));
+            typedef uint32_t v2u_t __attribute__((ext_vector_type(2)));
+            const int gq = lane_e >> 4, quad = ((gq & 1) << 1) | (gq >> 1), li = lane_e & 15, hs = lane_e >> 5, ss = gq & 1;
+            const int lq = li >> 2, lp = li & 3;
+            int lo[2];
+#pragma unroll
+            for (int fp = 0; fp < 2; ++fp) lo[fp] = (4 * quad + lq) * 64 + ((((lp >> 1) + 2 * fp) ^ quad) * 16) + (lp & 1) * 8;
+            bf16_t* const vtb = pr.vt + (int64_t)b * pr.stridevt + m0;
+            const int ldv = (int)pr.ldvt;
+            static_for<4>([&](auto f_c) {
+              constexpr int F = decltype(f_c)::value, nt = F >> 1, fp = F & 1;
+              const int n = n0 + blk_col(nt) + fp * 16 + li;
+              bf16_t* const vrow = vtb + (int64_t)(n - pr.split) * ldv + 16 * ss + 8 * hs;
+              static_for<2>([&](auto h_c) {
+                constexpr int G0 = decltype(h_c)::value * 8;
+                v2u_t x[8];
+                static_for<8>([&](auto j_c) {
+                  constexpr int G = G0 + decltype(j_c)::value;
+                  const v4i16_t r = __builtin_amdgcn_ds_read_tr16_b64_v4i16(
+                      (__attribute__((address_space(3))) v4i16_t*)(my + ((G >> 1) * NT + nt) * 2048 + (G & 1) * 1024 + lo[fp]));
+                  x[decltype(j_c)::value] = __builtin_bit_cast(v2u_t, r);
+                });
+                static_for<4>([&](auto k_c) {
+                  constexpr int k = decltype(k_c)::value, G = G0 + 2 * k;
+                  v2u_t a = x[2 * k], c = x[2 * k + 1];
+#pragma unroll
+                  for (int w = 0; w < 2; ++w) {
+                    const auto r = __builtin_amdgcn_permlane16_swap(a[w], c[w], false, false);
+                    a[w] = r[0], c[w] = r[1];
+                  }
+                  const int t0 = m0 + 16 * (G + ss);
+                  if (n < p.N) {
+                    bf16_t* const dst = vrow + 16 * G;
+                    if (t0 + 16 <= p.M) {
+                      ALG_STORE16(dst, make_uint4(a[0], a[1], c[0], c[1]));
+                    } else {
+                      const uint32_t u[4] = {a[0], a[1], c[0], c[1]};
+#pragma unroll
+                      for (int e = 0; e < 8; ++e)
+                        if (t0 + (e & 3) + 4 * hs + 8 * (e >> 2) < p.M)
+                          ((uint16_t*)dst)[e] = (uint16_t)(u[e >> 1] >> (16 * (e & 1)));
+                    }
+                  }
+                });
+                __builtin_amdgcn_sched_barrier(0);
+              });
+            });
+            return;
+          }
+        }
         if (perm) plain_loop(IntC<1>{}); else plain_loop(IntC<0>{});
         return;
       }
@@ -1301,7 +1361,7 @@
   };
 
   int total_wg = total1;
-  if constexpr (PAIR) total_wg += pr.m_tiles * pr.n_tiles * pr.p.batch;
+  if constexpr (TWO) total_wg += pr.m_tiles * pr.n_tiles * pr.p.batch;
   for (int L = blockIdx.x; L < total_wg; L += gridDim.x) {
     const int xcd = L & 7, q = total_wg >> 3, r = total_wg & 7;
     const int wg = (xcd < r ? xcd * (q + 1) : r * (q + 1) + (xcd - r) * q) + (L >> 3);
diff --git a/alg_amd/csrc/gemm_p11.hip b/alg_amd/csrc/gemm_p11.hip
--- a/alg_amd/csrc/gemm_p11.hip
+++ b/alg_amd/csrc/gemm_p11.hip
@@ -3,6 +3,26 @@
 namespace alg {
 int launch_gemm_p11(const alg_gemm_args* a, int m_tiles, int n_tiles, int64_t nwg, hipStream_t s) {
   return launch_gemm<11, 4>(a, m_tiles, n_tiles, nwg, s);
+}
+
+int launch_gemm_p11_qkv(const alg_gemm_args* a, int m_tiles, int n_tiles, int64_t nwg, void* vt, int64_t ldvt, int64_t stridevt,
+                        int split, hipStream_t s) {
+  const void* fn = (const void*)gemm_bf16_kernel<ALG_ACT_NONE, false, 11, 4, false, false, 3>;
+  static PerDeviceOnce attr_set;
+  const int dev_slot = current_device_slot();
+  if (!device_done(attr_set, dev_slot)) {
+    hipError_t e = hipFuncSetAttribute(fn, hipFuncAttributeMaxDynamicSharedMemorySize, GEMM_LDS_P9);
+    if (e != hipSuccess) {
+      set_error("alg_gemm_bf16_qkv: hipFuncSetAttribute(%d B LDS): %s", GEMM_LDS_P9, hipGetErrorString(e));
+      return ALG_ELAUNCH;
+    }
+    device_mark(attr_set, dev_slot);
+  }
+  GemmVtArgs v;
+  v.vt = (bf16_t*)vt, v.ldvt = ldvt, v.stridevt = stridevt, v.split = split;
+  hipLaunchKernelGGL((gemm_bf16_kernel<ALG_ACT_NONE, false, 11, 4, false, false, 3>), dim3(gemm_grid(nwg)), dim3(256), GEMM_LDS_P9, s, *a,
+                     m_tiles, n_tiles, gemm_group_m(11, n_tiles, a->K), v);
+  return check_launch("alg_gemm_bf16_qkv");
 }
 
 __global__ __launch_bounds__(256) void pack_b_p11_kernel(const bf16_t* __restrict__ w, uint4* __restrict__ out, int N, int K, int64_t ldb,
diff --git a/alg_amd/transformer_cogvideox.py b/alg_amd/transformer_cogvideox.py
--- a/alg_amd/transformer_cogvideox.py
+++ b/alg_amd/transformer_cogvideox.py
@@ -70,6 +70,7 @@
         self.pair_qkv = True
         self.fuse_qk_norm = False
         self.packed_weights = True
+        self.packed_qkv = True
         self._sincos = {}
         dev = self.device
         w = weights
@@ -120,6 +121,8 @@
             L["bf2"] = _bf(w[b + "ff.net.2.bias"], dev)
             for nm in ("wo", "wf1", "wf2"):
                 L["p" + nm] = _lib.PackedB(L[nm])
+            L["pwqkv"] = _lib.PackedB(torch.cat([L["wqk"], L["wv"]], dim=0))
+            L["bqkv"] = torch.cat([L["bqk"], L["bv"]])
             self.layers.append(L)
         ow, ob = w["norm_out.linear.weight"], w["norm_out.linear.bias"]
         sh_w, sc_w = ow.chunk(2, dim=0)
@@ -315,6 +318,7 @@
         F4 = cfg.ff_inner_mult * D
         packed = self.packed_weights and os.environ.get("ALG_GEMM_PIPE", "10") == "10"
         wo_k, wf1_k, wf2_k = ("pwo", "pwf1", "pwf2") if packed else ("wo", "wf1", "wf2")
+        qkv_one = packed and self.pair_qkv and self.packed_qkv and not self.fuse_qk_norm
         for li, L in enumerate(self.layers):
             m1 = li * 12 * D
             m2 = m1 + 6 * D
@@ -327,7 +331,14 @@
                 TM("gemm_qkv", _lib.gemm_pair_qk, qk_call, vt_call, L["norm_q_w"], L["norm_q_b"], L["norm_k_w"], L["norm_k_b"], cos, sin,
                                Hn, T, cfg.qk_norm_eps, q_scale=q_scale)
             else:
-                if self.pair_qkv:
+                if qkv_one:
+                    qkv_call = ((y, L["pwqkv"], qk, S, 3 * D, D, D, D, 2 * D), dict(bias=L["bqkv"], batch=N, strideA=S * D,
+                                                                                   strideC=S * 2 * D))
+                    try:
+                        TM("gemm_qkv", _lib.gemm_qkv, qkv_call, vt_call)
+                    except _lib.AlgHipError:
+                        TM("gemm_qkv", _lib.gemm_pair, qk_call, vt_call)
+                elif self.pair_qkv:
                     TM("gemm_qkv", _lib.gemm_pair, qk_call, vt_call)
                 else:
                     TM("gemm_qk", G, *qk_call[0], **qk_call[1])
diff --git a/alg_amd/transformer_wan.py b/alg_amd/transformer_wan.py
--- a/alg_amd/transformer_wan.py
+++ b/alg_amd/transformer_wan.py
@@ -122,6 +122,7 @@
         self.dual_cross = True
         self.fuse_quant = True
         self.packed_weights = True
+        self.packed_qkv = True
         if config.qk_norm != "rms_norm_across_heads" or config.attention_head_dim != 128:
             raise NotImplementedError("the Wan DiT path is built for rms_norm_across_heads and head_dim 128")
         if tuple(config.patch_size)[0] != 1:
@@ -195,6 +196,8 @@
                     setattr(L, name, (q, sc))
             else:
                 L.packed = {name: _lib.PackedB(getattr(L, name)) for name in ("wo", "cq_w", "co_w", "f1_w", "f2_w")}
+                L.pwqkv = _lib.PackedB(torch.cat([L.wqk, L.wv], dim=0))
+                L.bqkv = torch.cat([L.bqk, L.bv])
             self.blocks.append(L)
         self.w = w
         self._ws = {}
@@ -380,8 +383,18 @@
                 lin("gemm_qk", ws.y, L.wqk, ws.qk, N * S, 2 * D, D, D, 2 * D, requant=not fuse_q, bias=L.bqk)
                 T("gemm_vt", G, L.wv[0], ws.q8, ws.vt, D, S, D, D, D, S_pad, a_scale=L.wv[1], b_scale=ws.q8s, strideBScale=S, **vt_kw)
             elif self.pair_qkv:
-                T("gemm_qkv", _lib.gemm_pair, ((ws.y, L.wqk, ws.qk, N * S, 2 * D, D, D, D, 2 * D), dict(bias=L.bqk)),
-                  ((L.wv, ws.y, ws.vt, D, S, D, D, D, S_pad), vt_kw))
+                qk_call = ((ws.y, L.wqk, ws.qk, N * S, 2 * D, D, D, D, 2 * D), dict(bias=L.bqk))
+                vt_call = ((L.wv, ws.y, ws.vt, D, S, D, D, D, S_pad), vt_kw)
+                done = False
+                if use_packed and self.packed_qkv:
+                    try:
+                        T("gemm_qkv", _lib.gemm_qkv, ((ws.y, L.pwqkv, ws.qk, S, 3 * D, D, D, D, 2 * D),
+                                                      dict(bias=L.bqkv, batch=N, strideA=S * D, strideC=S * 2 * D)), vt_call)
+                        done = True
+                    except _lib.AlgHipError:
+                        pass
+                if not done:
+                    T("gemm_qkv", _lib.gemm_pair, qk_call, vt_call)
             else:
                 lin("gemm_qk", ws.y, L.wqk, ws.qk, N * S, 2 * D, D, D, 2 * D, bias=L.bqk)
                 T("gemm_vt", G, L.wv, ws.y, ws.vt, D, S, D, D, D, S_pad, **vt_kw)
diff --git a/include/alg_hip.h b/include/alg_hip.h
--- a/include/alg_hip.h
+++ b/include/alg_hip.h
@@ -103,6 +103,8 @@
 } alg_qk_norm_rope_args;
 int alg_gemm_bf16_pair_qk(const alg_gemm_args* qk, const alg_gemm_args* vt, const alg_qk_norm_rope_args* e, void* stream);
 
+int alg_gemm_bf16_qkv(const alg_gemm_args* qkv, const alg_gemm_args* vt, void* stream);
+
 int alg_gemm_fp8(const alg_gemm_args* args, void* stream);
 
 int alg_quantize_fp8_rows(const void* x, int64_t x_rstride, void* q, float* scale, int64_t rows, int K, void* stream);
```
